# karfly/learnable-triangulation-pytorch

Hardware: AMD Instinct MI355X
Metric: multi-view samples/sec (4-view vol-softmax forward) (higher is better)
Workload: dtype bf16

## Files before the change

include/lt_hip.h:

```cpp
#ifndef LT_HIP_H
#define LT_HIP_H

#include <stddef.h>
#include <stdint.h>

#ifdef __cplusplus
extern "C" {
#endif

#define LT_ABI_VERSION 1

enum { LT_F32 = 0, LT_BF16 = 1,
       LT_FP8 = 2  };
enum { LT_OK = 0, LT_ERR_INVALID = -1, LT_ERR_UNSUPPORTED = -2, LT_ERR_LAUNCH = -3 };

enum { LT_AGG_SUM = 0, LT_AGG_MAX = 1, LT_AGG_SOFTMAX = 2, LT_AGG_CONF = 3,
       LT_AGG_CONF_NORM = 4  };

enum {
    LT_EPI_RELU_PRE = 1,
    LT_EPI_RELU_POST = 2,
    LT_EPI_STORE_F32 = 4,
    LT_EPI_SIGMOID = 8,
    LT_EPI_RES_F32 = 64,
    LT_BN_FROZEN = 32,
    LT_BN_Y_BF16 = 128,
    LT_ACT_BF16 = 256
};

const char* lt_last_error(void);
int lt_abi_version(void);
int lt_device_info(int* cu_count, int* lds_per_cu, char* arch, int arch_len);

#define LT_CONV_MAX_PHASES 8

typedef struct lt_conv_phase {
    const void* weight;
    const int32_t* taps;
    int32_t ntaps;
    int32_t out_off[3];
    const void* weight_frag;
    int32_t weight_frag_layout;
} lt_conv_phase;

typedef struct lt_conv_desc {
    int32_t dtype;
    int32_t N, D, H, W, Cin;
    int32_t Do, Ho, Wo;
    int32_t stride[3], pad[3];
    int32_t OD, OH, OW;
    int32_t out_stride[3];
    int32_t Cout, ldc;
    int32_t cout_pad, k_pad;
    int32_t nphase;
    int32_t flags;
    int32_t tile;
    int32_t stages;
    lt_conv_phase phase[LT_CONV_MAX_PHASES];
} lt_conv_desc;

int lt_conv_pack_weights(const void* weight, int32_t cout_pad, int32_t k_pad, void* packed, void* stream);
int lt_conv_pack_weights_t32(const void* weight, int32_t cout_pad, int32_t k_pad, int32_t cin, int32_t ntaps, void* packed,
                             void* stream);
int lt_conv_pack_weights32(const void* weight, int32_t cout_pad, int32_t k_pad, void* packed, void* stream);

enum { LT_TILE_AUTO = 0,
       LT_TILE_128x128 = 1, LT_TILE_128x64 = 2, LT_TILE_256x32 = 3, LT_TILE_256x16 = 4, LT_TILE_64x64 = 5,
       LT_TILE2_128x128 = 11, LT_TILE2_128x64 = 12, LT_TILE2_256x32 = 13, LT_TILE2_256x16 = 14, LT_TILE2_64x64 = 15,
       LT_TILE_HALO = 20,
       LT_TILE3_288 = 30,
       LT_TILE_DIRECT = 99  };

int lt_conv_fwd(const lt_conv_desc* desc, const void* x, const float* bias, const float* scale, const float* shift,
                const void* residual, void* y, void* stream);
typedef struct lt_conv_skip {
    const void* x;
    int32_t cin;
    const void* weight_frag;
} lt_conv_skip;
int lt_conv_skip_fwd(const lt_conv_desc* desc, const void* x, const float* bias, const float* scale, const float* shift,
                     const lt_conv_skip* skip, void* y, void* stream);
typedef struct lt_conv_cat2 {
    const void* x;
    int32_t cin, H, W, stride;
} lt_conv_cat2;
int lt_conv_cat2_fwd(const lt_conv_desc* desc, const void* x, const lt_conv_cat2* second, const float* bias, const float* scale, const float* shift,
                     const void* residual, void* y, void* stream);
int lt_conv_cout_pad(int32_t cout);
int32_t lt_conv_chunk_samples(int32_t N, int64_t per_sample);

typedef struct lt_wshape {
    int32_t nd;
    int64_t s[5];
} lt_wshape;
int lt_sel_conv_skip(int32_t dtype, const int32_t x[5], const lt_wshape* w, const int32_t skip_x[5], const lt_wshape* skip_w);
int lt_sel_conv_cat2(int32_t dtype, const int32_t t2[5], const lt_wshape* w_expand, const int32_t x[5], const lt_wshape* w_down, int32_t stride_down);
int lt_sel_splitk_slices(const lt_conv_desc* d, const lt_wshape* w, int32_t transposed);
int lt_sel_bottleneck(int32_t dtype, const int32_t x[5], const lt_wshape w[3], const int32_t strides[3]);
int lt_sel_bottleneck_ds(int32_t dtype, const int32_t x[5], const lt_wshape w[3], const int32_t strides[3], const lt_wshape* w_down, int32_t stride_down);
int lt_sel_expand_reduce(int32_t dtype, const int32_t t2[5], const int32_t res[5], const lt_wshape* w_expand, const lt_wshape* w_reduce);
int lt_sel_stem_pool(int32_t dtype, const int32_t x[5], const lt_wshape* w, int32_t stride, int32_t pad, const int32_t pool[3]);
int lt_sel_pwchain(int32_t dtype, const int32_t x[5], int32_t nlayers, const lt_wshape* w);
int lt_sel_frag_layout(const lt_conv_desc* d, const lt_wshape* w, int32_t transposed, int32_t has_residual);

int lt_maxpool_fwd(int32_t dtype, const void* x, void* y, int32_t N, int32_t D, int32_t H, int32_t W, int32_t C,
                   const int32_t k[3], const int32_t s[3], const int32_t p[3], void* stream);

int lt_global_avgpool(int32_t dtype, const void* x, void* y, int32_t N, int32_t HW, int32_t C, void* stream);

int lt_nchw_to_nhwc(int32_t dtype, const float* x, void* y, int32_t N, int32_t C, int32_t HW, int32_t c_pad, void* stream);
int lt_nhwc_to_nchw_f32(int32_t dtype, const void* x, float* y, int32_t N, int32_t C, int32_t HW, int32_t ld, void* stream);

int lt_splitk_reduce(int32_t dtype, const float* partial, int32_t S, int64_t N, int64_t rows_per_sample, int32_t C, const float* bias,
                     const float* scale, const float* shift, const void* residual, void* y, int32_t flags, void* stream);

int lt_coord_volumes(const float* pos, const float* center, const float* rot, float step, int32_t B, int32_t V,
                     int32_t cmu_transfer, float* coords, void* stream);
int lt_rotate_points(const float* x, const float* rot, float* y, int64_t n, void* stream);

int lt_unproject_fwd(int32_t dtype, const void* feats, const float* proj, const float* coords, const float* conf,
                     void* out, int32_t B, int32_t NV, int32_t C, int32_t h, int32_t w, int32_t v0, int32_t v1,
                     int32_t v2, int32_t agg, void* stream);
int lt_unproject_grid_fwd(int32_t dtype, const void* feats, const float* proj, const float* pos, const float* center, const float* rot,
                          float step, int32_t cmu_transfer, float* coords_out, const float* conf, void* out, int32_t B, int32_t NV,
                          int32_t C, int32_t h, int32_t w, int32_t V, int32_t agg, void* stream);
enum { LT_KIND_MPII = 0, LT_KIND_COCO = 1 };
int lt_cuboid_from_keypoints(const float* keypoints_3d, int32_t B, int32_t J, int32_t kind, double cuboid_side, float* pos, float* center,
                             void* stream);

size_t lt_softargmax3d_workspace(int32_t B, int32_t J, int64_t nvox);
int lt_softargmax3d_fwd(const float* logits, const float* coords, float mult, int32_t softmax, int32_t channels_last,
                        int32_t ld, float* kp, float* probs, int32_t B, int32_t J, int64_t nvox, void* workspace,
                        void* stream);

int lt_softargmax2d_fwd(const float* heatmaps, float mult, int32_t softmax, float* coords, float* probs, int32_t NJ,
                        int32_t h, int32_t w, void* stream);
int lt_softargmax2d_bwd(const float* probs, const float* coords, const float* grad_coords, float mult, int32_t softmax, float* grad_heatmaps,
                        int32_t NJ, int32_t h, int32_t w, void* stream);
int lt_triangulate_dlt_bwd(const float* proj, const float* points, const float* conf, const float* grad_out, float* grad_points, float* grad_conf,
                           int32_t B, int32_t NV, int32_t J, void* stream);

size_t lt_unproject_bwd_workspace(int32_t B, int32_t NV, int32_t C, int32_t v0, int32_t v1, int32_t v2);
int lt_unproject_bwd(int32_t dtype, const void* feats, const float* proj, const float* coords, const float* conf, const float* grad_out,
                     float* grad_feats, float* grad_conf, int32_t B, int32_t NV, int32_t C, int32_t h, int32_t w, int32_t v0, int32_t v1,
                     int32_t v2, int32_t agg, void* workspace, size_t workspace_bytes, void* stream);
int lt_softargmax3d_bwd(const float* probs, const float* coords, const float* kp, const float* grad_kp, const int32_t* gp_idx,
                        const float* gp_val, float multiplier, int32_t softmax, int32_t channels_last, float* grad_logits, int32_t B,
                        int32_t J, int64_t nvox, void* stream);
int lt_softargmax3d_bwd_dense(const float* probs, const float* coords, const float* kp, const float* grad_kp, const int32_t* gp_idx,
                              const float* gp_val, const float* gp_dense, float* workspace_bj, float multiplier, int32_t softmax,
                              int32_t channels_last, float* grad_logits, int32_t B, int32_t J, int64_t nvox, void* stream);
int lt_volumetric_ce_fwd(const float* coords, const float* probs, const float* keypoints_gt, const float* validity, float* terms,
                         int32_t* idx, float* grad_val, int32_t B, int32_t J, int64_t nvox, void* stream);
size_t lt_bn_stats_workspace(int64_t rows, int32_t C);
int lt_bn_stats_fwd(int32_t dtype, const void* x, int64_t rows, int32_t C, float* mean, float* var, float* running_mean,
                    float* running_var, float momentum, void* workspace, void* stream);

int lt_bn_act_fwd(const void* y , const float* mean, const float* var, const float* gamma, const float* beta, const void* residual, void* z,
                  void* z_bf16 , int64_t rows, int32_t C, float eps,
                  int32_t flags, void* stream);
size_t lt_bn_act_bwd_workspace(int64_t rows, int32_t C);
int lt_bn_act_bwd(const void* dz, const void* y , const void* residual, const float* mean, const float* var, const float* gamma, const float* beta,
                  void* dy, void* dy_bf16 , float* dgamma, float* dbeta, void* dres, int32_t accumulate_res,
                  int64_t rows, int32_t C, float eps, int32_t flags, void* workspace, void* stream);
int lt_act_bwd(const void* dz, const void* z, const void* residual, void* dy, void* dres, int32_t accumulate_res, int64_t total, int32_t flags,
               void* stream);
size_t lt_channel_sum_workspace(int64_t rows, int32_t C);
int lt_channel_sum(const float* x, int64_t rows, int32_t C, float* out, int32_t accumulate, void* workspace, void* stream);
int lt_channel_sum_dt(int32_t dtype, const void* x, int64_t rows, int32_t C, float* out, int32_t accumulate, void* workspace, void* stream);
int lt_maxpool_bwd(const float* x, const float* dy, float* dx, int32_t N, int32_t D, int32_t H, int32_t W, int32_t C, const int32_t k[3],
                   const int32_t s[3], const int32_t p[3], void* stream);
int lt_maxpool_bwd_dt(int32_t dtype, const void* x, const void* dy, void* dx, int32_t N, int32_t D, int32_t H, int32_t W, int32_t C, const int32_t k[3],
                      const int32_t s[3], const int32_t p[3], void* stream);
size_t lt_conv_wgrad_workspace(int64_t rows, int32_t cout_pad, int32_t k_pad);
int lt_conv_wgrad(const float* dy, const float* x, const int32_t* taps, float* dw, int32_t N, int32_t D, int32_t H, int32_t W, int32_t Cin, int32_t Do,
                  int32_t Ho, int32_t Wo, const int32_t stride[3], const int32_t pad[3], int32_t Cout, int32_t ldy, int32_t cout_pad, int32_t k_pad,
                  int32_t ntaps, int32_t accumulate, void* workspace, void* stream);
size_t lt_pack_n8_bf16_bytes(int32_t N, int64_t P, int32_t C);
// ... 69 lines not shown
    int32_t N, H, W;
    int32_t Cin, Cout;
    const void* weight;
    const float* bias;
    const float* scale;
    const float* shift;
    int32_t x_layout;
} lt_stem_desc;
size_t lt_stem_packed_bytes(void);
int lt_stem_pack_weights(const void* weight, int32_t k_pad, void* packed, void* stream);
int lt_stem_pool_fwd(const lt_stem_desc* desc, const void* x, void* y, void* stream);

typedef struct {
    int32_t dtype;
    int32_t N, H, W;
    int32_t C, P;
    const void* weight[3];
    const float* bias[3];
    const float* scale[3];
    const float* shift[3];
} lt_bneck_desc;
int lt_bottleneck_fwd(const lt_bneck_desc* desc, const void* x, void* y, void* stream);

typedef struct {
    int32_t dtype;
    int32_t N, H, W;
    int32_t Cin, P, C;
    const void* weight[4];
    const float* scale[4];
    const float* shift[4];
} lt_bneck_ds_desc;
int lt_bottleneck_ds_fwd(const lt_bneck_ds_desc* desc, const void* x, void* y, void* stream);

typedef struct {
    int32_t dtype;
    int32_t C, P;
    int64_t M;
    const void* weight[2];
    const float* scale[2];
    const float* shift[2];
    const float* consts;
} lt_xr_desc;
int lt_expand_reduce_fwd(const lt_xr_desc* desc, const void* t2, const void* residual, void* y, void* t1_next, void* stream);

int lt_graph_begin(void* stream);
int lt_graph_end(void* stream, void** graph_exec_out);
int lt_graph_launch(void* graph_exec, void* stream);
int lt_graph_destroy(void* graph_exec);
int lt_event_create(void** ev_out);
int lt_event_record(void* ev, void* stream);
int lt_event_elapsed_ms(void* ev_start, void* ev_stop, float* ms_out);
int lt_event_destroy(void* ev);

typedef struct lt_plan lt_plan;
typedef struct lt_named_tensor {
    const char* name;
    const float* data;
    int32_t ndim;
    int64_t shape[5];
} lt_named_tensor;
typedef struct lt_vol_plan_config {
    int32_t dtype;
    int32_t num_layers;
    int32_t style_caffe;
    int32_t num_joints;
    int32_t B, NV, H, W;
    int32_t volume_size;
    double cuboid_side;
    double volume_multiplier;
    int32_t volume_softmax;
    int32_t aggregation;
    int32_t transfer_cmu_to_human36m;
    int32_t use_graph;
} lt_vol_plan_config;
typedef struct lt_plan_info_t {
    int32_t launches;
    int32_t heatmap_h, heatmap_w;
    double flops;
    int64_t bytes_allocated;
    int32_t n_expand_reduce, n_bottleneck, n_bottleneck_ds, n_conv_cat2, n_conv2d_halo, n_pwchain, n_stem_pool, n_splitk, n_conv_skip;
    int32_t graph_captured;
    const float* logits;
    int32_t logits_planar;
} lt_plan_info_t;
int lt_plan_create_vol(const lt_vol_plan_config* cfg, const lt_named_tensor* weights, int32_t nweights, lt_plan** plan_out);
int lt_plan_forward_vol(lt_plan* plan, const float* images, const double* K_host, const double* R_host, const double* t_host, const double* base_points_host,
                        const double* rot_host, float* keypoints_3d, float* volumes, float* features, float* coord_volumes, float* vol_confidences, void* stream);
enum { LT_MODEL_ALG = 1, LT_MODEL_RANSAC = 2 };
typedef struct lt_alg_plan_config {
    int32_t model;
    int32_t dtype;
    int32_t num_layers;
    int32_t style_caffe;
    int32_t num_joints;
    int32_t B, NV, H, W;
    int32_t use_confidences;
    int32_t heatmap_softmax;
    double heatmap_multiplier;
    int32_t direct_optimization;
    double reprojection_error_epsilon;
    int32_t use_graph;
} lt_alg_plan_config;
int lt_plan_create_alg(const lt_alg_plan_config* cfg, const lt_named_tensor* weights, int32_t nweights, lt_plan** plan_out);
int lt_plan_forward_alg(lt_plan* plan, const float* images, const float* proj, float* keypoints_3d, void* keypoints_2d, float* heatmaps,
                        float* confidences, void* stream);
typedef struct lt_cascade_plan_config {
    lt_alg_plan_config alg;
    lt_vol_plan_config vol;
    int32_t kind;
} lt_cascade_plan_config;
int lt_plan_create_cascade(const lt_cascade_plan_config* cfg, const lt_named_tensor* alg_weights, int32_t n_alg, const lt_named_tensor* vol_weights,
                           int32_t n_vol, lt_plan** plan_out);
int lt_plan_forward_cascade(lt_plan* plan, const float* images, const double* K_host, const double* R_host, const double* t_host, const double* rot_host,
                            float* keypoints_3d, float* alg_keypoints_3d, float* base_points, float* volumes, float* features, float* coord_volumes,
                            float* vol_confidences, void* stream);
int lt_plan_info(const lt_plan* plan, lt_plan_info_t* info);
void lt_plan_destroy(lt_plan* plan);

#ifdef __cplusplus
}
#endif
#endif
```

learnable-triangulation-pytorch_amd/csrc/conv2d_halo.hip:

```cpp
#include <stdlib.h>

#include <type_traits>

#include "conv_common.h"

using namespace lt;

namespace {

__device__ uint4 g_zero_page_2d[4];

typedef __attribute__((address_space(3))) void* lptr_t;

__device__ __forceinline__ void dma16p(const void* src, unsigned lds_base) {
    unsigned keep;
    lds_base = __builtin_amdgcn_readfirstlane(lds_base);
    asm volatile(
        "s_mov_b32 %0, m0\n\t"
        "s_mov_b32 m0, %2\n\t"
        "s_nop 0\n\t"
        "global_load_lds_dwordx4 %1, off\n\t"
        "s_mov_b32 m0, %0"
        : "=&s"(keep)
        : "v"(src), "s"(lds_base)
        : "memory");
}

template <int I0, int I1, typename F>
__device__ __forceinline__ void static_for_p(F&& f) {
    if constexpr (I0 < I1) {
        f(std::integral_constant<int, I0>{});
        static_for_p<I0 + 1, I1>(f);
    }
}

struct Halo2dPhase {
    const bf16_t* wfrag;
    const int4* taps;
    int ooh, oow;
};

struct Halo2dArgs {
    const bf16_t* x;
    bf16_t* y;
    const float* bias;
    const float* scale;
    const float* shift;
    int N, H, W, OH, OW, osh, osw, ldc, flags, tiles_h, tiles_w, pad_h, pad_w;
    int tile0;
    Halo2dPhase ph[4];
};

template <int TH, int NT, int NPH>
__global__ __launch_bounds__(512, (TH == 8 ? 1 : 2)) void conv2d_halo_kernel(const Halo2dArgs a) {
    typedef bf16_t T;
    constexpr int CIN = 256, CP = 256, TW = 24, G = CIN / 16, NB = CP / 32, PW = TW + 2, HH = TH + 2, PXB = CIN * 2;
    constexpr int RG = TH / 4, CG = TW / 8, FR = RG * CG;
    constexpr int HV = HH * PW, NI = HV * PXB / 1024;
    static_assert(HV % 2 == 0 && PXB == 512 && NB == 8, "two pixels per DMA piece; eight waves = eight output blocks");
    auto swz = [](int hh_, int hw_) -> int { return (hw_ & 7) | ((hh_ & 1) << 3); };

    extern __shared__ __attribute__((aligned(1024))) unsigned char smem[];
    const unsigned lds0 = (unsigned)(size_t)(lptr_t)smem;
    unsigned long long zp_bits = (unsigned long long)(size_t)g_zero_page_2d;
    asm volatile("" : "+s"(zp_bits));
    const void* const zero_page = (const void*)(size_t)zp_bits;

    const int t = threadIdx.x, lane = t & 63;
    const int wave = __builtin_amdgcn_readfirstlane(t >> 6);
    int lin = blockIdx.x;
    {
        const int nb = gridDim.x, q = nb >> 3, r = nb & 7, xcd = lin & 7, j = lin >> 3;
        lin = (xcd < r ? xcd * (q + 1) : r * (q + 1) + (xcd - r) * q) + j;
    }
    lin += a.tile0;
    const int tpi = a.tiles_h * a.tiles_w;
    const int n = lin / tpi, rem = lin - n * tpi;
    const int h0 = (rem / a.tiles_w) * TH, w0 = (rem % a.tiles_w) * TW;
    const T* __restrict__ x = a.x + (size_t)n * a.H * a.W * CIN;

    for (int i = wave; i < NI; i += 8) {
        const int hv = 2 * i + (lane >> 5), ps = lane & 31;
        const int hh_ = hv / PW, hw_ = hv - hh_ * PW;
        const int ih = h0 - 1 + hh_, iw = w0 - 1 + hw_;
        const bool ok = ((unsigned)ih < (unsigned)a.H) & ((unsigned)iw < (unsigned)a.W);
        const void* src = ok ? (const void*)(x + ((size_t)ih * a.W + iw) * CIN + (ps ^ swz(hh_, hw_)) * 8) : zero_page;
        dma16p(src, lds0 + i * 1024);
    }

    const int cb = wave;
    const int vl = lane & 31, hk = lane >> 5;
#ifndef LT_H2D_WD
#define LT_H2D_WD 7
#endif
    constexpr int NU = NT * G, WD = LT_H2D_WD, NS = WD + 1;
    static_assert(NU % NS == 0, "the fragment ring must close at a phase boundary");
    auto wptr = [&](int p) -> const T* { return a.ph[p].wfrag + ((size_t)cb * 64 + lane) * 8; };
    auto load_w = [&](int p, int u) -> V16 {
        V16 v;
        v.u = *(const uint4*)(wptr(p) + (size_t)u * NB * 64 * 8);
        return v;
    };
    V16 wf[NS];
#pragma unroll
    for (int u = 0; u < WD; ++u) wf[u] = load_w(0, u);

    float esc[16], esf[16];
    auto load_consts = [&]() {
#pragma unroll
        for (int e = 0; e < 16; ++e) {
            const int c = 32 * cb + 16 * (e >> 3) + 8 * hk + (e & 7);
            const float bi = a.bias ? a.bias[c] : 0.f, sc = a.scale ? a.scale[c] : 1.f, sf = a.shift ? a.shift[c] : 0.f;
            esc[e] = sc; esf[e] = bi * sc + sf;
        }
    };
    if constexpr (NPH > 1) load_consts();
    const EpiFloors fl = epi_floors(a.flags);
    int tapo[NPH][NT];
    {
        int4 tv[NPH][NT];
#pragma unroll
        for (int p = 0; p < NPH; ++p)
#pragma unroll
            for (int tp = 0; tp < NT; ++tp) tv[p][tp] = a.ph[p].taps[tp];
        bool bad = false;
#pragma unroll
        for (int p = 0; p < NPH; ++p)
#pragma unroll
            for (int tp = 0; tp < NT; ++tp) {
                const int dh = tv[p][tp].y - a.pad_h, dw = tv[p][tp].z - a.pad_w;
                bad |= (tv[p][tp].x != 0) | (dh < -1) | (dh > 1) | (dw < -1) | (dw > 1);
                tapo[p][tp] = __builtin_amdgcn_readfirstlane((1 + dh) * 32 + (1 + dw));
            }
        if (bad) __builtin_trap();
    }

    asm volatile("s_waitcnt vmcnt(0)\n\ts_barrier" ::: "memory");

    static_for_p<0, NPH>([&](auto pc) {
        constexpr int p = decltype(pc)::value;
        unsigned lp[NT][RG];
#pragma unroll
        for (int i = 0; i < RG; ++i) {
            const int th = 4 * i + (vl >> 3), tw = vl & 7;
#pragma unroll
            for (int tp = 0; tp < NT; ++tp) {
                const int row = th + (tapo[p][tp] >> 5), col = tw + (tapo[p][tp] & 31);
                lp[tp][i] = lds0 + (row * PW + col) * PXB + ((hk ^ swz(row, col)) << 4);
            }
        }
        f32x16 acc[FR];
#pragma unroll
        for (int f = 0; f < FR; ++f)
#pragma unroll
            for (int e = 0; e < 16; ++e) acc[f][e] = 0.f;
#ifndef LT_H2D_XLOOK
#define LT_H2D_XLOOK 1
#endif
        constexpr int XL = LT_H2D_XLOOK, XS = XL + 1;
        V16 xa[XS][FR];
        auto load_x = [&](auto uc, V16 (&dst)[FR]) {
            constexpr int u = decltype(uc)::value;
            constexpr int tap = u / G, g = u % G;
            static_for_p<0, FR>([&](auto fc) {
                constexpr int f = decltype(fc)::value, i = f / CG, j = f % CG;
                dst[f].u = *(const uint4*)((lptr_t)(size_t)((lp[tap][i] ^ (g << 5)) + j * 8 * PXB));
            });
        };
        static_for_p<0, XL>([&](auto uc) { load_x(uc, xa[decltype(uc)::value % XS]); });
        static_for_p<0, NU>([&](auto uc) {
            constexpr int u = decltype(uc)::value;
            if constexpr (u + WD < NU) wf[(u + WD) % NS] = load_w(p, u + WD);
            else if constexpr (p + 1 < NPH) wf[(u + WD) % NS] = load_w(p + 1, u + WD - NU);
            if constexpr (u + XL < NU) load_x(std::integral_constant<int, u + XL>{}, xa[(u + XL) % XS]);
#pragma unroll
            for (int f = 0; f < FR; ++f)
                acc[f] = __builtin_amdgcn_mfma_f32_32x32x16_bf16(wf[u % NS].h, xa[u % XS][f].h, acc[f], 0, 0, 0);
            __builtin_amdgcn_sched_barrier(0);
        });

        if constexpr (NPH == 1) load_consts();
#pragma unroll
        for (int f = 0; f < FR; ++f) {
            const int th = 4 * (f / CG) + (vl >> 3), tw = 8 * (f % CG) + (vl & 7);
            bf16_t* yo = a.y + (((size_t)n * a.OH + (h0 + th) * a.osh + a.ph[p].ooh) * a.OW + (w0 + tw) * a.osw + a.ph[p].oow) * a.ldc + 32 * cb + 8 * hk;
#pragma unroll
            for (int q = 0; q < 2; ++q) {
                unsigned o[4];
#pragma unroll
                for (int d = 0; d < 4; ++d) {
                    const int e = 8 * q + 2 * d;
                    o[d] = pack_bf16x2(epi_apply(fmaf(acc[f][e], esc[e], esf[e]), fl, 0.f), epi_apply(fmaf(acc[f][e + 1], esc[e + 1], esf[e + 1]), fl, 0.f));
                }
                *(uint4*)(yo + 16 * q) = make_uint4(o[0], o[1], o[2], o[3]);
            }
        }
    });
}

template <int TH, int NT, int NPH>
int launch_halo2d(const Halo2dArgs& a0, hipStream_t s, long long first = 0, long long count = -1) {
    Halo2dArgs a = a0;
    a.tiles_h = a.H / TH;
    a.tiles_w = a.W / 24;
    const long long total = (long long)a.N * a.tiles_h * a.tiles_w;
    if (count < 0) count = total - first;
    if (count <= 0) return LT_OK;
    a.tile0 = (int)first;
    constexpr int lds = (TH + 2) * 26 * 512;
    static_assert(lds <= 160 * 1024, "halo fits LDS");
    auto kern = conv2d_halo_kernel<TH, NT, NPH>;
    LT_OPT_IN_LDS(kern, 160 * 1024);
    hipLaunchKernelGGL(kern, dim3((unsigned)count), dim3(512), lds, s, a);
    LT_CHECK_LAUNCH("lt_conv_fwd(2D halo)");
    return LT_OK;
}

}

namespace lt {

int conv2d_halo_try(int dtype, const ConvArgs& c, int cout_pad, int nphase, hipStream_t s) {
    if (dtype != LT_BF16 || c.res || c.skip_x || c.x2 || !halo2d_fits(c, cout_pad, nphase)) return 0;
    Halo2dArgs a;
    for (int p = 0; p < nphase; ++p) {
        const PhaseArg& ph = c.phase[p];
        if (!ph.wfrag_t) return 0;
        a.ph[p].wfrag = (const bf16_t*)ph.wfrag_t; a.ph[p].taps = ph.taps; a.ph[p].ooh = ph.ooh; a.ph[p].oow = ph.oow;
    }
    a.x = (const bf16_t*)c.x; a.y = (bf16_t*)c.y;
    a.bias = c.bias; a.scale = c.scale; a.shift = c.shift;
    a.N = c.N; a.H = c.H; a.W = c.W; a.OH = c.OH; a.OW = c.OW; a.osh = c.osh; a.osw = c.osw; a.ldc = c.ldc; a.flags = c.flags; a.tiles_h = a.tiles_w = 0;
    a.pad_h = c.ph; a.pad_w = c.pw; a.tile0 = 0;
    const char* th = getenv("LT_H2D_TH");
    const long long tiles8 = (long long)c.N * (c.H / 8) * (c.W / 24);
    const int n_cu = lt::device_cu_count8();
    const bool th4 = th ? th[0] == '4' : tiles8 <= n_cu / 2;
    int rc;
    if (nphase != 1) rc = launch_halo2d<8, 4, 4>(a, s);
    else if (th4) rc = launch_halo2d<4, 9, 1>(a, s);
    else {
        const long long rem = tiles8 % n_cu;
        const bool split = !th && tiles8 > n_cu && rem > 0 && 2 * rem <= n_cu && (tiles8 - rem) % (c.W / 24) == 0 && !env_on("LT_H2D_NO_TAIL4");
        if (split) {
            rc = launch_halo2d<8, 9, 1>(a, s, 0, tiles8 - rem);
            if (rc == LT_OK) rc = launch_halo2d<4, 9, 1>(a, s, 2 * (tiles8 - rem), 2 * rem);
        } else rc = launch_halo2d<8, 9, 1>(a, s);
    }
    return rc == LT_OK ? 1 : rc;
}

}
```

learnable-triangulation-pytorch_amd/csrc/conv_common.h:

```cpp
#pragma once
#include "lt_common.h"

namespace lt {

typedef float f32x16 __attribute__((ext_vector_type(16)));
typedef float f32x4 __attribute__((ext_vector_type(4)));
typedef __bf16 bf16x8 __attribute__((ext_vector_type(8)));

struct PhaseArg {
    const void* w;
    const void* wfrag;
    const void* wfrag_t;
    const void* wfrag32;
    const int4* taps;
    int ntaps;
    int ood, ooh, oow;
};

struct ConvArgs {
    const void* x;
    void* y;
    const void* res;
    const float* bias;
    const float* scale;
    const float* shift;
    int N, D, H, W, Cin, log2Cin;
    int Do, Ho, Wo;
    int sd, sh, sw, pd, ph, pw;
    int OD, OH, OW, osd, osh, osw;
    int Cout, ldc, k_pad, flags;
    int M;
    int tiles_n;
    int stages;
    PhaseArg phase[LT_CONV_MAX_PHASES];
    const void* skip_x;
    const void* skip_w;
    const void* x2;
    int Cin2, H2, W2, s2;
};

inline ConvArgs conv_args_of(const lt_conv_desc& d) {
    ConvArgs a = {};
    a.N = d.N; a.D = d.D; a.H = d.H; a.W = d.W; a.Cin = d.Cin;
    a.Do = d.Do; a.Ho = d.Ho; a.Wo = d.Wo;
    a.sd = d.stride[0]; a.sh = d.stride[1]; a.sw = d.stride[2];
    a.pd = d.pad[0]; a.ph = d.pad[1]; a.pw = d.pad[2];
    a.OD = d.OD; a.OH = d.OH; a.OW = d.OW;
    a.osd = d.out_stride[0]; a.osh = d.out_stride[1]; a.osw = d.out_stride[2];
    a.Cout = d.Cout; a.ldc = d.ldc; a.k_pad = d.k_pad; a.flags = d.flags; a.tiles_n = 1; a.stages = d.stages;
    for (int p = 0; p < d.nphase && p < LT_CONV_MAX_PHASES; ++p) {
        const lt_conv_phase& ph = d.phase[p];
        a.phase[p].w = ph.weight;
        a.phase[p].wfrag = ph.weight_frag_layout == 1 ? ph.weight_frag : nullptr;
        a.phase[p].wfrag_t = ph.weight_frag_layout == 2 ? ph.weight_frag : nullptr;
        a.phase[p].wfrag32 = ph.weight_frag_layout == 3 ? ph.weight_frag : nullptr;
        a.phase[p].taps = (const int4*)ph.taps; a.phase[p].ntaps = ph.ntaps;
        a.phase[p].ood = ph.out_off[0]; a.phase[p].ooh = ph.out_off[1]; a.phase[p].oow = ph.out_off[2];
    }
    return a;
}

inline bool halo_col_fits(long long N, int D, int H, int W) {
    if (D % 4 || H % 8 || W % 8) return false;
    const long long nblk = N * (D / 4) * (H / 8) * (W / 8), cols = N * (H / 8) * (W / 8);
    return nblk >= 1024 && nblk % 8 == 0 && D / 4 >= 2 && cols % 8 == 0 && cols >= 256;
}

inline bool halo2d_fits(const ConvArgs& c, int cout_pad, int nphase) {
    if ((nphase != 1 && nphase != 4) || c.D != 1 || c.Do != 1 || c.OD != 1) return false;
    if (c.sh != 1 || c.sw != 1 || c.H != c.Ho || c.W != c.Wo || c.W % 24 || c.H % 8) return false;
    if (c.Cin != 256 || cout_pad != 256 || c.Cout != 256 || c.ldc % 8 || (c.flags & (LT_EPI_STORE_F32 | LT_EPI_SIGMOID)) || c.pd != 0) return false;
    if (nphase == 1 && (c.osh != 1 || c.osw != 1 || c.OH != c.Ho || c.OW != c.Wo || c.ph != 1 || c.pw != 1)) return false;
    if (nphase == 4 && (c.osh != 2 || c.osw != 2 || c.OH != 2 * c.Ho || c.OW != 2 * c.Wo || c.ph != 0 || c.pw != 0)) return false;
    for (int p = 0; p < nphase; ++p)
        if (c.phase[p].ntaps != (nphase == 1 ? 9 : 4) || c.phase[p].ood) return false;
    return true;
}

union V16 {
    uint4 u;
    f32x4 f;
    bf16x8 h;
};

template <typename T, int MF> struct Mma;
template <> struct Mma<float, 32> {
    typedef f32x16 acc_t;
    static __device__ __forceinline__ void run(acc_t& c, const V16& a, const V16& b) {
#pragma unroll
        for (int e = 0; e < 4; ++e) c = __builtin_amdgcn_mfma_f32_32x32x2f32(a.f[e], b.f[e], c, 0, 0, 0);
    }
};
template <> struct Mma<float, 16> {
    typedef f32x4 acc_t;
    static __device__ __forceinline__ void run(acc_t& c, const V16& a, const V16& b) {
#pragma unroll
        for (int e = 0; e < 4; ++e) c = __builtin_amdgcn_mfma_f32_16x16x4f32(a.f[e], b.f[e], c, 0, 0, 0);
    }
};
template <> struct Mma<bf16_t, 32> {
    typedef f32x16 acc_t;
    static __device__ __forceinline__ void run(acc_t& c, const V16& a, const V16& b) {
        c = __builtin_amdgcn_mfma_f32_32x32x16_bf16(a.h, b.h, c, 0, 0, 0);
    }
};
template <> struct Mma<bf16_t, 16> {
    typedef f32x4 acc_t;
    static __device__ __forceinline__ void run(acc_t& c, const V16& a, const V16& b) {
        c = __builtin_amdgcn_mfma_f32_16x16x32_bf16(a.h, b.h, c, 0, 0, 0);
    }
};

union V16Q {
    uint4 u;
    long q[2];
};
template <> struct Mma<fp8_t, 32> {
    typedef f32x16 acc_t;
    static __device__ __forceinline__ void run(acc_t& c, const V16& a, const V16& b) {
        V16Q qa, qb;
        qa.u = a.u; qb.u = b.u;
        c = __builtin_amdgcn_mfma_f32_32x32x16_fp8_fp8(qa.q[0], qb.q[0], c, 0, 0, 0);
        c = __builtin_amdgcn_mfma_f32_32x32x16_fp8_fp8(qa.q[1], qb.q[1], c, 0, 0, 0);
    }
};
template <> struct Mma<fp8_t, 16> {
    typedef f32x4 acc_t;
    static __device__ __forceinline__ void run(acc_t& c, const V16& a, const V16& b) {
        V16Q qa, qb;
        qa.u = a.u; qb.u = b.u;
        c = __builtin_amdgcn_mfma_f32_16x16x32_fp8_fp8(qa.q[0], qb.q[0], c, 0, 0, 0);
        c = __builtin_amdgcn_mfma_f32_16x16x32_fp8_fp8(qa.q[1], qb.q[1], c, 0, 0, 0);
    }
};

__device__ __forceinline__ void decode_row(const ConvArgs& a, int m, int& n, int& od, int& oh, int& ow) {
    int hw = a.Ho * a.Wo;
    int dhw = a.Do * hw;
    n = m / dhw;
    int r = m - n * dhw;
    od = r / hw;
    r -= od * hw;
    oh = r / a.Wo;
    ow = r - oh * a.Wo;
}

constexpr int ROW_BYTES = 128;
constexpr int LT_EPI_NO_RES_PREFETCH = 1 << 16;
constexpr int LT_EPI_NO_XCD_REMAP = 1 << 17;

int conv2_dispatch(int dtype, const ConvArgs& a, int cout_pad, int nphase, int max_taps, int tile, hipStream_t s);
int conv3_try(int dtype, const ConvArgs& a, int cout_pad, int nphase, int max_taps, bool forced, hipStream_t s);
int conv7_try(const ConvArgs& a, int cout_pad, int max_taps, bool pw, hipStream_t s);
int conv_pw_try(int dtype, const ConvArgs& a, int cout_pad, int nphase, hipStream_t s);
int conv2d_halo_try(int dtype, const ConvArgs& a, int cout_pad, int nphase, hipStream_t s);
int conv3d_halo_try(int dtype, const ConvArgs& a, int cout_pad, int nphase, bool forced, hipStream_t s);

}
```

learnable-triangulation-pytorch_amd/csrc/conv_igemm.hip:

```cpp
#include <stdlib.h>

#include "conv_common.h"

using namespace lt;

namespace {


template <typename T, int BM, int BN, int WM, int WN, int MF>
__global__ __launch_bounds__(256) void conv_igemm_kernel(const ConvArgs a) {
    constexpr int VEC = elt<T>::vec;
    constexpr int BK = 8 * VEC;
    constexpr int A_IT = BM / 32;
    constexpr int B_VECS = BN * 8;
    constexpr int B_IT = (B_VECS + 255) / 256;
    constexpr int SM = WM / MF, SN = WN / MF;
    constexpr int WAVES_N = BN / WN;
    constexpr int G = (MF == 32) ? 4 : 2;
    constexpr int NACC = (MF == 32) ? 16 : 4;
    static_assert((BM / WM) * WAVES_N == 4, "4 waves");
    typedef typename Mma<T, MF>::acc_t acc_t;

    extern __shared__ __attribute__((aligned(16))) unsigned char smem[];
    unsigned char* sA = smem;
// ... 321 lines not shown
                                      (((d->flags & LT_EPI_STORE_F32) && (!residual || (d->flags & LT_EPI_RES_F32))) ||
                                       (!(d->flags & LT_EPI_STORE_F32) && d->Cout % 8 == 0 && d->ldc % 8 == 0))),
               LT_ERR_UNSUPPORTED, "lt_conv_fwd: an fp8 convolution stores fp32 (LT_EPI_STORE_F32, fp32 residual: LT_EPI_RES_F32) or, with Cout %% 8 == 0, bf16 (bf16 residual)");
    LT_REQUIRE(d->dtype != LT_FP8 || d->tile == LT_TILE_AUTO || d->tile == LT_TILE_HALO || (d->tile >= LT_TILE2_128x128 && d->tile <= LT_TILE2_64x64), LT_ERR_UNSUPPORTED,
               "lt_conv_fwd: fp8 convolutions run on the generic implicit-GEMM tiles and the halo kernel only");
    const int l2 = ilog2_exact(d->Cin);
    LT_REQUIRE(l2 >= 0 && d->Cin >= vec, LT_ERR_UNSUPPORTED,
               "lt_conv_fwd: Cin=%d must be a power of two >= %d (pad the channel dimension)", d->Cin, vec);
    LT_REQUIRE(d->nphase >= 1 && d->nphase <= LT_CONV_MAX_PHASES, LT_ERR_INVALID, "lt_conv_fwd: nphase=%d", d->nphase);
    LT_REQUIRE(d->k_pad > 0 && d->k_pad % (8 * vec) == 0, LT_ERR_INVALID, "lt_conv_fwd: k_pad=%d not a multiple of %d", d->k_pad, 8 * vec);
    LT_REQUIRE(d->Cout >= 1 && d->ldc >= d->Cout && d->cout_pad >= d->Cout, LT_ERR_INVALID, "lt_conv_fwd: Cout/ldc/cout_pad");
    LT_REQUIRE(!(d->flags & LT_EPI_RES_F32) || ((d->flags & LT_EPI_STORE_F32) && d->dtype != LT_F32), LT_ERR_INVALID,
               "lt_conv_fwd: LT_EPI_RES_F32 goes with LT_EPI_STORE_F32 on a bf16 / fp8 convolution");
    const long long M = (long long)d->N * d->Do * d->Ho * d->Wo;
    const long long in_elems = (long long)d->N * d->D * d->H * d->W * d->Cin;
    const long long out_pix = (long long)d->N * d->OD * d->OH * d->OW;
    LT_REQUIRE(M > 0 && M < (1ll << 31) && in_elems < (1ll << 31) && out_pix < (1ll << 31), LT_ERR_UNSUPPORTED,
               "lt_conv_fwd: tensor too large for 32-bit indexing (M=%lld, in=%lld)", M, in_elems);
    ConvArgs a = conv_args_of(*d);
    a.x = x; a.y = y; a.res = residual; a.bias = bias; a.scale = scale; a.shift = shift; a.log2Cin = l2; a.M = (int)M;
    a.skip_x = skip ? skip->x : nullptr; a.skip_w = skip ? skip->weight_frag : nullptr;
    a.x2 = cat2 ? cat2->x : nullptr; a.Cin2 = cat2 ? cat2->cin : 0; a.H2 = cat2 ? cat2->H : 0; a.W2 = cat2 ? cat2->W : 0; a.s2 = cat2 ? cat2->stride : 0;
    int max_taps = 0;
    for (int p = 0; p < d->nphase; ++p) {
        const lt_conv_phase& ph = d->phase[p];
        LT_REQUIRE(ph.weight && ph.taps && ph.ntaps >= 1, LT_ERR_INVALID, "lt_conv_fwd: phase %d incomplete", p);
        LT_REQUIRE((long long)ph.ntaps * d->Cin <= d->k_pad, LT_ERR_INVALID, "lt_conv_fwd: phase %d: ntaps*Cin > k_pad", p);
        if (ph.ntaps > max_taps) max_taps = ph.ntaps;
    }
    LT_REQUIRE(max_taps <= 2048, LT_ERR_UNSUPPORTED, "lt_conv_fwd: too many taps (%d)", max_taps);
    hipStream_t s = (hipStream_t)stream;
    if (skip) {
        LT_REQUIRE(skip->x && skip->weight_frag && skip->cin == 16 && d->dtype == LT_BF16 && !residual && d->Cin == 32 && d->Cout == 32 && d->cout_pad == 32,
                   LT_ERR_UNSUPPORTED, "lt_conv_skip_fwd: bf16 3x3x3 32 -> 32 with a 16-channel skip tensor only (cin %d, Cin %d, Cout %d)", skip->cin, d->Cin, d->Cout);
        const int rc = conv3d_halo_try(LT_BF16, a, d->cout_pad, d->nphase, true, s);
        LT_REQUIRE(rc == 1, rc < 0 ? rc : LT_ERR_UNSUPPORTED, "lt_conv_skip_fwd: this shape is not covered by the column-walk halo kernel (N %d, %d x %d x %d)",
                   d->N, d->D, d->H, d->W);
        return LT_OK;
    }
    if (cat2) {
        const bool pointwise = d->nphase == 1 && d->phase[0].ntaps == 1 && d->D == 1 && d->Do == 1 && d->OD == 1 && d->H == d->Ho && d->W == d->Wo &&
                               d->OH == d->Ho && d->OW == d->Wo && d->stride[1] == 1 && d->stride[2] == 1 && d->pad[1] == 0 && d->pad[2] == 0 &&
                               d->out_stride[1] == 1 && d->out_stride[2] == 1 && !d->phase[0].out_off[1] && !d->phase[0].out_off[2];
        LT_REQUIRE(cat2->x && d->dtype == LT_BF16 && pointwise && d->Cin % 32 == 0 && cat2->cin % 32 == 0 && d->k_pad == d->Cin + cat2->cin && d->k_pad % 64 == 0 &&
                       d->cout_pad % 256 == 0 && d->phase[0].weight_frag_layout == 3 && d->phase[0].weight_frag && (cat2->stride == 1 || cat2->stride == 2) &&
                       cat2->H == d->Ho * cat2->stride && cat2->W == d->Wo * cat2->stride && !(d->flags & (LT_EPI_STORE_F32 | LT_EPI_SIGMOID)) &&
                       (long long)d->N * cat2->H * cat2->W * cat2->cin < (1ll << 31),
                   LT_ERR_UNSUPPORTED, "lt_conv_cat2_fwd: bf16 1x1 convolution, Cin %d + %d (multiples of 32, k_pad %d their sum), cout_pad %d (%% 256), fragment layout 3, "
                   "second map %d x %d = stride %d x the output's", d->Cin, cat2->cin, d->k_pad, d->cout_pad, cat2->H, cat2->W, cat2->stride);
        const int rc = conv7_try(a, d->cout_pad, max_taps, true, s);
        LT_REQUIRE(rc == 1, rc < 0 ? rc : LT_ERR_UNSUPPORTED, "lt_conv_cat2_fwd: not covered by the 288 x 256 pointwise kernel");
        return LT_OK;
    }
    if (d->dtype == LT_F32) return dispatch<float>(a, d->cout_pad, d->nphase, max_taps, d->tile, s);
    if (d->dtype == LT_FP8) {
        if ((d->tile == LT_TILE_AUTO || d->tile == LT_TILE_HALO) && !(d->flags & LT_EPI_STORE_F32)) {
            const int rc = conv3d_halo_try(LT_FP8, a, d->cout_pad, d->nphase, d->tile == LT_TILE_HALO, s);
            if (rc == 1) return LT_OK;
            if (rc < 0) return rc;
        }
        LT_REQUIRE(d->tile != LT_TILE_HALO, LT_ERR_UNSUPPORTED, "lt_conv_fwd: LT_TILE_HALO requested but this fp8 problem has no halo kernel");
        return conv2_dispatch(LT_FP8, a, d->cout_pad, d->nphase, max_taps, d->tile, s);
    }
    return dispatch<bf16_t>(a, d->cout_pad, d->nphase, max_taps, d->tile, s);
}

extern "C" int lt_conv_fwd(const lt_conv_desc* d, const void* x, const float* bias, const float* scale, const float* shift,
                           const void* residual, void* y, void* stream) {
    return conv_fwd_impl(d, x, bias, scale, shift, residual, nullptr, nullptr, y, stream);
}

extern "C" int lt_conv_cat2_fwd(const lt_conv_desc* d, const void* x, const lt_conv_cat2* second, const float* bias, const float* scale, const float* shift,
                                const void* residual, void* y, void* stream) {
    LT_REQUIRE(second, LT_ERR_INVALID, "lt_conv_cat2_fwd: null second-source descriptor");
    return conv_fwd_impl(d, x, bias, scale, shift, residual, nullptr, second, y, stream);
}

extern "C" int lt_conv_skip_fwd(const lt_conv_desc* d, const void* x, const float* bias, const float* scale, const float* shift,
                                const lt_conv_skip* skip, void* y, void* stream) {
    LT_REQUIRE(skip, LT_ERR_INVALID, "lt_conv_skip_fwd: null skip descriptor");
    return conv_fwd_impl(d, x, bias, scale, shift, nullptr, skip, nullptr, y, stream);
}

extern "C" int lt_conv_cout_pad(int32_t cout) {
    if (cout <= 16) return 16;
    if (cout <= 32) return 32;
    if (cout <= 64) return 64;
    return (cout + 127) / 128 * 128;
}
```

learnable-triangulation-pytorch_amd/csrc/plan.hip:

```cpp
#include <math.h>
#include <stdlib.h>
#include <string.h>

#include <array>
#include <deque>
#include <functional>
#include <map>
#include <string>
#include <unordered_map>
#include <vector>

#include "lt_common.h"

using namespace lt;

namespace {

#define PL_TRY(call)                   \
    do {                               \
        const int rc_ = (call);        \
        if (rc_ != LT_OK) return rc_;  \
    } while (0)
#define PL_HIP(call)                                                        \
    do {                                                                    \
// ... 106 lines not shown
    LT_REQUIRE(stride == 2, LT_ERR_UNSUPPORTED, "plan: only stride-2 transposed convolutions");
    const int ks[3] = {kd, kh, kw}, dims[3] = {D, Hh, W};
    int outs[3];
    for (int i = 0; i < 3; ++i) {
        if (!nd3 && i == 0) { outs[i] = 1; continue; }
        const int o = (dims[i] - 1) * 2 - 2 * pd[i] + ks[i] + output_padding;
        LT_REQUIRE(o == 2 * dims[i], LT_ERR_UNSUPPORTED, "plan: a transposed convolution must exactly double the size (k = 4, p = 1 / k = 2, p = 0)");
        outs[i] = o;
    }
    const int cp = cout_pad_of(cout);
    struct DimPhase { int phi; std::vector<std::pair<int, int>> taps; };
    auto dim_phases = [&](int i) {
        std::vector<DimPhase> res;
        if (!nd3 && i == 0) { res.push_back({0, {{0, 0}}}); return res; }
        for (int phi = 0; phi < 2; ++phi) {
            DimPhase dp; dp.phi = phi;
            for (int kk = 0; kk < ks[i]; ++kk)
                if (floormod(phi + pd[i] - kk, 2) == 0) dp.taps.push_back({kk, floordiv(phi + pd[i] - kk, 2)});
            res.push_back(dp);
        }
        return res;
    };
    const int64_t ktot = (int64_t)kd * kh * kw;
    struct Raw { std::vector<std::pair<std::vector<float>, int>> dummy; };
    std::vector<PhaseSpec> phases;
    std::vector<std::vector<int>> phase_k;
    int ntaps_max = 0;
    for (const DimPhase& A : dim_phases(0))
        for (const DimPhase& Bp : dim_phases(1))
            for (const DimPhase& Cp : dim_phases(2)) {
                PhaseSpec ph; std::vector<int> kidx;
                for (auto& ta : A.taps)
                    for (auto& tb : Bp.taps)
                        for (auto& tc : Cp.taps) {
                            const int da = ta.second, db = tb.second, dc = tc.second;
                            ph.taps.push_back(da); ph.taps.push_back(db); ph.taps.push_back(dc); ph.taps.push_back(((da * Hh + db) * W + dc) * cin);
                            kidx.push_back((ta.first * kh + tb.first) * kw + tc.first);
                        }
                if (kidx.empty()) { ph.taps = {0, 0, 0, 0}; kidx.push_back(-1); }
                ph.ntaps = (int)kidx.size();
                ph.off[0] = A.phi; ph.off[1] = Bp.phi; ph.off[2] = Cp.phi;
                if (ph.ntaps > ntaps_max) ntaps_max = ph.ntaps;
                phases.push_back(ph); phase_k.push_back(kidx);
            }
    const int K = ntaps_max * cin, k_pad = (K + kstep - 1) / kstep * kstep;
    for (size_t p = 0; p < phases.size(); ++p) {
        PhaseSpec& ph = phases[p];
        ph.w.assign((size_t)cp * k_pad, 0.f);
        for (int t = 0; t < ph.ntaps; ++t) {
            const int kt = phase_k[p][t];
            if (kt < 0) continue;
            for (int ci = 0; ci < cin; ++ci)
                for (int co = 0; co < cout; ++co) ph.w[(size_t)co * k_pad + (size_t)t * cin + ci] = w.d[((int64_t)ci * cout + co) * ktot + kt];
        }
    }
    LT_REQUIRE((int)phases.size() <= LT_CONV_MAX_PHASES, LT_ERR_UNSUPPORTED, "plan: %d phases", (int)phases.size());
    sp.Cin = cin; sp.Do = D; sp.Ho = Hh; sp.Wo = W; sp.OD = outs[0]; sp.OH = outs[1]; sp.OW = outs[2];
    for (int i = 0; i < 3; ++i) { sp.st[i] = 1; sp.pd[i] = 0; }
    sp.ostr[0] = nd3 ? 2 : 1; sp.ostr[1] = 2; sp.ostr[2] = 2;
    sp.Cout = cout; sp.cout_pad = cp; sp.k_pad = k_pad;
    fold_bn(cout, bias, bn, cp, sp.bias, sp.scale, sp.shift);
    sp.ph = std::move(phases);
    return LT_OK;
}

}

struct lt_plan {
    lt_vol_plan_config cfg;
    int model = 0;
    lt_alg_plan_config acfg = {};
    const char* who = "lt_plan_create_vol";
    int dtype = LT_F32, es = 4;
    std::unordered_map<std::string, const lt_named_tensor*> sd;
    std::vector<void*> allocs;
    std::map<std::pair<size_t, int>, std::vector<char*>> pool;
    size_t bytes_alloc = 0;
    double flops = 0;
    typedef std::function<int(hipStream_t)> Op;
    std::vector<Op> ops;
    int npre = 0, ntail = 0;
    std::deque<lt_conv_desc> conv_descs;
    std::deque<lt_conv_skip> skip_descs;
    std::deque<lt_conv_cat2> cat2_descs;
    std::deque<lt_pwchain_desc> pw_descs;
    std::deque<lt_stem_desc> stem_descs;
    std::deque<lt_bneck_desc> bneck_descs;
    std::deque<lt_bneck_ds_desc> bneck_ds_descs;
    std::deque<lt_xr_desc> xr_descs;
    hipGraphExec_t graph = nullptr;
    bool captured = false;
    hipStream_t own_stream = nullptr; hipEvent_t own_ev[2] = {nullptr, nullptr};
    const float* cur_images = nullptr;
    float* out_kp = nullptr; float* out_probs = nullptr; float* out_feats = nullptr;
    const float* cur_proj = nullptr; void* out_kp2d = nullptr; float* out_hm = nullptr; float* out_conf = nullptr;
    float* geo_dev = nullptr; float* geo_host[GEO_RING] = {nullptr, nullptr, nullptr, nullptr}; hipEvent_t geo_ev[GEO_RING] = {nullptr, nullptr, nullptr, nullptr};
    int geo_slot = 0; size_t n_geo = 0, o_pos = 0, o_cen = 0, o_rot = 0;
    Act feats, vol, logits, volc;
    float* coords = nullptr; float* kp = nullptr; float* probs = nullptr; void* sa_ws = nullptr;
    Act algc;
    float* hm_nchw = nullptr; float* kp_hm = nullptr; int64_t* kp_i64 = nullptr;
    int hm_h = 0, hm_w = 0;
    lt_plan* sub_alg = nullptr; lt_plan* sub_vol = nullptr; int kind = 0;
    float* cproj_dev = nullptr; float* cproj_host[GEO_RING] = {nullptr, nullptr, nullptr, nullptr}; float* ckp_alg = nullptr;
    int n_xr = 0, n_bneck = 0, n_bneck_ds = 0, n_cat2 = 0, n_halo2d = 0, n_pwchain = 0, n_stem = 0, n_splitk = 0, n_conv_skip = 0;

    ~lt_plan() {
        if (graph) (void)hipGraphExecDestroy(graph);
        if (own_stream) (void)hipStreamDestroy(own_stream);
        for (int i = 0; i < 2; ++i) if (own_ev[i]) (void)hipEventDestroy(own_ev[i]);
        for (void* p : allocs) (void)hipFree(p);
        for (int i = 0; i < GEO_RING; ++i) { if (geo_host[i]) (void)hipHostFree(geo_host[i]); if (geo_ev[i]) (void)hipEventDestroy(geo_ev[i]); }
        for (int i = 0; i < GEO_RING; ++i) if (cproj_host[i]) (void)hipHostFree(cproj_host[i]);
        delete sub_alg;
        delete sub_vol;
    }

    int dev_alloc(size_t bytes, void** out) {
        void* p = nullptr;
        PL_HIP(hipMalloc(&p, bytes ? bytes : 16));
        allocs.push_back(p);
        bytes_alloc += bytes;
        *out = p;
        return LT_OK;
    }
    int alloc(int n, int d, int h, int w, int c, int esz, Act& a) {
        a = Act(); a.n = n; a.d = d; a.h = h; a.w = w; a.c = c; a.es = esz;
        auto it = pool.find({a.bytes(), esz});
        if (it != pool.end() && !it->second.empty()) { a.p = it->second.back(); it->second.pop_back(); return LT_OK; }
        void* p; PL_TRY(dev_alloc(a.bytes(), &p)); a.p = (char*)p;
        return LT_OK;
    }
    void release(const Act& a) { if (a.p && a.pooled) pool[{a.bytes(), a.es}].push_back(a.p); }
    int upload(const void* host, size_t bytes, void** out) {
        PL_TRY(dev_alloc(bytes, out));
        PL_HIP(hipMemcpy(*out, host, bytes, hipMemcpyHostToDevice));
        return LT_OK;
    }
    int upload_f32(const std::vector<float>& v, const float** out) { void* p; PL_TRY(upload(v.data(), v.size() * 4, &p)); *out = (const float*)p; return LT_OK; }
    int upload_w(const std::vector<float>& v, const void** out) {
        if (es == 4) { void* p; PL_TRY(upload(v.data(), v.size() * 4, &p)); *out = p; return LT_OK; }
        std::vector<unsigned short> h(v.size());
        for (size_t i = 0; i < v.size(); ++i) h[i] = bf16_rne(v[i]);
        void* p; PL_TRY(upload(h.data(), h.size() * 2, &p)); *out = p;
        return LT_OK;
    }
    int upload_i32(const std::vector<int32_t>& v, const int32_t** out) { void* p; PL_TRY(upload(v.data(), v.size() * 4, &p)); *out = (const int32_t*)p; return LT_OK; }

    int get(const std::string& name, WT& w, int nd_expect = 0) {
        auto it = sd.find(name);
        LT_REQUIRE(it != sd.end(), LT_ERR_INVALID, "%s: state dict has no '%s'", who, name.c_str());
        const lt_named_tensor* t = it->second;
        LT_REQUIRE(t->data && t->ndim >= 1 && t->ndim <= 5 && (!nd_expect || t->ndim == nd_expect), LT_ERR_INVALID, "%s: '%s' has %d dimensions", who, name.c_str(), t->ndim);
        w.d = t->data; w.nd = t->ndim;
        for (int i = 0; i < t->ndim; ++i) w.s[i] = t->shape[i];
        return LT_OK;
    }
    bool has(const std::string& name) const { return sd.find(name) != sd.end(); }
    int get_vec(const std::string& name, int n, const float** out) {
        WT w; PL_TRY(get(name, w));
        LT_REQUIRE(w.numel() == n, LT_ERR_INVALID, "%s: '%s' has %lld elements, expected %d", who, name.c_str(), (long long)w.numel(), n);
        *out = w.d;
        return LT_OK;
    }
    int get_bn(const std::string& prefix, int c, BN& bn) {
        PL_TRY(get_vec(prefix + ".weight", c, &bn.g)); PL_TRY(get_vec(prefix + ".bias", c, &bn.b));
        PL_TRY(get_vec(prefix + ".running_mean", c, &bn.m)); PL_TRY(get_vec(prefix + ".running_var", c, &bn.v));
        return LT_OK;
    }

    struct ConvOpt {
        const float* bias = nullptr; const BN* bn = nullptr;
        int stride = 1, pad = 0; bool transposed = false, relu = false, relu_pre = false, out_f32 = false, sigmoid = false;
        const Act* residual = nullptr;
        const Act* skip_x = nullptr; const WT* skip_w = nullptr; const float* skip_bias = nullptr; const BN* skip_bn = nullptr;
    };

    void fill_desc(lt_conv_desc& d, const ConvSpec& sp) {
        memset(&d, 0, sizeof(d));
        d.dtype = dtype;
        d.N = sp.N; d.D = sp.D; d.H = sp.H; d.W = sp.W; d.Cin = sp.Cin; d.Do = sp.Do; d.Ho = sp.Ho; d.Wo = sp.Wo;
        for (int i = 0; i < 3; ++i) { d.stride[i] = sp.st[i]; d.pad[i] = sp.pd[i]; d.out_stride[i] = sp.ostr[i]; }
        d.OD = sp.OD; d.OH = sp.OH; d.OW = sp.OW;
        d.Cout = sp.Cout; d.ldc = sp.Cout; d.cout_pad = sp.cout_pad; d.k_pad = sp.k_pad;
        d.nphase = (int)sp.ph.size(); d.flags = sp.flags; d.tile = 0; d.stages = 0;
        for (size_t i = 0; i < sp.ph.size(); ++i) {
            d.phase[i].ntaps = sp.ph[i].ntaps;
            for (int k = 0; k < 3; ++k) d.phase[i].out_off[k] = sp.ph[i].off[k];
        }
    }

    int pack_frag(const void* wdev, size_t elems, int which, int cout_pad, int k_pad, int cin, int ntaps, const void** out) {
        void* p; PL_TRY(dev_alloc(elems * 2, &p));
        int rc;
        if (which == 2) rc = lt_conv_pack_weights_t32(wdev, cout_pad, k_pad, cin, ntaps, p, nullptr);
        else if (which == 3) rc = lt_conv_pack_weights32(wdev, cout_pad, k_pad, p, nullptr);
        else rc = lt_conv_pack_weights(wdev, cout_pad, k_pad, p, nullptr);
        PL_TRY(rc);
        PL_HIP(hipStreamSynchronize(nullptr));
        *out = p;
        return LT_OK;
    }

    int conv(const Act& x, const WT& w, const ConvOpt& o, Act& y) {
        const int flags = (o.relu ? LT_EPI_RELU_POST : 0) | (o.relu_pre ? LT_EPI_RELU_PRE : 0) | (o.out_f32 ? LT_EPI_STORE_F32 : 0) | (o.sigmoid ? LT_EPI_SIGMOID : 0);
        const int in[5] = {x.n, x.d, x.h, x.w, x.c};
        ConvSpec sp;
        PL_TRY(make_conv_spec(w, o.bias, o.bn, in, o.stride, o.pad, es, o.transposed, flags, 0, sp));
        const lt_wshape ws = wshape(w);
        lt_conv_skip* sk = nullptr;
        if (o.skip_x) {
            const lt_wshape sws = wshape(*o.skip_w);
            LT_REQUIRE(!o.residual && !o.relu_pre && !o.out_f32 && lt_sel_conv_skip(dtype, in, &ws, dims(*o.skip_x).data(), &sws), LT_ERR_INVALID, "plan: conv_skip on an unsupported shape");
            const int sin[5] = {o.skip_x->n, o.skip_x->d, o.skip_x->h, o.skip_x->w, o.skip_x->c};
            ConvSpec ss;
            PL_TRY(make_conv_spec(*o.skip_w, o.skip_bias, o.skip_bn, sin, 1, 0, es, false, 0, 0, ss));
            LT_REQUIRE(ss.cout_pad == 32 && sp.cout_pad == 32, LT_ERR_INVALID, "plan: conv_skip widths");
            std::vector<float> wf((size_t)32 * ss.k_pad);
            for (int co = 0; co < 32; ++co) for (int k = 0; k < ss.k_pad; ++k) wf[(size_t)co * ss.k_pad + k] = ss.ph[0].w[(size_t)co * ss.k_pad + k] * ss.scale[co];
            for (int co = 0; co < 32; ++co) { const float bs = ss.bias[co] * ss.scale[co]; const float t = sp.shift[co] + bs; sp.shift[co] = t + ss.shift[co]; }
            const void* wsk; PL_TRY(upload_w(wf, &wsk));
            const void* wfr; PL_TRY(pack_frag(wsk, 32 * 16, 2, 32, ss.k_pad, 16, 1, &wfr));
            skip_descs.emplace_back();
            sk = &skip_descs.back();
            sk->x = o.skip_x->p; sk->cin = 16; sk->weight_frag = wfr;
            ++n_conv_skip;
        }
        lt_conv_desc d0;
        fill_desc(d0, sp);
        const int S = lt_sel_splitk_slices(&d0, &ws, o.transposed);
        if (S > 1) return conv_splitk(x, w, sp, S, o.residual, y);
        PL_TRY(alloc(sp.N, sp.OD, sp.OH, sp.OW, sp.Cout, o.out_f32 ? 4 : es, y));
        if (o.residual) LT_REQUIRE(o.residual->n == y.n && o.residual->d == y.d && o.residual->h == y.h && o.residual->w == y.w && o.residual->c == y.c && o.residual->es == es,
                                   LT_ERR_INVALID, "plan: residual shape");
        conv_descs.push_back(d0);
        lt_conv_desc& d = conv_descs.back();
        const int layout = lt_sel_frag_layout(&d, &ws, o.transposed, o.residual != nullptr);
        if (layout == 2 && w.nd == 4) ++n_halo2d;
        for (size_t i = 0; i < sp.ph.size(); ++i) {
            const PhaseSpec& ph = sp.ph[i];
            const void* wdev; PL_TRY(upload_w(ph.w, &wdev));
            const int32_t* tdev; PL_TRY(upload_i32(ph.taps, &tdev));
            d.phase[i].weight = wdev; d.phase[i].taps = tdev;
            if (layout) {
                const void* wfr; PL_TRY(pack_frag(wdev, (size_t)sp.cout_pad * sp.k_pad, layout, sp.cout_pad, sp.k_pad, sp.Cin, ph.ntaps, &wfr));
                d.phase[i].weight_frag = wfr; d.phase[i].weight_frag_layout = layout;
            }
        }
        const float *bi, *sc, *sh;
        PL_TRY(upload_f32(sp.bias, &bi)); PL_TRY(upload_f32(sp.scale, &sc)); PL_TRY(upload_f32(sp.shift, &sh));
        long long taps = 0;
        for (auto& q : sp.ph) taps += q.ntaps;
        flops += 2.0 * sp.N * sp.Do * sp.Ho * sp.Wo * sp.Cout * taps * (o.transposed ? w.s[0] : w.s[1]);
        const lt_conv_desc* dp = &d;
        const void* xp = x.p; void* yp = y.p; const void* rp = o.residual ? o.residual->p : nullptr;
        if (sk) {
            flops += 2.0 * sp.N * sp.Do * sp.Ho * sp.Wo * sp.Cout * 16;
            ops.push_back([=](hipStream_t s) { return lt_conv_skip_fwd(dp, xp, bi, sc, sh, sk, yp, s); });
        } else
            ops.push_back([=](hipStream_t s) { return lt_conv_fwd(dp, xp, bi, sc, sh, rp, yp, s); });
        return LT_OK;
    }

    int conv_splitk(const Act& x, const WT& w, const ConvSpec& sp, int S, const Act* residual, Act& y) {
        const PhaseSpec& ph0 = sp.ph[0];
        const int ntaps = ph0.ntaps, Cin = sp.Cin, kstep = 128 / es;
        std::vector<int> bounds(S + 1);
        int maxg = 0;
        for (int i = 0; i <= S; ++i) bounds[i] = ntaps * i / S;
        for (int i = 0; i < S; ++i) if (bounds[i + 1] - bounds[i] > maxg) maxg = bounds[i + 1] - bounds[i];
        const int kp = (maxg * Cin + kstep - 1) / kstep * kstep;
        Act part; PL_TRY(alloc(sp.N, S * sp.Do, sp.Ho, sp.Wo, sp.Cout, 4, part));
        PL_TRY(alloc(sp.N, sp.Do, sp.Ho, sp.Wo, sp.Cout, es, y));
        const long long rows = (long long)sp.N * sp.Do * sp.Ho * sp.Wo;
        conv_descs.emplace_back();
        lt_conv_desc& d = conv_descs.back();
        fill_desc(d, sp);
        d.OD = S * sp.Do; d.k_pad = kp; d.nphase = S; d.flags = LT_EPI_STORE_F32;
        d.tile = rows >= 8192 ? LT_TILE2_128x128 : LT_TILE2_64x64;
        for (int i = 0; i < S; ++i) {
            const int t0 = bounds[i], t1 = bounds[i + 1];
            std::vector<float> wk((size_t)sp.cout_pad * kp, 0.f);
            for (int co = 0; co < sp.cout_pad; ++co)
                for (int k = t0 * Cin; k < t1 * Cin; ++k) wk[(size_t)co * kp + (k - t0 * Cin)] = ph0.w[(size_t)co * sp.k_pad + k];
            std::vector<int32_t> tp(ph0.taps.begin() + 4 * t0, ph0.taps.begin() + 4 * t1);
            const void* wdev; PL_TRY(upload_w(wk, &wdev));
            const int32_t* tdev; PL_TRY(upload_i32(tp, &tdev));
            d.phase[i].weight = wdev; d.phase[i].taps = tdev; d.phase[i].ntaps = t1 - t0;
            d.phase[i].out_off[0] = i * sp.Do; d.phase[i].out_off[1] = 0; d.phase[i].out_off[2] = 0;
        }
        std::vector<float> zero(sp.cout_pad, 0.f), one(sp.cout_pad, 1.f);
        const float *ibi, *isc, *ish, *bi, *sc, *sh;
        PL_TRY(upload_f32(zero, &ibi)); PL_TRY(upload_f32(one, &isc)); PL_TRY(upload_f32(zero, &ish));
        PL_TRY(upload_f32(sp.bias, &bi)); PL_TRY(upload_f32(sp.scale, &sc)); PL_TRY(upload_f32(sp.shift, &sh));
        flops += 2.0 * rows * sp.Cout * ntaps * w.s[1];
        const lt_conv_desc* dp = &d;
        const void* xp = x.p; float* pp = (float*)part.p; void* yp = y.p; const void* rp = residual ? residual->p : nullptr;
        ops.push_back([=](hipStream_t s) { return lt_conv_fwd(dp, xp, ibi, isc, ish, nullptr, pp, s); });
        const int dt = dtype, N = sp.N, C = sp.Cout, fl = sp.flags;
        const long long R = (long long)sp.Do * sp.Ho * sp.Wo;
        ops.push_back([=](hipStream_t s) { return lt_splitk_reduce(dt, pp, S, N, R, C, bi, sc, sh, rp, yp, fl, s); });
        release(part);
        ++n_splitk;
        return LT_OK;
    }

    int conv_cat2(const Act& t2, const WT& we, const BN& bne, const Act& x, const WT& wd, const BN& bnd, int sds, Act& y) {
        const int N = t2.n, Ho = t2.h, Wo = t2.w, P = t2.c, Cc = (int)we.s[0], Cin2 = (int)wd.s[1];
        const int t2s[5] = {t2.n, t2.d, t2.h, t2.w, t2.c}, xs[5] = {x.n, x.d, x.h, x.w, x.c};
        ConvSpec s3, sd_;
        PL_TRY(make_conv_spec(we, nullptr, &bne, t2s, 1, 0, es, false, LT_EPI_RELU_POST, 0, s3));
        PL_TRY(make_conv_spec(wd, nullptr, &bnd, xs, sds, 0, es, false, 0, 0, sd_));
        LT_REQUIRE(s3.cout_pad == Cc && sd_.cout_pad == Cc, LT_ERR_INVALID, "plan: conv_cat2 widths");
        const int kp = P + Cin2;
        std::vector<float> wcat((size_t)Cc * kp), shift(Cc), zero(Cc, 0.f);
        for (int co = 0; co < Cc; ++co) {
            for (int k = 0; k < P; ++k) wcat[(size_t)co * kp + k] = s3.ph[0].w[(size_t)co * s3.k_pad + k] * s3.scale[co];
            for (int k = 0; k < Cin2; ++k) wcat[(size_t)co * kp + P + k] = sd_.ph[0].w[(size_t)co * sd_.k_pad + k] * sd_.scale[co];
            const float a = s3.bias[co] * s3.scale[co], a2 = a + s3.shift[co], b = sd_.bias[co] * sd_.scale[co], b2 = b + sd_.shift[co];
            shift[co] = a2 + b2;
        }
        PL_TRY(alloc(N, 1, Ho, Wo, Cc, es, y));
        conv_descs.emplace_back();
        lt_conv_desc& d = conv_descs.back();
        memset(&d, 0, sizeof(d));
        d.dtype = dtype; d.N = N; d.D = 1; d.H = Ho; d.W = Wo; d.Cin = P; d.Do = 1; d.Ho = Ho; d.Wo = Wo;
        for (int i = 0; i < 3; ++i) { d.stride[i] = 1; d.pad[i] = 0; d.out_stride[i] = 1; }
        d.OD = 1; d.OH = Ho; d.OW = Wo; d.Cout = Cc; d.ldc = Cc; d.cout_pad = Cc; d.k_pad = kp; d.nphase = 1; d.flags = LT_EPI_RELU_POST;
        const void* wdev; PL_TRY(upload_w(wcat, &wdev));
        const int32_t* tdev; PL_TRY(upload_i32(s3.ph[0].taps, &tdev));
        const void* wfr; PL_TRY(pack_frag(wdev, (size_t)Cc * kp, 3, Cc, kp, 0, 0, &wfr));
        d.phase[0].weight = wdev; d.phase[0].taps = tdev; d.phase[0].ntaps = 1; d.phase[0].weight_frag = wfr; d.phase[0].weight_frag_layout = 3;
        cat2_descs.emplace_back();
        lt_conv_cat2& c2 = cat2_descs.back();
        c2.x = x.p; c2.cin = Cin2; c2.H = x.h; c2.W = x.w; c2.stride = sds;
        const float *bi, *sh;
        PL_TRY(upload_f32(zero, &bi)); PL_TRY(upload_f32(shift, &sh));
        flops += 2.0 * N * Ho * Wo * Cc * kp;
        const lt_conv_desc* dp = &d; const lt_conv_cat2* cp = &c2;
        const void* xp = t2.p; void* yp = y.p;
        ops.push_back([=](hipStream_t s) { return lt_conv_cat2_fwd(dp, xp, cp, bi, nullptr, sh, nullptr, yp, s); });
        ++n_cat2;
        return LT_OK;
// ... 150 lines not shown
        else { b.strides[0] = stride; b.strides[1] = 1; b.strides[2] = 1; }
        for (int i = 0; i < b.nconv; ++i) {
            PL_TRY(get(pre + ".conv" + std::to_string(i + 1) + ".weight", b.w[i], 4));
            PL_TRY(get_bn(pre + ".bn" + std::to_string(i + 1), (int)b.w[i].s[0], b.bn[i]));
        }
        if (ds) { PL_TRY(get(pre + ".downsample.0.weight", b.wd, 4)); PL_TRY(get_bn(pre + ".downsample.1", (int)b.wd.s[0], b.bnd)); }
        return LT_OK;
    }
    int record_block(const Block& b, const Act& x, const Act* t1_in, const Block* nxt, Act& y, Act& t1n) {
        t1n = Act();
        const lt_wshape w3[3] = {wshape(b.w[0]), wshape(b.w[1]), wshape(b.w[2])}, wd = wshape(b.wd);
        if (b.bottleneck && !b.has_ds && !t1_in && !nxt && lt_sel_bottleneck(dtype, dims(x).data(), w3, b.strides)) return bottleneck(x, b.w, b.bn, y);
        if (b.bottleneck && b.has_ds && !t1_in && !nxt && lt_sel_bottleneck_ds(dtype, dims(x).data(), w3, b.strides, &wd, b.sds))
            return bottleneck_ds(x, b.w, b.bn, b.wd, b.bnd, y);
        if (t1_in || nxt) {
            Act t1, t2;
            ConvOpt o;
            if (t1_in) t1 = *t1_in;
            else { o = ConvOpt(); o.bn = &b.bn[0]; o.relu = true; PL_TRY(conv(x, b.w[0], o, t1)); }
            o = ConvOpt(); o.bn = &b.bn[1]; o.relu = true; o.pad = 1; PL_TRY(conv(t1, b.w[1], o, t2));
            release(t1);
            const lt_wshape wr = nxt ? wshape(nxt->w[0]) : lt_wshape{};
            if (nxt && lt_sel_expand_reduce(dtype, dims(t2).data(), dims(x).data(), &w3[2], &wr)) {
                PL_TRY(expand_reduce(t2, x, b.w[2], b.bn[2], nxt->w[0], nxt->bn[0], y, t1n));
                release(t2);
                return LT_OK;
            }
            o = ConvOpt(); o.bn = &b.bn[2]; o.relu = true; o.residual = &x; PL_TRY(conv(t2, b.w[2], o, y));
            release(t2);
            return LT_OK;
        }
        if (b.bottleneck && b.has_ds) {
            const int Ho = (x.h - 1) / b.sds + 1, Wo = (x.w - 1) / b.sds + 1;
            const int t2s[5] = {x.n, 1, Ho, Wo, (int)b.w[2].s[1]};
            if (lt_sel_conv_cat2(dtype, t2s, &w3[2], dims(x).data(), &wd, b.sds)) {
                Act t1, t2; ConvOpt o;
                o.bn = &b.bn[0]; o.relu = true; o.stride = b.strides[0]; PL_TRY(conv(x, b.w[0], o, t1));
                o = ConvOpt(); o.bn = &b.bn[1]; o.relu = true; o.stride = b.strides[1]; o.pad = 1; PL_TRY(conv(t1, b.w[1], o, t2));
                release(t1);
                PL_TRY(conv_cat2(t2, b.w[2], b.bn[2], x, b.wd, b.bnd, b.sds, y));
                release(t2);
                return LT_OK;
            }
        }
        Act res = x; bool own_res = false;
        if (b.has_ds) { ConvOpt o; o.bn = &b.bnd; o.stride = b.sds; PL_TRY(conv(x, b.wd, o, res)); own_res = true; }
        Act cur = x;
        for (int i = 0; i < b.nconv; ++i) {
            const bool last = i + 1 == b.nconv;
            ConvOpt o; o.bn = &b.bn[i]; o.relu = true; o.stride = b.strides[i]; o.pad = (int)b.w[i].s[2] / 2; o.residual = last ? &res : nullptr;
            Act z; PL_TRY(conv(cur, b.w[i], o, z));
            if (cur.p != x.p) release(cur);
            cur = z;
        }
        if (own_res) release(res);
        y = cur;
        return LT_OK;
    }

    int record_gap_head(const std::string& pre, const Act& x, Act& out) {
        WT w0, w4; const float *b0, *b4; BN bn1, bn5;
        PL_TRY(get(pre + ".features.0.weight", w0, 4)); PL_TRY(get_vec(pre + ".features.0.bias", (int)w0.s[0], &b0)); PL_TRY(get_bn(pre + ".features.1", (int)w0.s[0], bn1));
        PL_TRY(get(pre + ".features.4.weight", w4, 4)); PL_TRY(get_vec(pre + ".features.4.bias", (int)w4.s[0], &b4)); PL_TRY(get_bn(pre + ".features.5", (int)w4.s[0], bn5));
        Act y, p, g;
        ConvOpt o; o.bias = b0; o.bn = &bn1; o.pad = 1; o.relu = true; PL_TRY(conv(x, w0, o, y));
        PL_TRY(maxpool(y, 2, 2, 0, 2, p)); release(y);
        o = ConvOpt(); o.bias = b4; o.bn = &bn5; o.pad = 1; o.relu = true; PL_TRY(conv(p, w4, o, y)); release(p);
        PL_TRY(maxpool(y, 2, 2, 0, 2, p)); release(y);
        PL_TRY(global_avgpool(p, g)); release(p);
        Act cur = g;
        for (int i = 0; i < 3; ++i) {
            WT lw; const float* lb;
            PL_TRY(get(pre + ".head." + std::to_string(2 * i) + ".weight", lw, 2));
            PL_TRY(get_vec(pre + ".head." + std::to_string(2 * i) + ".bias", (int)lw.s[0], &lb));
            lw.nd = 4; lw.s[2] = 1; lw.s[3] = 1;
            ConvOpt lo; lo.bias = lb; lo.relu = i < 2; lo.sigmoid = i == 2; lo.out_f32 = i == 2;
            Act z; PL_TRY(conv(cur, lw, lo, z)); release(cur);
            cur = z;
        }
        out = cur;
        return LT_OK;
    }

    int record_backbone(int N, int Hh, int W, int num_layers, bool caffe, const char* conf_head, bool want_heatmaps, Act& feats256, Act& conf, Act& heatmaps) {
        int nb[4]; bool bott;
        switch (num_layers) {
            case 18: bott = false; nb[0] = 2; nb[1] = 2; nb[2] = 2; nb[3] = 2; break;
            case 34: bott = false; nb[0] = 3; nb[1] = 4; nb[2] = 6; nb[3] = 3; break;
            case 50: bott = true; nb[0] = 3; nb[1] = 4; nb[2] = 6; nb[3] = 3; break;
            case 101: bott = true; nb[0] = 3; nb[1] = 4; nb[2] = 23; nb[3] = 3; break;
            case 152: bott = true; nb[0] = 3; nb[1] = 8; nb[2] = 36; nb[3] = 3; break;
            default: set_error("%s: num_layers %d (18 / 34 / 50 / 101 / 152)", who, num_layers); return LT_ERR_INVALID;
        }
        if (caffe) bott = true;
        const int exp = bott ? 4 : 1;
        WT w1; BN bn1;
        PL_TRY(get("backbone.conv1.weight", w1, 4)); PL_TRY(get_bn("backbone.bn1", 64, bn1));
        Act y;
        const int32_t stem_in[5] = {N, 1, Hh, W, 8}, pool[3] = {3, 2, 1};
        const lt_wshape ws1 = wshape(w1);
        if (w1.s[1] == 3 && lt_sel_stem_pool(dtype, stem_in, &ws1, 2, 3, pool)) PL_TRY(stem_pool(N, Hh, W, w1, bn1, y));
        else {
            const int cpad = 16 / es;
            Act xin; PL_TRY(alloc(N, 1, Hh, W, cpad, es, xin)); xin.pooled = false;
            const int dt = dtype; lt_plan* self = this; void* xp = xin.p;
            ops.push_back([=](hipStream_t s) { return lt_nchw_to_nhwc(dt, self->cur_images, xp, N, 3, Hh * W, cpad, s); });
            npre = 1;
            ConvOpt o; o.bn = &bn1; o.stride = 2; o.pad = 3; o.relu = true;
            Act c1; PL_TRY(conv(xin, w1, o, c1));
            PL_TRY(maxpool(c1, 3, 2, 1, 2, y)); release(c1);
        }
        int inplanes = 64;
        const int planes_of[4] = {64, 128, 256, 512};
        for (int li = 0; li < 4; ++li) {
            const int planes = planes_of[li], stride = li == 0 ? 1 : 2;
            std::vector<Block> blocks(nb[li]);
            for (int bi = 0; bi < nb[li]; ++bi) {
                const int st = bi == 0 ? stride : 1;
                const bool ds = bi == 0 && (st != 1 || inplanes != planes * exp);
                PL_TRY(load_block("backbone.layer" + std::to_string(li + 1) + "." + std::to_string(bi), bott, caffe, st, ds, blocks[bi]));
                inplanes = planes * exp;
            }
            Act t1; bool have_t1 = false;
            for (int bi = 0; bi < nb[li]; ++bi) {
                const Block& blk = blocks[bi];
                const Block* nxt = bi + 1 < nb[li] ? &blocks[bi + 1] : nullptr;
                const bool chain = nxt && blk.identity_bottleneck() && nxt->identity_bottleneck() && dtype == LT_BF16 && blk.w[2].s[0] == 1024 && blk.w[2].s[1] == 256 &&
                                   nxt->w[0].s[0] == 256 && nxt->w[0].s[1] == 1024;
                Act z, t1n;
                if (chain) PL_TRY(record_block(blk, y, have_t1 ? &t1 : nullptr, nxt, z, t1n));
                else if (have_t1) PL_TRY(record_block(blk, y, &t1, nullptr, z, t1n));
                else PL_TRY(record_block(blk, y, nullptr, nullptr, z, t1n));
                release(y);
                y = z; t1 = t1n; have_t1 = !t1n.null();
            }
        }
        conf = Act();
        if (conf_head) PL_TRY(record_gap_head(conf_head, y, conf));
        for (int i = 0; i < 3; ++i) {
            WT dw; BN dbn;
            PL_TRY(get("backbone.deconv_layers." + std::to_string(3 * i) + ".weight", dw, 4));
            PL_TRY(get_bn("backbone.deconv_layers." + std::to_string(3 * i + 1), (int)dw.s[1], dbn));
            const float* db = nullptr;
            if (has("backbone.deconv_layers." + std::to_string(3 * i) + ".bias")) PL_TRY(get_vec("backbone.deconv_layers." + std::to_string(3 * i) + ".bias", (int)dw.s[1], &db));
            LT_REQUIRE(dw.s[2] == 4 && dw.s[3] == 4, LT_ERR_UNSUPPORTED, "%s: only the 4x4 stride-2 deconvolution of the reference configs", who);
            ConvOpt o; o.bias = db; o.bn = &dbn; o.stride = 2; o.pad = 1; o.transposed = true; o.relu = true;
            Act z; PL_TRY(conv(y, dw, o, z)); release(y);
            y = z;
        }
        feats256 = y;
        heatmaps = Act();
        if (want_heatmaps) {
            WT fw; const float* fb;
            PL_TRY(get("backbone.final_layer.weight", fw, 4)); PL_TRY(get_vec("backbone.final_layer.bias", (int)fw.s[0], &fb));
            ConvOpt o; o.bias = fb; o.pad = fw.s[2] == 3 ? 1 : 0; o.out_f32 = true;
            PL_TRY(conv(y, fw, o, heatmaps));
        }
        return LT_OK;
    }

    struct C3 { WT w; const float* b = nullptr; BN bn; bool has_bn = false; };
    int load_c3(const std::string& conv, const std::string& bnname, bool transposed, C3& c) {
        PL_TRY(get(conv + ".weight", c.w, 5));
        const int cout = (int)(transposed ? c.w.s[1] : c.w.s[0]);
        PL_TRY(get_vec(conv + ".bias", cout, &c.b));
        if (!bnname.empty()) { PL_TRY(get_bn(bnname, cout, c.bn)); c.has_bn = true; }
        return LT_OK;
    }
    int res3d(const std::string& pre, const Act& x, Act& out) {
        C3 c0, c3, sk;
        PL_TRY(load_c3(pre + ".res_branch.0", pre + ".res_branch.1", false, c0));
        PL_TRY(load_c3(pre + ".res_branch.3", pre + ".res_branch.4", false, c3));
        const bool has_skip = has(pre + ".skip_con.0.weight");
        if (has_skip) PL_TRY(load_c3(pre + ".skip_con.0", pre + ".skip_con.1", false, sk));
        const int mid[5] = {x.n, x.d, x.h, x.w, (int)c0.w.s[0]};
        Act y, z;
        const lt_wshape w3 = wshape(c3.w), wsk = has_skip ? wshape(sk.w) : lt_wshape{};
        if (has_skip && lt_sel_conv_skip(dtype, mid, &w3, dims(x).data(), &wsk)) {
            ConvOpt o; o.bias = c0.b; o.bn = &c0.bn; o.pad = 1; o.relu = true; PL_TRY(conv(x, c0.w, o, y));
            o = ConvOpt(); o.bias = c3.b; o.bn = &c3.bn; o.pad = 1; o.relu = true; o.skip_x = &x; o.skip_w = &sk.w; o.skip_bias = sk.b; o.skip_bn = &sk.bn;
            PL_TRY(conv(y, c3.w, o, z)); release(y);
            out = z;
            return LT_OK;
        }
        Act skip = x; bool own = false;
        if (has_skip) { ConvOpt o; o.bias = sk.b; o.bn = &sk.bn; PL_TRY(conv(x, sk.w, o, skip)); own = true; }
        ConvOpt o; o.bias = c0.b; o.bn = &c0.bn; o.pad = 1; o.relu = true; PL_TRY(conv(x, c0.w, o, y));
        o = ConvOpt(); o.bias = c3.b; o.bn = &c3.bn; o.pad = 1; o.relu = true; o.residual = &skip; PL_TRY(conv(y, c3.w, o, z));
        release(y);
        if (own) release(skip);
        out = z;
        return LT_OK;
    }
    int record_v2v(const Act& vol_in, Act& logits_out) {
        const std::string V = "volume_net.";
        Act x = vol_in, y;
        {
            C3 c; PL_TRY(load_c3(V + "front_layers.0.block.0", V + "front_layers.0.block.1", false, c));
            ConvOpt o; o.bias = c.b; o.bn = &c.bn; o.pad = (int)(c.w.s[2] - 1) / 2; o.relu = true;
            PL_TRY(conv(x, c.w, o, y)); release(x); x = y;
            for (int i = 1; i <= 3; ++i) { PL_TRY(res3d(V + "front_layers." + std::to_string(i), x, y)); release(x); x = y; }
        }
        {
            const std::string E = V + "encoder_decoder.";
            Act skips[5];
            for (int lvl = 1; lvl <= 5; ++lvl) {
                PL_TRY(res3d(E + "skip_res" + std::to_string(lvl), x, skips[lvl - 1]));
                Act p; PL_TRY(maxpool(x, 2, 2, 0, 3, p)); release(x);
                PL_TRY(res3d(E + "encoder_res" + std::to_string(lvl), p, x)); release(p);
            }
            PL_TRY(res3d(E + "mid_res", x, y)); release(x); x = y;
            for (int lvl = 5; lvl >= 1; --lvl) {
                PL_TRY(res3d(E + "decoder_res" + std::to_string(lvl), x, y)); release(x);
                C3 u; PL_TRY(load_c3(E + "decoder_upsample" + std::to_string(lvl) + ".block.0", E + "decoder_upsample" + std::to_string(lvl) + ".block.1", true, u));
                ConvOpt o; o.bias = u.b; o.bn = &u.bn; o.stride = 2; o.pad = 0; o.transposed = true; o.relu_pre = true; o.residual = &skips[lvl - 1];
                PL_TRY(conv(y, u.w, o, x));
                release(y); release(skips[lvl - 1]);
            }
        }
        PL_TRY(res3d(V + "back_layers.0", x, y)); release(x); x = y;
        C3 t1, t2, ol;
        PL_TRY(load_c3(V + "back_layers.1.block.0", V + "back_layers.1.block.1", false, t1));
        PL_TRY(load_c3(V + "back_layers.2.block.0", V + "back_layers.2.block.1", false, t2));
        PL_TRY(load_c3(V + "output_layer", "", false, ol));
        std::vector<PwLayer> chain = {{t1.w, t1.b, &t1.bn, true}, {t2.w, t2.b, &t2.bn, true}, {ol.w, ol.b, nullptr, false}};
        const lt_wshape wchain[3] = {wshape(t1.w), wshape(t2.w), wshape(ol.w)};
        if (lt_sel_pwchain(dtype, dims(x).data(), 3, wchain)) {
            PL_TRY(pwchain(x, chain, logits_out)); release(x);
            return LT_OK;
        }
        for (C3* c : {&t1, &t2}) { ConvOpt o; o.bias = c->b; o.bn = &c->bn; o.relu = true; PL_TRY(conv(x, c->w, o, y)); release(x); x = y; }
        ConvOpt o; o.bias = ol.b; o.out_f32 = true;
        PL_TRY(conv(x, ol.w, o, logits_out)); release(x);
        return LT_OK;
    }

    int build() {
        const int B = cfg.B, NV = cfg.NV, V = cfg.volume_size, J = cfg.num_joints;
        Act f256, no_hm;
        const bool conf_head = cfg.aggregation == LT_AGG_CONF || cfg.aggregation == LT_AGG_CONF_NORM;
        PL_TRY(record_backbone(B * NV, cfg.H, cfg.W, cfg.num_layers, cfg.style_caffe != 0, conf_head ? "backbone.vol_confidences" : nullptr, false, f256, volc, no_hm));
        WT pw; const float* pb;
        PL_TRY(get("process_features.0.weight", pw, 4)); PL_TRY(get_vec("process_features.0.bias", (int)pw.s[0], &pb));
        LT_REQUIRE(pw.s[0] == 32, LT_ERR_UNSUPPORTED, "lt_plan_create_vol: process_features has %d output channels (32)", (int)pw.s[0]);
        ConvOpt o; o.bias = pb;
        PL_TRY(conv(f256, pw, o, feats)); release(f256);
        feats.pooled = false;
        hm_h = feats.h; hm_w = feats.w;
        n_geo = (size_t)B * NV * 12 + (size_t)B * 15; o_pos = (size_t)B * NV * 12; o_cen = o_pos + 3 * B; o_rot = o_pos + 6 * B;
        void* g; PL_TRY(dev_alloc(n_geo * 4, &g)); geo_dev = (float*)g;
        for (int i = 0; i < GEO_RING; ++i) { PL_HIP(hipHostMalloc((void**)&geo_host[i], n_geo * 4, hipHostMallocDefault)); }
        void* c; PL_TRY(dev_alloc((size_t)B * V * V * V * 3 * 4, &c)); coords = (float*)c;
        PL_TRY(alloc(B, V, V, V, 32, es, vol));
        const float step = (float)(cfg.cuboid_side / (double)(V - 1));
        {
            const int dt = dtype, agg = cfg.aggregation, cmu = cfg.transfer_cmu_to_human36m ? 1 : 0, h = hm_h, w = hm_w;
            const float* gp = geo_dev; const size_t op = o_pos, oc = o_cen, orr = o_rot;
            const void* fp = feats.p; float* cp = coords; void* vp = vol.p; const float* confp = volc.null() ? nullptr : (const float*)volc.p;
            ops.push_back([=](hipStream_t s) { return lt_unproject_grid_fwd(dt, fp, gp, gp + op, gp + oc, gp + orr, step, cmu, cp, confp, vp, B, NV, 32, h, w, V, agg, s); });
        }
        PL_TRY(record_v2v(vol, logits));
        void* k; PL_TRY(dev_alloc((size_t)B * J * 3 * 4, &k)); kp = (float*)k;
        PL_TRY(dev_alloc((size_t)B * J * V * V * V * 4, &k)); probs = (float*)k;
        const long long nvox = (long long)V * V * V;
        const size_t wsb = lt_softargmax3d_workspace(B, J, nvox);
        PL_TRY(dev_alloc(wsb ? wsb : 16, &sa_ws));
        {
            const int dt = dtype, h = hm_h, w = hm_w; const void* fp = feats.p; lt_plan* self = this;
            ops.push_back([=](hipStream_t s) { return self->out_feats ? lt_nhwc_to_nchw_f32(dt, fp, self->out_feats, B * NV, 32, h * w, 32, s) : LT_OK; });
        }
        {
            const float mult = (float)cfg.volume_multiplier; const int sm = cfg.volume_softmax ? 1 : 0, cl = logits.planar ? 0 : 1;
            const float* lp = (const float*)logits.p; const float* cp = coords; void* ws = sa_ws; lt_plan* self = this;
            float* kpd = kp; float* prd = probs;
            ops.push_back([=](hipStream_t s) {
                return lt_softargmax3d_fwd(lp, cp, mult, sm, cl, J, self->out_kp ? self->out_kp : kpd, self->out_probs ? self->out_probs : prd, B, J, nvox, ws, s);
            });
        }
        ntail = 2;
        return LT_OK;
    }

    int build_alg() {
        const lt_alg_plan_config& c = acfg;
        const int B = c.B, NV = c.NV, N = B * NV, J = c.num_joints, Hh = c.H, W = c.W;
        const bool ransac = c.model == LT_MODEL_RANSAC;
        Act f256, hm;
        PL_TRY(record_backbone(N, Hh, W, c.num_layers, c.style_caffe != 0, !ransac && c.use_confidences ? "backbone.alg_confidences" : nullptr, true, f256, algc, hm));
        release(f256);
        LT_REQUIRE(hm.c == J, LT_ERR_INVALID, "%s: backbone.final_layer has %d output channels, num_joints is %d", who, hm.c, J);
        hm_h = hm.h; hm_w = hm.w;
        const int h = hm_h, w = hm_w;
        void* q;
        PL_TRY(dev_alloc((size_t)N * J * h * w * 4, &q)); hm_nchw = (float*)q;
        const float* hp = (const float*)hm.p; float* hn = hm_nchw; lt_plan* self = this;
        if (ransac) {
            PL_TRY(dev_alloc((size_t)N * J * 2 * 8, &q)); kp_i64 = (int64_t*)q;
            const int ld = hm.c; int64_t* kpp = kp_i64;
            ops.push_back([=](hipStream_t s) { return lt_heatmap_argmax_nchw_f32(hp, ld, hn, nullptr, kpp, N, J, h, w, Hh, W, s); });
            const double eps = c.reprojection_error_epsilon; const int direct = c.direct_optimization ? 1 : 0;
            ops.push_back([=](hipStream_t s) { return lt_triangulate_ransac(self->cur_proj, kpp, nullptr, 0, eps, direct, self->out_kp, nullptr, B, NV, J, s); });
            ntail = 1;
            return LT_OK;
        }
        ops.push_back([=](hipStream_t s) { return lt_nhwc_to_nchw_f32(LT_F32, hp, hn, N, J, h * w, J, s); });
        PL_TRY(dev_alloc((size_t)N * J * 2 * 4, &q)); kp_hm = (float*)q;
        PL_TRY(dev_alloc((size_t)N * J * h * w * 4, &q)); probs = (float*)q;
        {
            const float mult = (float)c.heatmap_multiplier; const int sm = c.heatmap_softmax ? 1 : 0; float* kh = kp_hm; float* pr = probs;
            ops.push_back([=](hipStream_t s) { return lt_softargmax2d_fwd(hn, mult, sm, kh, self->out_hm ? self->out_hm : pr, N * J, h, w, s); });
        }
        {
            const float sx = (float)((double)W / (double)w), sy = (float)((double)Hh / (double)h);
            const float* kh = kp_hm; const float* cp = algc.null() ? nullptr : (const float*)algc.p; const int ldc = algc.null() ? J : algc.c;
            ops.push_back([=](hipStream_t s) {
                return lt_alg_tail_fwd(kh, cp, ldc, self->cur_proj, sx, sy, (float*)self->out_kp2d, self->out_conf, self->out_kp, B, NV, J, s);
            });
        }
        ntail = 2;
        return LT_OK;
    }

    int enter(hipStream_t& st, bool& detour) {
        detour = st == nullptr && cfg.use_graph;
        if (!detour) return LT_OK;
        if (!own_stream) {
            PL_HIP(hipStreamCreateWithFlags(&own_stream, hipStreamNonBlocking));
            for (int i = 0; i < 2; ++i) PL_HIP(hipEventCreateWithFlags(&own_ev[i], hipEventDisableTiming));
        }
// ... 208 lines not shown
    }
    PL_TRY(p->leave(st, detour));
    return LT_OK;
}

extern "C" int lt_plan_create_cascade(const lt_cascade_plan_config* cfg, const lt_named_tensor* alg_weights, int32_t n_alg, const lt_named_tensor* vol_weights,
                                      int32_t n_vol, lt_plan** plan_out) {
    const char* who = "lt_plan_create_cascade";
    LT_REQUIRE(cfg && alg_weights && vol_weights && plan_out && n_alg > 0 && n_vol > 0, LT_ERR_INVALID, "%s: null argument", who);
    const lt_alg_plan_config& a = cfg->alg; const lt_vol_plan_config& v = cfg->vol;
    PL_TRY(check_alg_config(a, who));
    LT_REQUIRE(a.model == LT_MODEL_ALG, LT_ERR_INVALID, "%s: alg.model %d (the pelvis comes from LT_MODEL_ALG; LT_MODEL_RANSAC is not a stage of the cascade)", who, a.model);
    PL_TRY(check_vol_config(&v, who));
    LT_REQUIRE(v.B == a.B && v.NV == a.NV && v.H == a.H && v.W == a.W, LT_ERR_INVALID,
               "%s: vol.B %d, vol.NV %d, vol.H %d, vol.W %d differ from alg.B %d, alg.NV %d, alg.H %d, alg.W %d (both stages read the same images)", who, v.B, v.NV, v.H,
               v.W, a.B, a.NV, a.H, a.W);
    LT_REQUIRE(cfg->kind == LT_KIND_MPII || cfg->kind == LT_KIND_COCO, LT_ERR_INVALID, "%s: kind %d (LT_KIND_MPII | LT_KIND_COCO)", who, cfg->kind);
    const int need = cfg->kind == LT_KIND_COCO ? 13 : 7;
    LT_REQUIRE(a.num_joints >= need, LT_ERR_INVALID, "%s: alg.num_joints %d, kind '%s' reads joint %d", who, a.num_joints, cfg->kind == LT_KIND_COCO ? "coco" : "mpii", need - 1);
    PL_TRY(check_alg_heads(a, alg_weights, n_alg, who));
    *plan_out = nullptr;
    lt_plan* p = new lt_plan();
    p->who = who; p->model = MODEL_CASCADE; p->kind = cfg->kind;
    p->cfg = v; p->acfg = a;
    p->cfg.use_graph = (a.use_graph || v.use_graph) ? 1 : 0;
    p->dtype = v.dtype; p->es = v.dtype == LT_F32 ? 4 : 2;
    int rc = make_alg_plan(a, alg_weights, n_alg, who, &p->sub_alg);
    if (rc == LT_OK) rc = make_vol_plan(&v, vol_weights, n_vol, who, &p->sub_vol);
    auto finish = [&]() -> int {
        const size_t nproj = (size_t)a.B * a.NV * 12 * 4;
        void* q;
        PL_TRY(p->dev_alloc(nproj, &q)); p->cproj_dev = (float*)q;
        PL_TRY(p->dev_alloc((size_t)a.B * a.num_joints * 3 * 4, &q)); p->ckp_alg = (float*)q;
        for (int i = 0; i < GEO_RING; ++i) PL_HIP(hipHostMalloc((void**)&p->cproj_host[i], nproj, hipHostMallocDefault));
        return LT_OK;
    };
    if (rc == LT_OK) rc = finish();
    if (rc != LT_OK) { delete p; return rc; }
    *plan_out = p;
    return LT_OK;
}

extern "C" int lt_plan_forward_cascade(lt_plan* p, const float* images, const double* K_host, const double* R_host, const double* t_host, const double* rot_host,
                                       float* keypoints_3d, float* alg_keypoints_3d, float* base_points, float* volumes, float* features, float* coord_volumes,
                                       float* vol_confidences, void* stream) {
    LT_REQUIRE(p, LT_ERR_INVALID, "lt_plan_forward_cascade: null argument");
    LT_REQUIRE(p->model == MODEL_CASCADE, LT_ERR_INVALID, "lt_plan_forward_cascade: the plan is %s; run it with %s", plan_kind_name(p),
               p->model == 0 ? "lt_plan_forward_vol" : "lt_plan_forward_alg");
    LT_REQUIRE(images && K_host && R_host && t_host && keypoints_3d, LT_ERR_INVALID, "lt_plan_forward_cascade: null argument (images, K, R, t and keypoints_3d are required)");
    lt_plan* A = p->sub_alg; lt_plan* Vp = p->sub_vol;
    LT_REQUIRE(!vol_confidences || !Vp->volc.null(), LT_ERR_INVALID,
               "lt_plan_forward_cascade: vol_confidences asked of a plan without the confidence head (aggregation %d)", Vp->cfg.aggregation);
    hipStream_t st = (hipStream_t)stream;
    bool detour;
    PL_TRY(p->enter(st, detour));
    const int B = Vp->cfg.B, NV = Vp->cfg.NV, V = Vp->cfg.volume_size;
    PL_TRY(Vp->stage_geometry(K_host, R_host, t_host, nullptr, rot_host, st, p->cproj_host));
    PL_HIP(hipMemcpyAsync(p->cproj_dev, p->cproj_host[Vp->geo_slot], (size_t)B * NV * 12 * 4, hipMemcpyHostToDevice, st));
    PL_HIP(hipEventRecord(Vp->geo_ev[Vp->geo_slot], st));
    float* kp_alg = alg_keypoints_3d ? alg_keypoints_3d : p->ckp_alg;
    A->cur_images = images; A->cur_proj = p->cproj_dev; A->out_kp = kp_alg; A->out_kp2d = nullptr; A->out_hm = nullptr; A->out_conf = nullptr;
    PL_TRY(A->run(st));
    PL_TRY(lt_cuboid_from_keypoints(kp_alg, B, p->acfg.num_joints, p->kind, Vp->cfg.cuboid_side, Vp->geo_dev + Vp->o_pos, Vp->geo_dev + Vp->o_cen, st));
    if (base_points) PL_HIP(hipMemcpyAsync(base_points, Vp->geo_dev + Vp->o_cen, (size_t)B * 3 * 4, hipMemcpyDeviceToDevice, st));
    Vp->cur_images = images; Vp->out_kp = keypoints_3d; Vp->out_probs = volumes; Vp->out_feats = features;
    PL_TRY(Vp->run(st));
    if (coord_volumes) PL_HIP(hipMemcpyAsync(coord_volumes, Vp->coords, (size_t)B * V * V * V * 3 * 4, hipMemcpyDeviceToDevice, st));
    if (vol_confidences) PL_HIP(hipMemcpyAsync(vol_confidences, Vp->volc.p, (size_t)B * NV * 32 * 4, hipMemcpyDeviceToDevice, st));
    PL_TRY(p->leave(st, detour));
    return LT_OK;
}

extern "C" int lt_plan_info(const lt_plan* p, lt_plan_info_t* info) {
    LT_REQUIRE(p && info, LT_ERR_INVALID, "lt_plan_info: null argument");
    memset(info, 0, sizeof(*info));
    if (p->model == MODEL_CASCADE) {
        lt_plan_info_t a;
        PL_TRY(lt_plan_info(p->sub_vol, info));
        PL_TRY(lt_plan_info(p->sub_alg, &a));
        info->launches += a.launches + 1;
        info->flops += a.flops; info->bytes_allocated += a.bytes_allocated + (int64_t)p->bytes_alloc;
        info->n_expand_reduce += a.n_expand_reduce; info->n_bottleneck += a.n_bottleneck; info->n_bottleneck_ds += a.n_bottleneck_ds; info->n_conv_cat2 += a.n_conv_cat2;
        info->n_conv2d_halo += a.n_conv2d_halo; info->n_pwchain += a.n_pwchain; info->n_stem_pool += a.n_stem_pool; info->n_splitk += a.n_splitk;
        info->n_conv_skip += a.n_conv_skip;
        info->graph_captured = (!p->sub_alg->cfg.use_graph || a.graph_captured) && (!p->sub_vol->cfg.use_graph || info->graph_captured) &&
                               (p->sub_alg->cfg.use_graph || p->sub_vol->cfg.use_graph) ? 1 : 0;
        return LT_OK;
    }
    info->launches = (int32_t)p->ops.size();
    info->heatmap_h = p->hm_h; info->heatmap_w = p->hm_w;
    info->flops = p->flops; info->bytes_allocated = (int64_t)p->bytes_alloc;
    info->n_expand_reduce = p->n_xr; info->n_bottleneck = p->n_bneck; info->n_bottleneck_ds = p->n_bneck_ds; info->n_conv_cat2 = p->n_cat2;
    info->n_conv2d_halo = p->n_halo2d; info->n_pwchain = p->n_pwchain; info->n_stem_pool = p->n_stem; info->n_splitk = p->n_splitk; info->n_conv_skip = p->n_conv_skip;
    info->graph_captured = p->captured ? 1 : 0;
    info->logits = (const float*)p->logits.p; info->logits_planar = p->logits.planar ? 1 : 0;
    return LT_OK;
}

extern "C" void lt_plan_destroy(lt_plan* p) { delete p; }
```

learnable-triangulation-pytorch_amd/csrc/select.hip:

```cpp
#include "conv_common.h"

using namespace lt;

namespace {

bool wshape_is(const lt_wshape* w, int nd, int64_t s0, int64_t s1, int64_t s2, int64_t s3, int64_t s4 = 0) {
    const int64_t s[5] = {s0, s1, s2, s3, s4};
    if (w->nd != nd) return false;
    for (int i = 0; i < nd; ++i)
        if (w->s[i] != s[i]) return false;
    return true;
}

bool pointwise(const lt_wshape* w) {
    for (int i = 2; i < w->nd; ++i)
        if (w->s[i] != 1) return false;
    return true;
}

}

extern "C" int lt_sel_conv_skip(int32_t dtype, const int32_t x[5], const lt_wshape* w, const int32_t skip_x[5], const lt_wshape* skip_w) {
    if (dtype != LT_BF16 || env_on("LT_NO_CONV_SKIP") || env_on("LT_HALO_NO_COL") || env_on("LT_HALO_NO_PERSIST") || env_on("LT_CONV_NO_HALO")) return 0;
    if (!wshape_is(w, 5, 32, 32, 3, 3, 3) || !wshape_is(skip_w, 5, 32, 16, 1, 1, 1)) return 0;
    const int N = x[0], D = x[1], H = x[2], W = x[3];
    if (x[4] != 32 || skip_x[0] != N || skip_x[1] != D || skip_x[2] != H || skip_x[3] != W || skip_x[4] != 16) return 0;
    const int nc = lt_conv_chunk_samples(N, (long long)D * H * W * 32);
    if (nc < 1) return 0;
    return halo_col_fits(nc, D, H, W) && halo_col_fits(N - (N - 1) / nc * nc, D, H, W);
}

extern "C" int lt_sel_conv_cat2(int32_t dtype, const int32_t t2[5], const lt_wshape* we, const int32_t x[5], const lt_wshape* wd, int32_t s) {
    if (dtype != LT_BF16 || env_on("LT_NO_CONV_CAT2") || env_on("LT_CONV_NO_V7") || env_on("LT_CONV_NO_V3")) return 0;
    const int N = t2[0], Ho = t2[2], Wo = t2[3], P = t2[4];
    if (t2[1] != 1 || we->nd != 4 || wd->nd != 4 || !pointwise(we) || !pointwise(wd)) return 0;
    const long long Cc = we->s[0], Cin2 = wd->s[1];
    if (we->s[1] != P || wd->s[0] != Cc || (s != 1 && s != 2) || x[0] != N || x[1] != 1 || x[2] != Ho * s || x[3] != Wo * s || x[4] != Cin2) return 0;
    if (P % 32 || Cin2 % 32 || (P + Cin2) % 64 || Cc % 256 || (P & (P - 1))) return 0;
    const long long tiles = (((long long)N * Ho * Wo + 287) / 288) * (Cc / 256);
    if (tiles < 200 && !env_on("LT_CAT2_ANY_SIZE")) return 0;
    return (long long)N * Ho * Wo * Cc < (1ll << 31) && (long long)N * x[2] * x[3] * Cin2 < (1ll << 31);
}

extern "C" int lt_sel_splitk_slices(const lt_conv_desc* d, const lt_wshape* w, int32_t transposed) {
    if (d->dtype != LT_BF16 || transposed || (d->flags & (LT_EPI_STORE_F32 | LT_EPI_SIGMOID)) || env_on("LT_CONV_NO_SPLITK")) return 1;
    if (w->nd != 5 || w->s[2] != 3 || w->s[3] != 3 || w->s[4] != 3) return 1;
    for (int i = 0; i < 3; ++i)
        if (d->stride[i] != 1 || d->pad[i] != 1) return 1;
    if (d->Cin < 128 || d->Cin % 64 || d->Cout % 4 || d->Cout != d->cout_pad || d->D * d->H * d->W > 512) return 1;
    const long long rows = (long long)d->N * d->Do * d->Ho * d->Wo;
    const int bm = rows >= 8192 ? 128 : 64;
    const long long tiles = ((rows + bm - 1) / bm) * (d->cout_pad / bm);
    const long long S = 256 / tiles;
    return S > 8 ? 8 : S < 1 ? 1 : (int)S;
}

extern "C" int lt_sel_bottleneck(int32_t dtype, const int32_t x[5], const lt_wshape w[3], const int32_t strides[3]) {
    if (dtype != LT_BF16 || env_on("LT_NO_BNECK")) return 0;
    if (x[1] != 1 || strides[0] != 1 || strides[1] != 1 || strides[2] != 1) return 0;
    const int C = x[4];
    const int64_t P = w[0].s[0];
    if (!((C == 256 && P == 64) || (C == 512 && P == 128))) return 0;
    if (!wshape_is(&w[0], 4, P, C, 1, 1) || !wshape_is(&w[1], 4, P, P, 3, 3) || !wshape_is(&w[2], 4, C, P, 1, 1)) return 0;
    return x[2] % 8 == 0 && x[3] % 16 == 0 && (long long)x[0] * x[2] * x[3] * C < (1ll << 31);
}

extern "C" int lt_sel_bottleneck_ds(int32_t dtype, const int32_t x[5], const lt_wshape w[3], const int32_t strides[3], const lt_wshape* wd, int32_t sd) {
    if (dtype != LT_BF16 || env_on("LT_NO_BNECK") || env_on("LT_NO_BNECK_DS")) return 0;
    if (x[1] != 1 || strides[0] != 1 || strides[1] != 1 || strides[2] != 1 || sd != 1) return 0;
    if (x[4] != 64 || !wshape_is(&w[0], 4, 64, 64, 1, 1) || !wshape_is(&w[1], 4, 64, 64, 3, 3) || !wshape_is(&w[2], 4, 256, 64, 1, 1) ||
        !wshape_is(wd, 4, 256, 64, 1, 1))
        return 0;
    return x[2] % 8 == 0 && x[3] % 16 == 0 && (long long)x[0] * x[2] * x[3] * 256 < (1ll << 31);
}

extern "C" int lt_sel_expand_reduce(int32_t dtype, const int32_t t2[5], const int32_t res[5], const lt_wshape* we, const lt_wshape* wr) {
    if (dtype != LT_BF16 || env_on("LT_NO_XR")) return 0;
    if (t2[1] != 1 || res[1] != 1 || t2[0] != res[0] || t2[2] != res[2] || t2[3] != res[3] || res[4] != 1024 || t2[4] != 256) return 0;
    if ((long long)t2[0] * t2[2] * t2[3] < 36 * 96 && !env_on("LT_XR_ANY_SIZE")) return 0;
    return wshape_is(we, 4, 1024, 256, 1, 1) && wshape_is(wr, 4, 256, 1024, 1, 1);
}

extern "C" int lt_sel_stem_pool(int32_t dtype, const int32_t x[5], const lt_wshape* w, int32_t stride, int32_t pad, const int32_t pool[3]) {
    return dtype == LT_BF16 && x[1] == 1 && x[4] == 8 && w->nd == 4 && w->s[2] == 7 && w->s[3] == 7 && w->s[0] == 64 && w->s[1] <= 8 && stride == 2 &&
           pad == 3 && pool[0] == 3 && pool[1] == 2 && pool[2] == 1;
}

extern "C" int lt_sel_pwchain(int32_t dtype, const int32_t x[5], int32_t nlayers, const lt_wshape* w) {
    if (dtype != LT_BF16 || nlayers < 1 || nlayers > LT_PWCHAIN_MAX || x[4] != 32) return 0;
    if ((long long)x[0] * x[1] * x[2] * x[3] % 64) return 0;
    int64_t cin = 32;
    for (int i = 0; i < nlayers; ++i) {
        if (!pointwise(&w[i]) || w[i].s[1] != cin || w[i].s[0] > 32 || (i + 1 < nlayers && w[i].s[0] != 32)) return 0;
        cin = w[i].s[0];
    }
    return 1;
}

extern "C" int lt_sel_frag_layout(const lt_conv_desc* d, const lt_wshape* w, int32_t transposed, int32_t has_residual) {
    if (d->dtype != LT_BF16) return 0;
    const bool w3x3 = !transposed && wshape_is(w, 4, 256, 256, 3, 3) && d->W == 24;
    const bool w4x4t = transposed && wshape_is(w, 4, 256, 256, 4, 4) && !env_on("LT_DECONV_NO_H2D");
    if ((w3x3 || w4x4t) && d->tile == LT_TILE_AUTO && !has_residual && !env_on("LT_CONV_NO_H2D") && !env_on("LT_CONV_V1") &&
        ((long long)d->N * (d->H / 8) * (d->W / 24) >= 60 || env_on("LT_H2D_ANY_SIZE")) && halo2d_fits(conv_args_of(*d), d->cout_pad, d->nphase))
        return 2;
    if (d->cout_pad % 256 == 0 && d->k_pad % 64 == 0) {
        const bool short_pw = pointwise(w) && d->k_pad <= 256 && !transposed;
        return !env_on("LT_CONV_NO_V7") && !short_pw ? 3 : 1;
    }
    const bool wreg = wshape_is(w, 5, 64, 64, 3, 3, 3) || wshape_is(w, 5, 64, 32, 3, 3, 3) || wshape_is(w, 5, 128, 128, 3, 3, 3) || wshape_is(w, 5, 32, 16, 3, 3, 3);
    if (transposed || !wreg || d->Cin != w->s[1]) return 0;
    for (int i = 0; i < 3; ++i)
// ... 4 lines not shown
```

learnable-triangulation-pytorch_amd/lt_engine.py:

```python
import ctypes as C
from collections import OrderedDict
from dataclasses import dataclass, field
from typing import List, Optional, Tuple

import numpy as np
import torch
import torch.nn as nn

import lt_hip as H

BN_EPS = 1e-5


def cout_pad_of(cout):
    if cout <= 16:
        return 16
    if cout <= 32:
        return 32
    if cout <= 64:
        return 64
    return (cout + 127) // 128 * 128


def conv_chunk_samples(N, per_sample):
# ... 98 lines not shown
        k_pad = (K + kstep - 1) // kstep * kstep
        wk = w.permute(0, 2, 3, 4, 1).reshape(cout, K)
        taps = [(a, b, c, ((a * Hh + b) * W + c) * cin_buf) for a in range(kd) for b in range(kh) for c in range(kw)]
        bi, sc, sh = fold_bn(cout, bias, bn, cp)
        spec = ConvSpec(N, D, Hh, W, cin_buf, Do, Ho, Wo, st, pd, Do, Ho, Wo, (1, 1, 1), cout, cp, k_pad, flags, bi, sc, sh)
        spec.phases.append(ConvPhaseSpec(_pad_k(wk, cp, k_pad), torch.tensor(taps, dtype=torch.int32).reshape(-1, 4), (0, 0, 0)))
        return spec
    cin, cout, kd, kh, kw = w.shape
    assert cin == cin_buf, "transposed conv input may not be channel padded"
    nd3 = weight.dim() == 5
    assert all(s == 2 for s in (st if nd3 else st[1:])), "only stride-2 transposed convolutions"
    ks = (kd, kh, kw)
    dims = (D, Hh, W)
    outs = []
    for i in range(3):
        if not nd3 and i == 0:
            outs.append(1)
        else:
            o = (dims[i] - 1) * 2 - 2 * pd[i] + ks[i] + output_padding
            assert o == 2 * dims[i], "transposed conv must exactly double the size (k=4,p=1 / k=2,p=0; with output_padding=1: k=3,p=1 / k=1,p=0 -- the input gradients of the stride-2 convolutions)"
            outs.append(o)
    cp = cout_pad_of(cout)

    def dim_phases(i):
        if not nd3 and i == 0:
            return [(0, [(0, 0)])]
        res = []
        for phi in (0, 1):
            res.append((phi, [(kk, (phi + pd[i] - kk) // 2) for kk in range(ks[i]) if (phi + pd[i] - kk) % 2 == 0]))
        return res

    phase_list = []
    ntaps_max = 0
    for pa, ta in dim_phases(0):
        for pb, tb in dim_phases(1):
            for pc, tc in dim_phases(2):
                taps, cols = [], []
                for (ka, da) in ta:
                    for (kb, db) in tb:
                        for (kc, dc) in tc:
                            taps.append((da, db, dc, ((da * Hh + db) * W + dc) * cin))
                            cols.append(w[:, :, ka, kb, kc].t())
                if not taps:
                    taps, cols = [(0, 0, 0, 0)], [torch.zeros(cout, cin)]
                wk = torch.cat(cols, dim=1)
                phase_list.append((wk, taps, (pa, pb, pc)))
                ntaps_max = max(ntaps_max, len(taps))
    K = ntaps_max * cin
    k_pad = (K + kstep - 1) // kstep * kstep
    bi, sc, sh = fold_bn(cout, bias, bn, cp)
    ostr = (2 if nd3 else 1, 2, 2)
    spec = ConvSpec(N, D, Hh, W, cin, D, Hh, W, (1, 1, 1), (0, 0, 0), outs[0], outs[1], outs[2], ostr, cout, cp, k_pad, flags, bi, sc, sh)
    for wk, taps, off in phase_list:
        spec.phases.append(ConvPhaseSpec(_pad_k(wk, cp, k_pad), torch.tensor(taps, dtype=torch.int32).reshape(-1, 4), off))
    assert len(spec.phases) <= H.MAX_PHASES
    return spec


def stage_images(x, act, stream):
    N, Cc, Hh, W = x.shape
    H.check(H.lib().lt_nchw_to_nhwc(H.dtype_code(act.t.dtype), x.data_ptr(), act.t.data_ptr(), N, Cc, Hh * W, act.t.shape[-1], stream), "lt_nchw_to_nhwc")


class Act:
    __slots__ = ("t", "pooled")

    def __init__(self, t):
        self.t = t
        self.pooled = True

    @property
    def shape(self):
        return tuple(self.t.shape)


class Recorder:

    dtype = torch.float32
    live_weights = False

    def _declines(self, *a, **k):
        return False

    can_conv_skip = can_conv_cat2 = can_chain_pointwise = can_bottleneck = can_bottleneck_ds = can_expand_reduce = can_stem_pool = _declines


class PlanBuilder(Recorder):

    def __init__(self, device, dtype, tile_override=0, dry_run=False, stages=0):
        self.device = torch.device(device)
        self.dry_run = dry_run
        if self.device.type != "cuda" and not dry_run:
            raise RuntimeError("liblt_hip plans run on the GPU only (device=%s); there is no CPU fallback" % device)
        self.lib = None if dry_run else H.lib()
        self.dtype = dtype
        self.code = H.dtype_code(dtype)
        self.out_dtype = torch.bfloat16 if dtype == torch.float8_e4m3fn else dtype
        self.ops = []
        self.keep = []
        self.pool = {}
        self.tile_override = tile_override
        self.stages = stages
        self.live_weights = False
        self.live_frag = False
        self.flops = 0
        self.bytes_alloc = 0
        self.ntail = 0
        self.npre = 0

    def alloc(self, shape, dtype=None):
        dtype = dtype or self.dtype
        n = int(np.prod(shape)) * esize(dtype)
        lst = self.pool.get((n, dtype))
        if lst:
            t = lst.pop().view(*shape)
        else:
            t = torch.empty(shape, dtype=dtype, device=self.device)
            self.bytes_alloc += n
        self.keep.append(t)
        return Act(t)

    def release(self, act):
        if act is None or not act.pooled:
            return
        t = act.t
        n = t.numel() * t.element_size()
        self.pool.setdefault((n, t.dtype), []).append(t.reshape(-1))

    def const(self, t, dtype=None):
        t = t.to(device=self.device, dtype=dtype or t.dtype).contiguous()
        self.keep.append(t)
        return t

    def _add(self, fn, kind="op", label="", flops=0, nbytes=0, info=None):
        meta = {"kind": kind, "label": label, "flops": flops, "bytes": nbytes}
        if self.dry_run:
            meta["info"] = info or {}
        self.last_info = info or {}
        self.ops.append((fn, meta))

    def _fusable(self):
        return not (self.live_weights or self.tile_override)

    def can_conv_skip(self, x_shape, weight, skip_shape, skip_weight):
        if not self._fusable():
            return False
        return bool(H.lib().lt_sel_conv_skip(self.code, H.dims(x_shape), H.wshape(weight), H.dims(skip_shape), H.wshape(skip_weight)))

    def _desc(self, spec):
        d = H.ConvDesc()
        d.dtype = self.code
        d.N, d.D, d.H, d.W, d.Cin = spec.N, spec.D, spec.H, spec.W, spec.Cin
        d.Do, d.Ho, d.Wo = spec.Do, spec.Ho, spec.Wo
        d.stride = H.i3(spec.stride); d.pad = H.i3(spec.pad)
        d.OD, d.OH, d.OW = spec.OD, spec.OH, spec.OW
        d.out_stride = H.i3(spec.out_stride)
        d.Cout, d.ldc, d.cout_pad, d.k_pad = spec.Cout, spec.Cout, spec.cout_pad, spec.k_pad
        d.nphase, d.flags, d.tile, d.stages = len(spec.phases), spec.flags, self.tile_override, self.stages
        for i, ph in enumerate(spec.phases):
            d.phase[i].ntaps = ph.taps.shape[0]; d.phase[i].out_off = H.i3(ph.out_off)
        return d

    def frag_layout(self, spec, weight, transposed, residual):
        if self.live_weights and not self.live_frag:
            return 0
        return H.lib().lt_sel_frag_layout(self._desc(spec), H.wshape(weight), int(transposed), int(residual))

    @staticmethod
    def _frag_packer(layout, spec, ntaps):
        if layout == 2:
            return lambda sp, dp, a=(spec.cout_pad, spec.k_pad, spec.Cin, ntaps): H.check(
                H.lib().lt_conv_pack_weights_t32(sp, *a, dp, H.cur_stream()), "lt_conv_pack_weights_t32")
        name = "lt_conv_pack_weights32" if layout == 3 else "lt_conv_pack_weights"
        return lambda sp, dp, a=(spec.cout_pad, spec.k_pad): H.check(getattr(H.lib(), name)(sp, *a, dp, H.cur_stream()), name)

    def _frag_copy(self, wdev, layout, spec, ntaps):
        wfr = torch.empty_like(wdev)
        pack = self._frag_packer(layout, spec, ntaps)
        if not self.dry_run:
            pack(wdev.data_ptr(), wfr.data_ptr())
        self.keep.append(wfr)
        return wfr, pack

    def _pack_layer(self, weight, bn, in_shape, pad, flags):
        spec = make_conv_spec(weight, None, bn, in_shape, 1, pad, self.dtype, False, flags)
        ph = spec.phases[0]
        ntaps = int(ph.taps.shape[0])
        assert spec.cout_pad == spec.Cout and spec.k_pad == ntaps * spec.Cin, (spec.cout_pad, spec.k_pad)
        wdev = self.const(ph.weight, self.dtype)
        sc, sh = self.const(spec.scale), self.const(spec.shift)
        wfr, _ = self._frag_copy(wdev, 2, spec, ntaps)
        self.flops += 2 * spec.N * spec.Ho * spec.Wo * spec.Cout * ntaps * spec.Cin
        return spec, wfr.data_ptr(), sc.data_ptr(), sh.data_ptr()

    def conv(self, x, weight, bias=None, bn=None, stride=1, pad=0, transposed=False, relu=False, relu_pre=False,
             residual=None, out_f32=False, out=None, sigmoid=False, output_padding=0, residual_f32=False, skip=None):
        flags = ((H.EPI_RELU_POST if relu else 0) | (H.EPI_RELU_PRE if relu_pre else 0) | (H.EPI_STORE_F32 if out_f32 else 0)
                 | (H.EPI_SIGMOID if sigmoid else 0) | (H.EPI_RES_F32 if residual_f32 else 0))
        assert not residual_f32 or (out_f32 and residual is not None and self.dtype in (torch.bfloat16, torch.float8_e4m3fn))
        spec = make_conv_spec(weight, bias, bn, x.shape, stride, pad, self.dtype, transposed, flags, output_padding)
        skip_info = None
        if skip is not None:
            sx, sw, sb, sbn = skip
            assert residual is None and not relu_pre and not out_f32 and out is None and self.can_conv_skip(x.shape, weight, sx.shape, sw)
            ss = make_conv_spec(sw, sb, sbn, sx.shape, 1, 0, self.dtype, False, 0)
            assert ss.cout_pad == spec.cout_pad == 32
            wfold = (ss.phases[0].weight * ss.scale[:, None]).to(self.dtype)
            spec.shift = spec.shift + ss.bias * ss.scale + ss.shift
            wfr, _ = self._frag_copy(self.const(wfold, self.dtype), 2, ss, 1)
            sk = H.ConvSkip()
            sk.x, sk.cin, sk.weight_frag = sx.t.data_ptr(), 16, wfr.data_ptr()
            self.keep += [sx.t, sk]
            skip_info = {"x": sx, "w": wfold[:, :16].float(), "desc": sk}
        S = self.splitk_slices(spec, weight, transposed, out_f32, sigmoid, out)
        if S > 1:
            return self._conv_splitk(x, weight, spec, S, residual)
        y = out or self.alloc((spec.N, spec.OD, spec.OH, spec.OW, spec.Cout), torch.float32 if out_f32 else self.out_dtype)
        self.keep.append(x.t)
        if residual is not None:
            self.keep.append(residual.t)
        if residual is not None:
            assert residual.shape == y.shape and residual.t.dtype == (torch.float32 if residual_f32 else self.out_dtype), (residual.shape, y.shape)
        d = self._desc(spec)
        layout = self.frag_layout(spec, weight, transposed, residual is not None)
        wdevs, wfrags = [], []
        for i, ph in enumerate(spec.phases):
            wdev = self.const(ph.weight, self.dtype)
            wdevs.append(wdev)
            tdev = self.const(ph.taps)
            d.phase[i].weight = wdev.data_ptr(); d.phase[i].taps = tdev.data_ptr()
            if layout and not self.dry_run:
                wfr, pack = self._frag_copy(wdev, layout, spec, int(ph.taps.shape[0]))
                wfrags.append((i, wfr, pack))
                d.phase[i].weight_frag, d.phase[i].weight_frag_layout = wfr.data_ptr(), layout
        bi, sc, sh = self.const(spec.bias), self.const(spec.scale), self.const(spec.shift)
        self.keep.append(d)
        macs = spec.N * spec.Do * spec.Ho * spec.Wo * spec.Cout * sum(int(p.taps.shape[0]) for p in spec.phases) * (
            weight.shape[1] if not transposed else weight.shape[0])
        self.flops += 2 * macs
        ksz = "x".join(str(k) for k in weight.shape[2:])
        label = "%s%s %d->%d @%s" % ("deconv" if transposed else "conv", ksz, spec.Cin, spec.Cout,
                                     "x".join(str(v) for v in (spec.N, spec.Do, spec.Ho, spec.Wo)))
        esz = esize(self.dtype)
        nbytes = (x.t.numel() + y.t.numel() + (residual.t.numel() if residual is not None else 0)) * esz + \
            sum(p.weight.numel() for p in spec.phases) * esz
        info = {"spec": spec, "x": x, "y": y, "res": residual, "wdev": wdevs, "bias_dev": bi, "scale_dev": sc, "shift_dev": sh, "desc": d, "wfrag": wfrags}
        if skip_info is not None:
            macs += spec.N * spec.Do * spec.Ho * spec.Wo * spec.Cout * 16
            self.flops += 2 * spec.N * spec.Do * spec.Ho * spec.Wo * spec.Cout * 16
            nbytes += skip_info["x"].t.numel() * esz
            info["skip"] = skip_info
            self._add(lambda s, d=d, xp=x.t.data_ptr(), bip=bi.data_ptr(), scp=sc.data_ptr(), shp=sh.data_ptr(), sk=skip_info["desc"], yp=y.t.data_ptr():
                      H.check(self.lib.lt_conv_skip_fwd(C.byref(d), xp, bip, scp, shp, C.byref(sk), yp, s), "lt_conv_skip_fwd"),
                      "conv", label + " + skip conv1x1x1 16->32", 2 * macs, nbytes, info)
            return y
        self._add(lambda s, d=d, xp=x.t.data_ptr(), bip=bi.data_ptr(), scp=sc.data_ptr(), shp=sh.data_ptr(),
                  rp=H.ptr(residual.t) if residual is not None else None, yp=y.t.data_ptr():
                  H.check(self.lib.lt_conv_fwd(C.byref(d), xp, bip, scp, shp, rp, yp, s), "lt_conv_fwd"),
                  "conv", label, 2 * macs, nbytes, info)
        return y

    def can_conv_cat2(self, t2_shape, w_expand, x_shape, w_down, stride_down):
        if not self._fusable():
            return False
        return bool(H.lib().lt_sel_conv_cat2(self.code, H.dims(t2_shape), H.wshape(w_expand), H.dims(x_shape), H.wshape(w_down), stride_down))

    def conv_cat2(self, t2, w_expand, bn_expand, x, w_down, bn_down, stride_down):
        assert self.can_conv_cat2(t2.shape, w_expand, x.shape, w_down, stride_down)
        N, _, Ho, Wo, P = t2.shape
        Cc, Cin2 = w_expand.shape[0], w_down.shape[1]
        s3 = make_conv_spec(w_expand, None, bn_expand, t2.shape, 1, 0, self.dtype, False, H.EPI_RELU_POST)
        sd = make_conv_spec(w_down, None, bn_down, x.shape, stride_down, 0, self.dtype, False, 0)
        assert s3.cout_pad == sd.cout_pad == Cc and (s3.Do, s3.Ho, s3.Wo) == (sd.Do, sd.Ho, sd.Wo) == (1, Ho, Wo)
        wcat = torch.cat([s3.phases[0].weight[:, :P] * s3.scale[:, None], sd.phases[0].weight[:, :Cin2] * sd.scale[:, None]], dim=1).to(self.dtype)
        shift = (s3.bias * s3.scale + s3.shift) + (sd.bias * sd.scale + sd.shift)
        kp = P + Cin2
        spec = ConvSpec(N, 1, Ho, Wo, kp, 1, Ho, Wo, (1, 1, 1), (0, 0, 0), 1, Ho, Wo, (1, 1, 1), Cc, Cc, kp, H.EPI_RELU_POST,
                        torch.zeros(Cc), torch.ones(Cc), shift)
        spec.phases.append(ConvPhaseSpec(wcat.float(), s3.phases[0].taps, (0, 0, 0)))
        y = self.alloc((N, 1, Ho, Wo, Cc))
        self.keep += [t2.t, x.t]
        d = self._desc(spec)
        d.Cin, d.tile, d.stages = P, 0, 0
        wdev = self.const(wcat, self.dtype)
        tdev = self.const(s3.phases[0].taps)
        wfr, _ = self._frag_copy(wdev, 3, spec, 1)
        d.phase[0].weight, d.phase[0].taps = wdev.data_ptr(), tdev.data_ptr()
        d.phase[0].weight_frag, d.phase[0].weight_frag_layout = wfr.data_ptr(), 3
        c2 = H.ConvCat2()
        c2.x, c2.cin, c2.H, c2.W, c2.stride = x.t.data_ptr(), Cin2, x.shape[2], x.shape[3], stride_down
        bi, sh = self.const(spec.bias), self.const(spec.shift)
        self.keep += [d, c2]
        macs = N * Ho * Wo * Cc * kp
        self.flops += 2 * macs
        esz = t2.t.element_size()
        nbytes = (t2.t.numel() + N * Ho * Wo * Cin2 + y.t.numel() + wcat.numel()) * esz
        label = "conv1x1 %d+%d->%d @%s (expand + stride-%d downsample)" % (P, Cin2, Cc, "x".join(str(v) for v in (N, 1, Ho, Wo)), stride_down)
        self._add(lambda s, d=d, xp=t2.t.data_ptr(), c2=c2, bip=bi.data_ptr(), shp=sh.data_ptr(), yp=y.t.data_ptr():
                  H.check(self.lib.lt_conv_cat2_fwd(C.byref(d), xp, C.byref(c2), bip, None, shp, None, yp, s), "lt_conv_cat2_fwd"),
                  "conv", label, 2 * macs, nbytes, {"cat2": True, "spec": spec, "x": t2, "x2": x, "stride2": stride_down, "y": y})
        return y

    def splitk_slices(self, spec, weight, transposed, out_f32, sigmoid, out):
        if not self._fusable() or out is not None:
            return 1
        d = self._desc(spec)
        d.flags |= (H.EPI_STORE_F32 if out_f32 else 0) | (H.EPI_SIGMOID if sigmoid else 0)
        return H.lib().lt_sel_splitk_slices(d, H.wshape(weight), int(transposed))

    def _conv_splitk(self, x, weight, spec, S, residual):
        ph0 = spec.phases[0]
        ntaps, Cin = ph0.taps.shape[0], spec.Cin
        bounds = [ntaps * i // S for i in range(S + 1)]
        kstep = k_step_of(self.dtype)
        kp = (max(bounds[i + 1] - bounds[i] for i in range(S)) * Cin + kstep - 1) // kstep * kstep
        ident = (torch.zeros(spec.cout_pad), torch.ones(spec.cout_pad), torch.zeros(spec.cout_pad))
        pspec = ConvSpec(spec.N, spec.D, spec.H, spec.W, Cin, spec.Do, spec.Ho, spec.Wo, spec.stride, spec.pad, S * spec.Do, spec.Ho, spec.Wo, (1, 1, 1),
                         spec.Cout, spec.cout_pad, kp, H.EPI_STORE_F32, *ident)
        for i in range(S):
            t0, t1 = bounds[i], bounds[i + 1]
            pspec.phases.append(ConvPhaseSpec(_pad_k(ph0.weight[:, t0 * Cin:t1 * Cin], spec.cout_pad, kp), ph0.taps[t0:t1].contiguous(), (i * spec.Do, 0, 0)))
        part = self.alloc((spec.N, S * spec.Do, spec.Ho, spec.Wo, spec.Cout), torch.float32)
        y = self.alloc((spec.N, spec.Do, spec.Ho, spec.Wo, spec.Cout))
        self.keep.append(x.t)
        if residual is not None:
            assert residual.shape == y.shape and residual.t.dtype == self.dtype, (residual.shape, y.shape)
            self.keep.append(residual.t)
        rows = spec.N * spec.Do * spec.Ho * spec.Wo
        d = self._desc(pspec)
        d.tile = H.TILE2_128x128 if rows >= 8192 else H.TILE2_64x64
        wdevs = []
        for i, ph in enumerate(pspec.phases):
            wdev, tdev = self.const(ph.weight, self.dtype), self.const(ph.taps)
            wdevs.append(wdev)
            d.phase[i].weight = wdev.data_ptr(); d.phase[i].taps = tdev.data_ptr()
        ibi, isc, ish = (self.const(t) for t in ident)
        bi, sc, sh = self.const(spec.bias), self.const(spec.scale), self.const(spec.shift)
# ... 307 lines not shown
```

learnable-triangulation-pytorch_amd/lt_hip.py:

```python
import ctypes as C
import os

import torch

HERE = os.path.dirname(os.path.abspath(__file__))
LIB_PATH = os.environ.get("LT_HIP_LIB") or os.path.join(HERE, "lib", "liblt_hip.so")

LT_F32, LT_BF16, LT_FP8 = 0, 1, 2
AGG = {"sum": 0, "max": 1, "softmax": 2, "conf": 3, "conf_norm": 4}
LT_MODEL_ALG, LT_MODEL_RANSAC = 1, 2
LT_KIND_MPII, LT_KIND_COCO = 0, 1
KIND = {"mpii": LT_KIND_MPII, "coco": LT_KIND_COCO}
EPI_RELU_PRE, EPI_RELU_POST, EPI_STORE_F32, EPI_SIGMOID = 1, 2, 4, 8
EPI_RES_F32 = 64
BN_FROZEN = 32
BN_Y_BF16 = 128
ACT_BF16 = 256
TILE_AUTO, TILE_128x128, TILE_128x64, TILE_256x32, TILE_256x16, TILE_64x64, TILE_DIRECT = 0, 1, 2, 3, 4, 5, 99
TILE2_128x128, TILE2_128x64, TILE2_256x32, TILE2_256x16, TILE2_64x64 = 11, 12, 13, 14, 15
TILE_HALO = 20
TILE3_288 = 30
MAX_PHASES = 8

vp, i32, i64, f32 = C.c_void_p, C.c_int32, C.c_int64, C.c_float


class ConvPhase(C.Structure):
    _fields_ = [("weight", vp), ("taps", vp), ("ntaps", i32), ("out_off", i32 * 3), ("weight_frag", vp), ("weight_frag_layout", i32)]


class ConvDesc(C.Structure):
    _fields_ = [("dtype", i32), ("N", i32), ("D", i32), ("H", i32), ("W", i32), ("Cin", i32),
                ("Do", i32), ("Ho", i32), ("Wo", i32), ("stride", i32 * 3), ("pad", i32 * 3),
                ("OD", i32), ("OH", i32), ("OW", i32), ("out_stride", i32 * 3),
                ("Cout", i32), ("ldc", i32), ("cout_pad", i32), ("k_pad", i32),
                ("nphase", i32), ("flags", i32), ("tile", i32), ("stages", i32),
                ("phase", ConvPhase * MAX_PHASES)]


class ConvSkip(C.Structure):
    _fields_ = [("x", vp), ("cin", i32), ("weight_frag", vp)]


class ConvCat2(C.Structure):
    _fields_ = [("x", vp), ("cin", i32), ("H", i32), ("W", i32), ("stride", i32)]


class WShape(C.Structure):
    _fields_ = [("nd", i32), ("s", i64 * 5)]


def wshape(t):
    return WShape(t.dim(), (i64 * 5)(*t.shape))


def dims(shape):
    return (i32 * 5)(*shape)


PWCHAIN_MAX = 3


class PwChainDesc(C.Structure):
    _fields_ = [("dtype", i32), ("nlayers", i32), ("rows", i64), ("cin", i32), ("ldy", i32),
                ("cout", i32 * PWCHAIN_MAX), ("k_pad", i32 * PWCHAIN_MAX), ("flags", i32 * PWCHAIN_MAX),
                ("weight", vp * PWCHAIN_MAX), ("bias", vp * PWCHAIN_MAX), ("scale", vp * PWCHAIN_MAX), ("shift", vp * PWCHAIN_MAX),
                ("plane", i64)]


class StemDesc(C.Structure):
    _fields_ = [("dtype", i32), ("N", i32), ("H", i32), ("W", i32), ("Cin", i32), ("Cout", i32),
                ("weight", vp), ("bias", vp), ("scale", vp), ("shift", vp), ("x_layout", i32)]


class BneckDesc(C.Structure):
    _fields_ = [("dtype", i32), ("N", i32), ("H", i32), ("W", i32), ("C", i32), ("P", i32),
                ("weight", vp * 3), ("bias", vp * 3), ("scale", vp * 3), ("shift", vp * 3)]


class BneckDsDesc(C.Structure):
    _fields_ = [("dtype", i32), ("N", i32), ("H", i32), ("W", i32), ("Cin", i32), ("P", i32), ("C", i32),
                ("weight", vp * 4), ("scale", vp * 4), ("shift", vp * 4)]


class XrDesc(C.Structure):
    _fields_ = [("dtype", i32), ("C", i32), ("P", i32), ("M", C.c_int64), ("weight", vp * 2), ("scale", vp * 2), ("shift", vp * 2), ("consts", vp)]


class NamedTensor(C.Structure):
    _fields_ = [("name", C.c_char_p), ("data", vp), ("ndim", i32), ("shape", C.c_int64 * 5)]


class VolPlanConfig(C.Structure):
    _fields_ = [("dtype", i32), ("num_layers", i32), ("style_caffe", i32), ("num_joints", i32), ("B", i32), ("NV", i32), ("H", i32), ("W", i32),
                ("volume_size", i32), ("cuboid_side", C.c_double), ("volume_multiplier", C.c_double), ("volume_softmax", i32), ("aggregation", i32),
                ("transfer_cmu_to_human36m", i32), ("use_graph", i32)]


class AlgPlanConfig(C.Structure):
    _fields_ = [("model", i32), ("dtype", i32), ("num_layers", i32), ("style_caffe", i32), ("num_joints", i32), ("B", i32), ("NV", i32), ("H", i32),
                ("W", i32), ("use_confidences", i32), ("heatmap_softmax", i32), ("heatmap_multiplier", C.c_double), ("direct_optimization", i32),
                ("reprojection_error_epsilon", C.c_double), ("use_graph", i32)]


class CascadePlanConfig(C.Structure):
    _fields_ = [("alg", AlgPlanConfig), ("vol", VolPlanConfig), ("kind", i32)]


class PlanInfo(C.Structure):
    _fields_ = [("launches", i32), ("heatmap_h", i32), ("heatmap_w", i32), ("flops", C.c_double), ("bytes_allocated", C.c_int64),
                ("n_expand_reduce", i32), ("n_bottleneck", i32), ("n_bottleneck_ds", i32), ("n_conv_cat2", i32), ("n_conv2d_halo", i32), ("n_pwchain", i32),
                ("n_stem_pool", i32), ("n_splitk", i32), ("n_conv_skip", i32), ("graph_captured", i32), ("logits", vp), ("logits_planar", i32)]


SIGNATURES = {
    "lt_plan_create_vol": (C.c_int, [C.POINTER(VolPlanConfig), C.POINTER(NamedTensor), i32, C.POINTER(vp)]),
    "lt_plan_forward_vol": (C.c_int, [vp, vp, vp, vp, vp, vp, vp, vp, vp, vp, vp, vp, vp]),
    "lt_plan_create_alg": (C.c_int, [C.POINTER(AlgPlanConfig), C.POINTER(NamedTensor), i32, C.POINTER(vp)]),
    "lt_plan_forward_alg": (C.c_int, [vp, vp, vp, vp, vp, vp, vp, vp]),
    "lt_plan_create_cascade": (C.c_int, [C.POINTER(CascadePlanConfig), C.POINTER(NamedTensor), i32, C.POINTER(NamedTensor), i32, C.POINTER(vp)]),
    "lt_plan_forward_cascade": (C.c_int, [vp, vp, vp, vp, vp, vp, vp, vp, vp, vp, vp, vp, vp, vp]),
    "lt_plan_info": (C.c_int, [vp, C.POINTER(PlanInfo)]),
    "lt_plan_destroy": (None, [vp]),
    "lt_last_error": (C.c_char_p, []),
    "lt_abi_version": (C.c_int, []),
    "lt_device_info": (C.c_int, [C.POINTER(C.c_int), C.POINTER(C.c_int), C.c_char_p, C.c_int]),
    "lt_conv_fwd": (C.c_int, [C.POINTER(ConvDesc), vp, vp, vp, vp, vp, vp, vp]),
    "lt_conv_skip_fwd": (C.c_int, [C.POINTER(ConvDesc), vp, vp, vp, vp, C.POINTER(ConvSkip), vp, vp]),
    "lt_conv_cat2_fwd": (C.c_int, [C.POINTER(ConvDesc), vp, C.POINTER(ConvCat2), vp, vp, vp, vp, vp, vp]),
    "lt_conv_cout_pad": (C.c_int, [i32]),
    "lt_conv_chunk_samples": (i32, [i32, i64]),
    "lt_sel_conv_skip": (C.c_int, [i32, i32 * 5, C.POINTER(WShape), i32 * 5, C.POINTER(WShape)]),
    "lt_sel_conv_cat2": (C.c_int, [i32, i32 * 5, C.POINTER(WShape), i32 * 5, C.POINTER(WShape), i32]),
    "lt_sel_splitk_slices": (C.c_int, [C.POINTER(ConvDesc), C.POINTER(WShape), i32]),
    "lt_sel_bottleneck": (C.c_int, [i32, i32 * 5, WShape * 3, i32 * 3]),
    "lt_sel_bottleneck_ds": (C.c_int, [i32, i32 * 5, WShape * 3, i32 * 3, C.POINTER(WShape), i32]),
    "lt_sel_expand_reduce": (C.c_int, [i32, i32 * 5, i32 * 5, C.POINTER(WShape), C.POINTER(WShape)]),
    "lt_sel_stem_pool": (C.c_int, [i32, i32 * 5, C.POINTER(WShape), i32, i32, i32 * 3]),
    "lt_sel_pwchain": (C.c_int, [i32, i32 * 5, i32, C.POINTER(WShape)]),
    "lt_sel_frag_layout": (C.c_int, [C.POINTER(ConvDesc), C.POINTER(WShape), i32, i32]),
    "lt_conv_pack_weights": (C.c_int, [vp, i32, i32, vp, vp]),
    "lt_conv_pack_weights_t32": (C.c_int, [vp, i32, i32, i32, i32, vp, vp]),
    "lt_conv_pack_weights32": (C.c_int, [vp, i32, i32, vp, vp]),
    "lt_pwchain_fwd": (C.c_int, [C.POINTER(PwChainDesc), vp, vp, vp]),
    "lt_stem_pool_fwd": (C.c_int, [C.POINTER(StemDesc), vp, vp, vp]),
    "lt_bottleneck_fwd": (C.c_int, [C.POINTER(BneckDesc), vp, vp, vp]),
    "lt_bottleneck_ds_fwd": (C.c_int, [C.POINTER(BneckDsDesc), vp, vp, vp]),
    "lt_expand_reduce_fwd": (C.c_int, [C.POINTER(XrDesc), vp, vp, vp, vp, vp]),
    "lt_stem_packed_bytes": (C.c_size_t, []),
    "lt_stem_pack_weights": (C.c_int, [vp, i32, vp, vp]),
    "lt_maxpool_fwd": (C.c_int, [i32, vp, vp, i32, i32, i32, i32, i32, i32 * 3, i32 * 3, i32 * 3, vp]),
    "lt_global_avgpool": (C.c_int, [i32, vp, vp, i32, i32, i32, vp]),
    "lt_nchw_to_nhwc": (C.c_int, [i32, vp, vp, i32, i32, i32, i32, vp]),
    "lt_nhwc_to_nchw_f32": (C.c_int, [i32, vp, vp, i32, i32, i32, i32, vp]),
    "lt_coord_volumes": (C.c_int, [vp, vp, vp, f32, i32, i32, i32, vp, vp]),
    "lt_rotate_points": (C.c_int, [vp, vp, vp, i64, vp]),
    "lt_unproject_fwd": (C.c_int, [i32, vp, vp, vp, vp, vp, i32, i32, i32, i32, i32, i32, i32, i32, i32, vp]),
    "lt_unproject_grid_fwd": (C.c_int, [i32, vp, vp, vp, vp, vp, f32, i32, vp, vp, vp, i32, i32, i32, i32, i32, i32, i32, vp]),
    "lt_cuboid_from_keypoints": (C.c_int, [vp, i32, i32, i32, C.c_double, vp, vp, vp]),
    "lt_softargmax3d_workspace": (C.c_size_t, [i32, i32, i64]),
    "lt_softargmax3d_fwd": (C.c_int, [vp, vp, f32, i32, i32, i32, vp, vp, i32, i32, i64, vp, vp]),
    "lt_softargmax2d_fwd": (C.c_int, [vp, f32, i32, vp, vp, i32, i32, i32, vp]),
    "lt_triangulate_dlt": (C.c_int, [vp, vp, vp, vp, i32, i32, i32, vp]),
    "lt_alg_tail_fwd": (C.c_int, [vp, vp, i32, vp, f32, f32, vp, vp, vp, i32, i32, i32, vp]),
    "lt_heatmap_argmax_nchw_f32": (C.c_int, [vp, i32, vp, vp, vp, i32, i32, i32, i32, i32, i32, vp]),
    "lt_triangulate_ransac": (C.c_int, [vp, vp, vp, i32, C.c_double, i32, vp, vp, i32, i32, i32, vp]),
    "lt_crop_resize_u8": (C.c_int, [vp, i64, vp, vp, i32, i32, i32, vp, vp, vp]),
    "lt_undistort_crop_resize_u8": (C.c_int, [vp, i64, vp, vp, vp, i64, i32, i32, i32, vp, vp, vp]),
    "lt_bn_act_fwd": (C.c_int, [vp, vp, vp, vp, vp, vp, vp, vp, i64, i32, f32, i32, vp]),
    "lt_bn_act_bwd_workspace": (C.c_size_t, [i64, i32]),
    "lt_bn_act_bwd": (C.c_int, [vp, vp, vp, vp, vp, vp, vp, vp, vp, vp, vp, vp, i32, i64, i32, f32, i32, vp, vp]),
    "lt_act_bwd": (C.c_int, [vp, vp, vp, vp, vp, i32, i64, i32, vp]),
    "lt_channel_sum_workspace": (C.c_size_t, [i64, i32]),
    "lt_channel_sum": (C.c_int, [vp, i64, i32, vp, i32, vp, vp]),
    "lt_channel_sum_dt": (C.c_int, [i32, vp, i64, i32, vp, i32, vp, vp]),
    "lt_maxpool_bwd_dt": (C.c_int, [i32, vp, vp, vp, i32, i32, i32, i32, i32, i32 * 3, i32 * 3, i32 * 3, vp]),
    "lt_convert_pad": (C.c_int, [i32, vp, i32, vp, i64, i32, i32, vp]),
    "lt_maxpool_bwd": (C.c_int, [vp, vp, vp, i32, i32, i32, i32, i32, i32 * 3, i32 * 3, i32 * 3, vp]),
    "lt_adam_step_multi": (C.c_int, [vp, i32, i32, f32, f32, f32, f32, i32, vp]),
    "lt_add_f32": (C.c_int, [vp, vp, i64, vp]),
    "lt_pad_channels_f32": (C.c_int, [vp, vp, i64, i32, i32, vp]),
    "lt_zero": (C.c_int, [vp, i64, vp]),
    "lt_softargmax2d_bwd": (C.c_int, [vp, vp, vp, C.c_float, i32, vp, i32, i32, i32, vp]),
    "lt_triangulate_dlt_bwd": (C.c_int, [vp, vp, vp, vp, vp, vp, i32, i32, i32, vp]),
    "lt_splitk_reduce": (C.c_int, [i32, vp, i32, i64, i64, i32, vp, vp, vp, vp, vp, i32, vp]),
    "lt_add_i64_multi": (C.c_int, [vp, i32, i64, vp]),
    "lt_cast_f32_bf16": (C.c_int, [vp, vp, i64, vp]),
    "lt_gather_f32_multi": (C.c_int, [vp, i32, i32, vp]),
    "lt_amax_f32": (C.c_int, [vp, i64, vp, vp]),
    "lt_amax_dt": (C.c_int, [i32, vp, i64, vp, vp]),
    "lt_quant_fp8_dt": (C.c_int, [i32, vp, vp, i64, vp, vp, vp]),
    "lt_quant_fp8": (C.c_int, [vp, vp, i64, vp, vp, vp]),
    "lt_gather_f32_fp8": (C.c_int, [vp, vp, vp, i64, vp, vp, vp]),
    "lt_scale_product": (C.c_int, [vp, i32, vp, vp, vp]),
    "lt_gather_f32": (C.c_int, [vp, vp, vp, i64, vp]),
    "lt_gather_f32_bf16": (C.c_int, [vp, vp, vp, i64, vp]),
    "lt_conv_wgrad_workspace": (C.c_size_t, [i64, i32, i32]),
    "lt_pack_n8_bf16_bytes": (C.c_size_t, [i32, i64, i32]),
    "lt_pack_n8_bf16": (C.c_int, [vp, vp, i32, i64, i32, i32, vp]),
    "lt_pack_n8_from_bf16": (C.c_int, [vp, vp, i32, i64, i32, i32, vp]),
    "lt_conv_wgrad_bf16_workspace": (C.c_size_t, [i64, i32, i32]),
    "lt_conv_wgrad_bf16": (C.c_int, [vp, vp, vp, vp, i32, i32, i32, i32, i32, i32, i32, i32, i32 * 3, i32 * 3, i32, i32, i32, i32, i32, i32, vp, vp]),
    "lt_conv_wgrad_bf16_nhwc_ok": (C.c_int, [i32, i32, i32, i32, i32, i32, i32, i32, i32, i32 * 3, i32 * 3, i32, i32, i32, i32, i32]),
    "lt_conv_wgrad_bf16_nhwc": (C.c_int, [vp, vp, vp, vp, i32, i32, i32, i32, i32, i32, i32, i32, i32, i32 * 3, i32 * 3, i32, i32, i32, i32, i32, i32, vp, vp]),
    "lt_conv_wgrad": (C.c_int, [vp, vp, vp, vp, i32, i32, i32, i32, i32, i32, i32, i32, i32 * 3, i32 * 3, i32, i32, i32, i32, i32, i32, vp, vp]),
    "lt_adam_step": (C.c_int, [vp, vp, vp, vp, i64, f32, f32, f32, f32, f32, i32, vp]),
    "lt_unproject_bwd_workspace": (C.c_size_t, [i32, i32, i32, i32, i32, i32]),
    "lt_unproject_bwd": (C.c_int, [i32, vp, vp, vp, vp, vp, vp, vp, i32, i32, i32, i32, i32, i32, i32, i32, i32, vp, C.c_size_t, vp]),
    "lt_global_avgpool_bwd": (C.c_int, [vp, vp, i32, i32, i32, i32, vp]),
    "lt_global_avgpool_bwd_dt": (C.c_int, [i32, vp, vp, i32, i32, i32, i32, vp]),
    "lt_softargmax3d_bwd": (C.c_int, [vp, vp, vp, vp, vp, vp, f32, i32, i32, vp, i32, i32, i64, vp]),
    "lt_softargmax3d_bwd_dense": (C.c_int, [vp, vp, vp, vp, vp, vp, vp, vp, f32, i32, i32, vp, i32, i32, i64, vp]),
    "lt_volumetric_ce_fwd": (C.c_int, [vp, vp, vp, vp, vp, vp, vp, i32, i32, i64, vp]),
    "lt_bn_stats_workspace": (C.c_size_t, [i64, i32]),
    "lt_bn_stats_fwd": (C.c_int, [i32, vp, i64, i32, vp, vp, vp, vp, f32, vp, vp]),
# ... 118 lines not shown
```

learnable-triangulation-pytorch_amd/mvn/models/pose_resnet.py:

```python
import torch
import torch.nn as nn

import lt_engine as E
import lt_hip as H

BN_MOMENTUM = 0.1

resnet_spec = {18: ("basic", [2, 2, 2, 2]), 34: ("basic", [3, 4, 6, 3]), 50: ("bottleneck", [3, 4, 6, 3]),
               101: ("bottleneck", [3, 4, 23, 3]), 152: ("bottleneck", [3, 8, 36, 3])}


def _bn(c):
    return nn.BatchNorm2d(c, momentum=BN_MOMENTUM)


def bn_tuple(bn):
    return E.BnParams(bn)


class ResidualBlock(nn.Module):

    def __init__(self, kind, inplanes, planes, stride=1, downsample=None, caffe=False):
        super().__init__()
        self.kind, self.stride = kind, stride
# ... 46 lines not shown
                b.release(t1)
                y = b.conv_cat2(t2, self.conv3.weight, bn_tuple(self.bn3), x, ds.weight, bn_tuple(self.downsample[1]), sds)
                b.release(t2)
                return y
        res = x
        if self.downsample is not None:
            res = b.conv(x, self.downsample[0].weight, None, bn_tuple(self.downsample[1]), stride=self.downsample[0].stride[0], pad=0)
        y = x
        for i in range(1, n + 1):
            conv, bn = getattr(self, "conv%d" % i), getattr(self, "bn%d" % i)
            last = i == n
            z = b.conv(y, conv.weight, None, bn_tuple(bn), stride=conv.stride[0], pad=conv.padding[0], relu=True,
                       residual=res if last else None)
            if y is not x:
                b.release(y)
            y = z
        if res is not x:
            b.release(res)
        return y


class GlobalAveragePoolingHead(nn.Module):

    def __init__(self, in_channels, n_classes):
        super().__init__()
        self.features = nn.Sequential(
            nn.Conv2d(in_channels, 512, 3, stride=1, padding=1), _bn(512), nn.MaxPool2d(2), nn.ReLU(inplace=True),
            nn.Conv2d(512, 256, 3, stride=1, padding=1), _bn(256), nn.MaxPool2d(2), nn.ReLU(inplace=True))
        self.head = nn.Sequential(nn.Linear(256, 512), nn.ReLU(inplace=True), nn.Linear(512, 256), nn.ReLU(inplace=True),
                                  nn.Linear(256, n_classes), nn.Sigmoid())

    def record(self, b, x):
        f = self.features
        y = b.conv(x, f[0].weight, f[0].bias, bn_tuple(f[1]), stride=1, pad=1, relu=True)
        p = b.maxpool(y, 2, 2, 0, nd=2); b.release(y)
        y = b.conv(p, f[4].weight, f[4].bias, bn_tuple(f[5]), stride=1, pad=1, relu=True); b.release(p)
        p = b.maxpool(y, 2, 2, 0, nd=2); b.release(y)
        g = b.global_avgpool(p); b.release(p)
        h = self.head
        y = b.conv(g, h[0].weight[:, :, None, None], h[0].bias, None, relu=True); b.release(g)
        z = b.conv(y, h[2].weight[:, :, None, None], h[2].bias, None, relu=True); b.release(y)
        o = b.conv(z, h[4].weight[:, :, None, None], h[4].bias, None, sigmoid=True, out_f32=True); b.release(z)
        return o


class PoseResNet(E.PlanCache):
    def __init__(self, block_kind, layers, num_joints, num_input_channels=3, deconv_with_bias=False, num_deconv_layers=3,
                 num_deconv_filters=(256, 256, 256), num_deconv_kernels=(4, 4, 4), final_conv_kernel=1,
                 alg_confidences=False, vol_confidences=False, caffe=False):
        super().__init__()
        assert all(k == 4 for k in num_deconv_kernels), "only the 4x4 stride-2 deconvolution of the reference configs"
        self.num_joints, self.num_input_channels = num_joints, num_input_channels
        self.block_kind, self.caffe = block_kind, caffe
        exp = 4 if block_kind == "bottleneck" else 1
        self.conv1 = nn.Conv2d(num_input_channels, 64, kernel_size=7, stride=2, padding=3, bias=False)
        self.bn1 = _bn(64)
        inplanes = 64
        for li, (planes, nb) in enumerate(zip((64, 128, 256, 512), layers), 1):
            stride = 1 if li == 1 else 2
            blocks = []
            for bi in range(nb):
                st = stride if bi == 0 else 1
                ds = None
                if bi == 0 and (st != 1 or inplanes != planes * exp):
                    ds = nn.Sequential(nn.Conv2d(inplanes, planes * exp, kernel_size=1, stride=st, bias=False), _bn(planes * exp))
                blocks.append(ResidualBlock(block_kind, inplanes, planes, st, ds, caffe))
                inplanes = planes * exp
            setattr(self, "layer%d" % li, nn.Sequential(*blocks))
        if alg_confidences:
            self.alg_confidences = GlobalAveragePoolingHead(inplanes, num_joints)
        if vol_confidences:
            self.vol_confidences = GlobalAveragePoolingHead(inplanes, 32)
        dl = []
        for i in range(num_deconv_layers):
            dl += [nn.ConvTranspose2d(inplanes, num_deconv_filters[i], kernel_size=4, stride=2, padding=1, output_padding=0,
                                      bias=deconv_with_bias), _bn(num_deconv_filters[i]), nn.ReLU(inplace=True)]
            inplanes = num_deconv_filters[i]
        self.deconv_layers = nn.Sequential(*dl)
        self.final_layer = nn.Conv2d(inplanes, num_joints, kernel_size=final_conv_kernel, stride=1,
                                     padding=1 if final_conv_kernel == 3 else 0)
        self.compute_dtype = torch.float32
        self._init_plan_cache()

    def record(self, b, x, want_heatmaps=True, image_cell=None):
        if b.can_stem_pool(x, self.conv1.weight, 2, 3, (3, 2, 1)):
            y = b.stem_pool(x, self.conv1.weight, bn_tuple(self.bn1), image_cell=image_cell)
        else:
            y = b.conv(x, self.conv1.weight, None, bn_tuple(self.bn1), stride=2, pad=3, relu=True)
            p = b.maxpool(y, 3, 2, 1, nd=2); b.release(y)
            y = p
        for li in range(1, 5):
            blocks = list(getattr(self, "layer%d" % li))
            t1 = None
            for bi, blk in enumerate(blocks):
                nxt = blocks[bi + 1] if bi + 1 < len(blocks) else None
                chain = (nxt is not None and blk.is_identity_bottleneck() and nxt.is_identity_bottleneck() and
                         tuple(blk.conv3.weight.shape[:2]) == (1024, 256) and tuple(nxt.conv1.weight.shape[:2]) == (256, 1024) and b.dtype == torch.bfloat16 and
                         not b.live_weights)
                if chain:
                    z, t1n = blk.record(b, y, t1=t1, next_block=nxt)
                elif t1 is not None:
                    z, t1n = blk.record(b, y, t1=t1), None
                else:
                    z, t1n = blk.record(b, y), None
                b.release(y)
                y, t1 = z, t1n
        alg = self.alg_confidences.record(b, y) if hasattr(self, "alg_confidences") else None
        vol = self.vol_confidences.record(b, y) if hasattr(self, "vol_confidences") else None
        for i in range(0, len(self.deconv_layers), 3):
            dc, bn = self.deconv_layers[i], self.deconv_layers[i + 1]
            z = b.conv(y, dc.weight, dc.bias, bn_tuple(bn), stride=2, pad=1, transposed=True, relu=True)
            b.release(y)
            y = z
        feats = y
        hm = None
        if want_heatmaps:
            fl = self.final_layer
            hm = b.conv(feats, fl.weight, fl.bias, None, stride=1, pad=fl.padding[0], out_f32=True)
        return hm, feats, alg, vol

    def heatmap_shape(self, h, w):
        def down(v, k, s, p):
            return (v + 2 * p - k) // s + 1
        for k, s, p in ((7, 2, 3), (3, 2, 1), (3, 2, 1), (3, 2, 1), (3, 2, 1)):
            h, w = down(h, k, s, p), down(w, k, s, p)
        return h * 8, w * 8

    def forward(self, x):
        H.require_gpu(x, "images")
        if self.training:
            raise NotImplementedError("training runs through VolumetricTriangulationNet, whose step is recorded as a whole (lt_train.py); "
                                      "the stand-alone forward of this module is inference only: call .eval()")
        key = (tuple(x.shape), self.compute_dtype, x.device)
        N, _, Hh, W = x.shape

        def build():
            b = E.PlanBuilder(x.device, self.compute_dtype)
            inp = b.alloc((N, 1, Hh, W, E.min_cin_of(self.compute_dtype)))
            outs = self.record(b, inp, True)
            return {"plan": b.finish(), "inp": inp, "outs": outs}

        with torch.cuda.device(x.device):
            P = self._plan_for(key, build)
            plan, inp, (hm, feats, alg, vol) = P["plan"], P["inp"], P["outs"]
            st = torch.cuda.current_stream(x.device).cuda_stream
            E.stage_images(x.float().contiguous(), inp, st)
            plan.run_eager(st)
            to_nchw = lambda a: a.t[:, 0].permute(0, 3, 1, 2).to(torch.float32, copy=True)
            conf = lambda a: None if a is None else a.t.reshape(N, -1).clone()
            return to_nchw(hm), to_nchw(feats), conf(alg), conf(vol)


def get_pose_net(config, device="cuda:0"):
    kind, layers = resnet_spec[config.num_layers]
    if config.style == "caffe":
        kind = "bottleneck"
    model = PoseResNet(kind, layers, config.num_joints, num_input_channels=3, deconv_with_bias=False, num_deconv_layers=3,
                       num_deconv_filters=(256, 256, 256), num_deconv_kernels=(4, 4, 4), final_conv_kernel=1,
                       alg_confidences=config.alg_confidences, vol_confidences=config.vol_confidences,
                       caffe=(config.style == "caffe"))
    if config.init_weights:
        print("Loading pretrained weights from: {}".format(config.checkpoint))
        own = model.state_dict()
        loaded = torch.load(config.checkpoint, map_location="cpu")
        loaded = loaded.get("state_dict", loaded)
        picked = {}
        for k, v in loaded.items():
            name = k.replace("module.", "")
            if name in own and v.shape == own[name].shape:
                picked[name] = v
            elif name in ("final_layer.weight", "final_layer.bias"):
                print("Reiniting final layer:", k)
                o = torch.zeros_like(own[name])
                if name.endswith("weight"):
                    nn.init.xavier_uniform_(o)
                n = min(o.shape[0], v.shape[0])
                o[:n] = v[:n]
                picked[name] = o
        missing = {k.replace("module.", "") for k in loaded} - set(picked)
        if missing:
            print("Parameters [{}] were not inited".format(missing))
        model.load_state_dict(picked, strict=False)
        print("Successfully loaded pretrained weights for backbone")
    return model
```

learnable-triangulation-pytorch_amd/mvn/models/triangulation.py:

```python
import ctypes as C

from collections import OrderedDict

import os

import numpy as np
import torch
import torch.nn as nn

import lt_engine as E
import lt_hip as H
from mvn.models import pose_resnet
from mvn.models.v2v import V2VModel
from mvn.utils import multiview, op, volumetric


GEO_RING = 4
MAX_LAUNCH_ELEMS = 2 ** 31


def _bn_in_train_mode(m):
    return any(isinstance(c, nn.modules.batchnorm._BatchNorm) and c.training for c in m.modules())


# ... 238 lines not shown

    @staticmethod
    def forward(ctx, plan, x, *params):
        ctx.set_materialize_grads(False)
        with torch.cuda.device(x.device):
            hm, conf = plan.forward(x)
        ctx.plan, ctx.step_id, ctx.params = plan, plan.step_id, params
        if conf.numel() == 0:
            ctx.mark_non_differentiable(conf)
        return hm, conf

    @staticmethod
    def backward(ctx, g_hm, g_conf):
        plan = ctx.plan
        if ctx.step_id != plan.step_id:
            raise RuntimeError("only the LATEST training forward of a shape can be backpropagated (its activations live in the plan's buffers, "
                               "which a newer forward has overwritten)")
        with torch.cuda.device(plan.device):
            pg = plan.backward(g_hm, g_conf)
        return (None, None) + tuple(pg.get(p) if p.requires_grad else None for p in ctx.params)


class _PlannedNet(E.PlanCache):

    def __init__(self):
        super().__init__()
        self.compute_dtype = torch.float32
        self.use_graph = True
        self.copy_outputs = True
        self.tile_override = 0
        self._stream = None
        self._init_plan_cache()

    def set_compute_dtype(self, dtype):
        H.dtype_code(dtype)
        self.compute_dtype = dtype
        return self

    def _open_plan(self, N, Hh, W, device, dry_run=False):
        b = E.PlanBuilder(device, self.compute_dtype, self.tile_override, dry_run=dry_run)
        x_in = b.alloc((N, 1, Hh, W, E.min_cin_of(self.compute_dtype)))
        x_in.pooled = False
        return b, x_in

    def _side_stream(self, device):
        if self._stream is None or self._stream.device != device:
            self._stream = torch.cuda.Stream(device=device)
        return self._stream


class VolumetricTriangulationNet(_PlannedNet):
    def __init__(self, config, device="cuda:0"):
        super().__init__()
        m = config.model
        self.num_joints = m.backbone.num_joints
        self.volume_aggregation_method = m.volume_aggregation_method
        self.volume_softmax = m.volume_softmax
        self.volume_multiplier = m.volume_multiplier
        self.volume_size = m.volume_size
        self.cuboid_side = m.cuboid_side
        self.kind = m.kind
        self.use_gt_pelvis = m.use_gt_pelvis
        self.heatmap_softmax = m.heatmap_softmax
        self.heatmap_multiplier = m.heatmap_multiplier
        self.transfer_cmu_to_human36m = m.transfer_cmu_to_human36m if hasattr(m, "transfer_cmu_to_human36m") else False
        if self.volume_aggregation_method not in H.AGG:
            raise ValueError("Unknown volume_aggregation_method: {}".format(self.volume_aggregation_method))
        m.backbone.alg_confidences = False
        m.backbone.vol_confidences = self.volume_aggregation_method.startswith("conf")
        self.backbone = pose_resnet.get_pose_net(m.backbone, device=device)
        for p in self.backbone.final_layer.parameters():
            p.requires_grad = False
        self.process_features = nn.Sequential(nn.Conv2d(256, 32, 1))
        self.volume_net = V2VModel(32, self.num_joints)
        if hasattr(m, "compute_dtype"):
            self.compute_dtype = {"fp32": torch.float32, "float32": torch.float32, "bf16": torch.bfloat16,
                                  "bfloat16": torch.bfloat16}[str(m.compute_dtype)]

    def _build_plan(self, B, NV, Hh, W, device, dry_run=False):
        V, J = self.volume_size, self.num_joints
        b, x_in = self._open_plan(B * NV, Hh, W, device, dry_run)
        lib = b.lib
        image_cell = {"ptr": None, "ref": None}
        _, feats256, _, volc = self.backbone.record(b, x_in, want_heatmaps=False, image_cell=image_cell)
        if not b.npre:
            image_cell = None
        pf = self.process_features[0]
        feats = b.conv(feats256, pf.weight, pf.bias, None)
        b.release(feats256)
        feats.pooled = False
        h, w = feats.shape[2], feats.shape[3]
        n_geo = B * NV * 12 + B * 15
        geo = torch.zeros(n_geo, dtype=torch.float32, device=device)
        geo_ring = [torch.zeros(n_geo, dtype=torch.float32) for _ in range(1 if dry_run else GEO_RING)]
        if not dry_run:
            geo_ring = [g.pin_memory() for g in geo_ring]
        geo_host = geo_ring[0]
        o_pos, o_cen, o_rot = B * NV * 12, B * NV * 12 + 3 * B, B * NV * 12 + 6 * B
        coords = torch.empty(B, V, V, V, 3, dtype=torch.float32, device=device)
        step = float(np.float32(self.cuboid_side / (V - 1)))
        gp = geo.data_ptr()
        cmu = int(bool(self.transfer_cmu_to_human36m))
        conf = None
        if volc is not None:
            conf = volc.t.reshape(B, NV, 32)
        vol = b.alloc((B, V, V, V, 32))
        esz = E.esize(self.compute_dtype)
        agg = H.AGG[self.volume_aggregation_method]
        b.custom(lambda st: H.check(lib.lt_unproject_grid_fwd(b.code, feats.t.data_ptr(), gp, gp + 4 * o_pos, gp + 4 * o_cen, gp + 4 * o_rot, step, cmu,
                                                              coords.data_ptr(), H.ptr(conf), vol.t.data_ptr(), B, NV, 32, h, w, V, agg, st),
                                    "lt_unproject_grid_fwd"),
                 "unproject", nbytes=(B * NV * h * w * 32 + B * V ** 3 * 32) * esz + B * V ** 3 * 12,
                 info={"feats": feats, "geo": geo, "coords": coords, "conf": conf, "vol": vol, "agg": self.volume_aggregation_method, "NV": NV,
                       "offs": (o_pos, o_cen, o_rot), "step": step, "cmu": cmu})
        logits = self.volume_net.record(b, vol)
        kp = torch.empty(B, J, 3, dtype=torch.float32, device=device)
        probs = torch.empty(B, J, V, V, V, dtype=torch.float32, device=device)
        ws = torch.empty(1 if dry_run else max(1, lib.lt_softargmax3d_workspace(B, J, V ** 3)), dtype=torch.uint8, device=device)
        mult, sm = float(self.volume_multiplier), int(bool(self.volume_softmax))
        cl = int(logits.t.is_contiguous())
        assert cl or logits.t.permute(0, 4, 1, 2, 3).is_contiguous()
        b.custom(lambda st, outs=None: None if not outs or len(outs) < 3 or outs[2] is None else H.check(lib.lt_nhwc_to_nchw_f32(
                     b.code, feats.t.data_ptr(), outs[2].data_ptr(), B * NV, 32, h * w, 32, st), "lt_nhwc_to_nchw_f32"),
                 "features_out", nbytes=B * NV * h * w * 32 * (esz + 4), info={"feats": feats}, tail=True)
        b.custom(lambda st, outs=None: H.check(lib.lt_softargmax3d_fwd(
                     logits.t.data_ptr(), coords.data_ptr(), mult, sm, cl, J, (outs[0] if outs else kp).data_ptr(),
                     (outs[1] if outs else probs).data_ptr(), B, J, V ** 3, ws.data_ptr(), st), "lt_softargmax3d_fwd"),
                 "softargmax3d", nbytes=2 * B * J * V ** 3 * 4,
                 info={"logits": logits, "coords": coords, "mult": mult, "softmax": sm, "kp": kp, "probs": probs}, tail=True)
        plan = b.finish()
        plan.keep += [geo, geo_ring, coords, kp, probs, ws]
        if image_cell is not None and not dry_run:
            x_in.t.untyped_storage().resize_(0)
        return {"plan": plan, "x_in": x_in, "image_cell": image_cell, "feats": feats, "geo": geo, "geo_host": geo_host, "geo_ring": geo_ring,
                "geo_events": [None] * len(geo_ring), "geo_slot": 0, "coords": coords, "kp": kp,
                "probs": probs, "conf": conf, "logits": logits, "vol": vol, "hw": (h, w), "offs": (o_pos, o_cen, o_rot),
                "captured": False}

    def _host_cameras(self, batch, B, image_shape, P):
        h, w = P["hw"]
        K, R, t = multiview.stack_cameras(batch["cameras"])
        proj = multiview.resized_projections(K, R, t, image_shape, (h, w))
        axis = [0, 1, 0] if self.kind == "coco" else [0, 0, 1]
        rot = np.empty((B, 9))
        for i in range(B):
            theta = np.random.uniform(0.0, 2 * np.pi) if self.training else 0.0
            rot[i] = volumetric.get_rotation_matrix(axis, theta).reshape(-1)
        o_pos, o_cen, o_rot = P["offs"]
        slot = P["geo_slot"] = (P["geo_slot"] + 1) % len(P["geo_ring"])
        ev = P["geo_events"][slot]
        if ev is not None:
            ev.synchronize()
        gh = P["geo_host"] = P["geo_ring"][slot]
        gh[:o_pos] = torch.from_numpy(proj.astype(np.float32).reshape(-1))
        gh[o_rot:] = torch.from_numpy(rot.astype(np.float32).reshape(-1))
        return gh

    def _host_geometry(self, batch, B, image_shape, P):
        kp3d = batch["keypoints_3d"] if self.use_gt_pelvis else batch["pred_keypoints_3d"]
        base = np.empty((B, 3), dtype=np.float64)
        for i in range(B):
            k3 = np.asarray(kp3d[i])
            base[i] = (k3[11, :3] + k3[12, :3]) / 2 if self.kind == "coco" else k3[6, :3]
        sides = np.array([self.cuboid_side] * 3)
        position = base - sides / 2
        gh = self._host_cameras(batch, B, image_shape, P)
        o_pos, o_cen, o_rot = P["offs"]
        gh[o_pos:o_cen] = torch.from_numpy(position.astype(np.float32).reshape(-1))
        gh[o_cen:o_rot] = torch.from_numpy(base.astype(np.float32).reshape(-1))
        return position, base, sides

    def max_samples_per_launch(self, NV, Hh, W):
# ... 415 lines not shown
```

Before: 1425.

## Fuse process_features 1x1 conv into last transposed-deconv halo kernel epilogue

Adds a fused path in the 2D halo transposed-conv kernel where the 256-channel ReLU output tile is fed directly into a 256->32 pointwise MFMA. Partial sums across the eight waves are reduced in LDS with serialized barriers, then bias and scale are applied and only the 32-channel result is written. This removes one kernel launch and the write and re-read of the full 256-channel feature map. In exchange it adds many barriers, extra LDS use and occupancy 1. The halo path is also relaxed to accept heights divisible by 4 via a TH=4 variant.

```diff
diff --git a/include/lt_hip.h b/include/lt_hip.h
--- a/include/lt_hip.h
+++ b/include/lt_hip.h
@@ -80,6 +80,15 @@
 } lt_conv_skip;
 int lt_conv_skip_fwd(const lt_conv_desc* desc, const void* x, const float* bias, const float* scale, const float* shift,
                      const lt_conv_skip* skip, void* y, void* stream);
+typedef struct lt_conv_pw {
+    const void* weight;
+    const float* bias;
+    const float* scale;
+    const float* shift;
+    int32_t cin, cout, cout_pad, k_pad, ldc, flags;
+} lt_conv_pw;
+int lt_conv_pw_fwd(const lt_conv_desc* desc, const void* x, const float* bias, const float* scale, const float* shift,
+                   const lt_conv_pw* pw, void* y, void* stream);
 typedef struct lt_conv_cat2 {
     const void* x;
     int32_t cin, H, W, stride;
@@ -94,6 +103,7 @@
     int64_t s[5];
 } lt_wshape;
 int lt_sel_conv_skip(int32_t dtype, const int32_t x[5], const lt_wshape* w, const int32_t skip_x[5], const lt_wshape* skip_w);
+int lt_sel_conv_pw(const lt_conv_desc* d, const lt_wshape* w, const lt_wshape* pw_w);
 int lt_sel_conv_cat2(int32_t dtype, const int32_t t2[5], const lt_wshape* w_expand, const int32_t x[5], const lt_wshape* w_down, int32_t stride_down);
 int lt_sel_splitk_slices(const lt_conv_desc* d, const lt_wshape* w, int32_t transposed);
 int lt_sel_bottleneck(int32_t dtype, const int32_t x[5], const lt_wshape w[3], const int32_t strides[3]);
@@ -329,6 +339,7 @@
     int32_t graph_captured;
     const float* logits;
     int32_t logits_planar;
+    int32_t n_conv_pw;
 } lt_plan_info_t;
 int lt_plan_create_vol(const lt_vol_plan_config* cfg, const lt_named_tensor* weights, int32_t nweights, lt_plan** plan_out);
 int lt_plan_forward_vol(lt_plan* plan, const float* images, const double* K_host, const double* R_host, const double* t_host, const double* base_points_host,
diff --git a/learnable-triangulation-pytorch_amd/csrc/conv2d_halo.hip b/learnable-triangulation-pytorch_amd/csrc/conv2d_halo.hip
--- a/learnable-triangulation-pytorch_amd/csrc/conv2d_halo.hip
+++ b/learnable-triangulation-pytorch_amd/csrc/conv2d_halo.hip
@@ -1,4 +1,5 @@
 #include <stdlib.h>
+#include <string.h>
 
 #include <type_traits>
 
@@ -49,10 +50,15 @@
     int N, H, W, OH, OW, osh, osw, ldc, flags, tiles_h, tiles_w, pad_h, pad_w;
     int tile0;
     Halo2dPhase ph[4];
+    const bf16_t* pw_w;
+    const float* pw_bias;
+    const float* pw_scale;
+    const float* pw_shift;
+    int pw_cout, pw_cout_pad, pw_kpad, pw_ldc, pw_flags;
 };
 
-template <int TH, int NT, int NPH>
-__global__ __launch_bounds__(512, (TH == 8 ? 1 : 2)) void conv2d_halo_kernel(const Halo2dArgs a) {
+template <int TH, int NT, int NPH, bool FPW>
+__device__ __forceinline__ void halo2d_body(const Halo2dArgs& a) {
     typedef bf16_t T;
     constexpr int CIN = 256, CP = 256, TW = 24, G = CIN / 16, NB = CP / 32, PW = TW + 2, HH = TH + 2, PXB = CIN * 2;
     constexpr int RG = TH / 4, CG = TW / 8, FR = RG * CG;
@@ -116,6 +122,21 @@
     };
     if constexpr (NPH > 1) load_consts();
     const EpiFloors fl = epi_floors(a.flags);
+    [[maybe_unused]] V16 w1[2];
+    [[maybe_unused]] float* const red = (float*)(smem + HV * PXB);
+    [[maybe_unused]] float* const pwc = red + FR * 1024;
+    if constexpr (FPW) {
+#pragma unroll
+        for (int kb = 0; kb < 2; ++kb) {
+            w1[kb].u = make_uint4(0, 0, 0, 0);
+            if (vl < a.pw_cout_pad) w1[kb].u = *(const uint4*)(a.pw_w + (size_t)vl * a.pw_kpad + 32 * cb + 16 * kb + 8 * hk);
+        }
+        if (t < 32) {
+            const bool in = t < a.pw_cout;
+            const float bi = in && a.pw_bias ? a.pw_bias[t] : 0.f, sc = in && a.pw_scale ? a.pw_scale[t] : 1.f, sf = in && a.pw_shift ? a.pw_shift[t] : 0.f;
+            pwc[t] = sc; pwc[32 + t] = bi * sc + sf;
+        }
+    }
     int tapo[NPH][NT];
     {
         int4 tv[NPH][NT];
@@ -135,7 +156,8 @@
         if (bad) __builtin_trap();
     }
 
-    asm volatile("s_waitcnt vmcnt(0)\n\ts_barrier" ::: "memory");
+    if constexpr (FPW) asm volatile("s_waitcnt vmcnt(0) lgkmcnt(0)\n\ts_barrier" ::: "memory");
+    else asm volatile("s_waitcnt vmcnt(0)\n\ts_barrier" ::: "memory");
 
     static_for_p<0, NPH>([&](auto pc) {
         constexpr int p = decltype(pc)::value;
@@ -180,22 +202,87 @@
         });
 
         if constexpr (NPH == 1) load_consts();
-#pragma unroll
-        for (int f = 0; f < FR; ++f) {
-            const int th = 4 * (f / CG) + (vl >> 3), tw = 8 * (f % CG) + (vl & 7);
-            bf16_t* yo = a.y + (((size_t)n * a.OH + (h0 + th) * a.osh + a.ph[p].ooh) * a.OW + (w0 + tw) * a.osw + a.ph[p].oow) * a.ldc + 32 * cb + 8 * hk;
-#pragma unroll
-            for (int q = 0; q < 2; ++q) {
-                unsigned o[4];
-#pragma unroll
-                for (int d = 0; d < 4; ++d) {
-                    const int e = 8 * q + 2 * d;
-                    o[d] = pack_bf16x2(epi_apply(fmaf(acc[f][e], esc[e], esf[e]), fl, 0.f), epi_apply(fmaf(acc[f][e + 1], esc[e + 1], esf[e + 1]), fl, 0.f));
+        if constexpr (FPW) {
+#pragma unroll
+            for (int f = 0; f < FR; ++f) {
+                V16 b[2];
+#pragma unroll
+                for (int q = 0; q < 2; ++q) {
+                    unsigned o[4];
+#pragma unroll
+                    for (int d = 0; d < 4; ++d) {
+                        const int e = 8 * q + 2 * d;
+                        o[d] = pack_bf16x2(epi_apply(fmaf(acc[f][e], esc[e], esf[e]), fl, 0.f), epi_apply(fmaf(acc[f][e + 1], esc[e + 1], esf[e + 1]), fl, 0.f));
+                    }
+                    b[q].u = make_uint4(o[0], o[1], o[2], o[3]);
                 }
-                *(uint4*)(yo + 16 * q) = make_uint4(o[0], o[1], o[2], o[3]);
+#pragma unroll
+                for (int e = 0; e < 16; ++e) acc[f][e] = 0.f;
+                acc[f] = __builtin_amdgcn_mfma_f32_32x32x16_bf16(w1[0].h, b[0].h, acc[f], 0, 0, 0);
+                acc[f] = __builtin_amdgcn_mfma_f32_32x32x16_bf16(w1[1].h, b[1].h, acc[f], 0, 0, 0);
+            }
+            __syncthreads();
+            for (int i = 0; i < wave; ++i) __syncthreads();
+#pragma unroll
+            for (int f = 0; f < FR; ++f) {
+                float* r = red + f * 1024 + 128 * hk + vl;
+#pragma unroll
+                for (int e = 0; e < 16; ++e) {
+                    const int co = (e & 3) + 8 * (e >> 2);
+                    float v = acc[f][e];
+                    if (wave > 0) v = r[co * 32] + v;
+                    r[co * 32] = v;
+                }
+                __syncthreads();
+            }
+            for (int i = wave; i < 7; ++i) __syncthreads();
+            const EpiFloors fl2 = epi_floors(a.pw_flags);
+            const bool vec = (a.pw_ldc & 7) == 0 && (a.pw_cout & 7) == 0;
+            for (int it = t; it < FR * 128; it += 512) {
+                const int f = it >> 7, v = (it >> 2) & 31, c8 = it & 3;
+                const int th = 4 * (f / CG) + (v >> 3), tw = 8 * (f % CG) + (v & 7);
+                const float* r = red + f * 1024 + c8 * 256 + v;
+                float val[8];
+#pragma unroll
+                for (int j = 0; j < 8; ++j) val[j] = epi_apply(fmaf(r[j * 32], pwc[8 * c8 + j], pwc[32 + 8 * c8 + j]), fl2, 0.f);
+                bf16_t* yo = a.y + (((size_t)n * a.OH + (h0 + th) * a.osh + a.ph[p].ooh) * a.OW + (w0 + tw) * a.osw + a.ph[p].oow) * a.pw_ldc + 8 * c8;
+                if (vec) {
+                    if (8 * c8 < a.pw_cout)
+                        *(uint4*)yo = make_uint4(pack_bf16x2(val[0], val[1]), pack_bf16x2(val[2], val[3]), pack_bf16x2(val[4], val[5]), pack_bf16x2(val[6], val[7]));
+                } else {
+#pragma unroll
+                    for (int j = 0; j < 8; ++j)
+                        if (8 * c8 + j < a.pw_cout) yo[j] = (bf16_t)(pack_bf16x2(val[j], 0.f) & 0xffffu);
+                }
+            }
+        } else {
+#pragma unroll
+            for (int f = 0; f < FR; ++f) {
+                const int th = 4 * (f / CG) + (vl >> 3), tw = 8 * (f % CG) + (vl & 7);
+                bf16_t* yo = a.y + (((size_t)n * a.OH + (h0 + th) * a.osh + a.ph[p].ooh) * a.OW + (w0 + tw) * a.osw + a.ph[p].oow) * a.ldc + 32 * cb + 8 * hk;
+#pragma unroll
+                for (int q = 0; q < 2; ++q) {
+                    unsigned o[4];
+#pragma unroll
+                    for (int d = 0; d < 4; ++d) {
+                        const int e = 8 * q + 2 * d;
+                        o[d] = pack_bf16x2(epi_apply(fmaf(acc[f][e], esc[e], esf[e]), fl, 0.f), epi_apply(fmaf(acc[f][e + 1], esc[e + 1], esf[e + 1]), fl, 0.f));
+                    }
+                    *(uint4*)(yo + 16 * q) = make_uint4(o[0], o[1], o[2], o[3]);
+                }
             }
         }
     });
+}
+
+template <int TH, int NT, int NPH>
+__global__ __launch_bounds__(512, (TH == 8 ? 1 : 2)) void conv2d_halo_kernel(const Halo2dArgs a) {
+    halo2d_body<TH, NT, NPH, false>(a);
+}
+
+template <int TH>
+__global__ __launch_bounds__(512, 1) void conv2d_halo_pw_kernel(const Halo2dArgs a) {
+    halo2d_body<TH, 4, 4, true>(a);
 }
 
 template <int TH, int NT, int NPH>
@@ -216,28 +303,51 @@
     return LT_OK;
 }
 
+template <int TH>
+int launch_halo2d_pw(const Halo2dArgs& a0, hipStream_t s) {
+    Halo2dArgs a = a0;
+    a.tiles_h = a.H / TH;
+    a.tiles_w = a.W / 24;
+    const long long total = (long long)a.N * a.tiles_h * a.tiles_w;
+    if (total <= 0) return LT_OK;
+    a.tile0 = 0;
+    constexpr int lds = (TH + 2) * 26 * 512 + (TH / 4) * 3 * 4096 + 256;
+    static_assert(lds <= 160 * 1024, "halo + reduction buffer fit LDS");
+    auto kern = conv2d_halo_pw_kernel<TH>;
+    LT_OPT_IN_LDS(kern, 160 * 1024);
+    hipLaunchKernelGGL(kern, dim3((unsigned)total), dim3(512), lds, s, a);
+    LT_CHECK_LAUNCH("lt_conv_pw_fwd(2D halo)");
+    return LT_OK;
+}
+
+void halo2d_args(const ConvArgs& c, int nphase, Halo2dArgs& a) {
+    memset(&a, 0, sizeof(a));
+    for (int p = 0; p < nphase; ++p) {
+        const PhaseArg& ph = c.phase[p];
+        a.ph[p].wfrag = (const bf16_t*)ph.wfrag_t; a.ph[p].taps = ph.taps; a.ph[p].ooh = ph.ooh; a.ph[p].oow = ph.oow;
+    }
+    a.x = (const bf16_t*)c.x; a.y = (bf16_t*)c.y;
+    a.bias = c.bias; a.scale = c.scale; a.shift = c.shift;
+    a.N = c.N; a.H = c.H; a.W = c.W; a.OH = c.OH; a.OW = c.OW; a.osh = c.osh; a.osw = c.osw; a.ldc = c.ldc; a.flags = c.flags;
+    a.pad_h = c.ph; a.pad_w = c.pw;
+}
+
 }
 
 namespace lt {
 
 int conv2d_halo_try(int dtype, const ConvArgs& c, int cout_pad, int nphase, hipStream_t s) {
     if (dtype != LT_BF16 || c.res || c.skip_x || c.x2 || !halo2d_fits(c, cout_pad, nphase)) return 0;
+    for (int p = 0; p < nphase; ++p)
+        if (!c.phase[p].wfrag_t) return 0;
     Halo2dArgs a;
-    for (int p = 0; p < nphase; ++p) {
-        const PhaseArg& ph = c.phase[p];
-        if (!ph.wfrag_t) return 0;
-        a.ph[p].wfrag = (const bf16_t*)ph.wfrag_t; a.ph[p].taps = ph.taps; a.ph[p].ooh = ph.ooh; a.ph[p].oow = ph.oow;
-    }
-    a.x = (const bf16_t*)c.x; a.y = (bf16_t*)c.y;
-    a.bias = c.bias; a.scale = c.scale; a.shift = c.shift;
-    a.N = c.N; a.H = c.H; a.W = c.W; a.OH = c.OH; a.OW = c.OW; a.osh = c.osh; a.osw = c.osw; a.ldc = c.ldc; a.flags = c.flags; a.tiles_h = a.tiles_w = 0;
-    a.pad_h = c.ph; a.pad_w = c.pw; a.tile0 = 0;
+    halo2d_args(c, nphase, a);
     const char* th = getenv("LT_H2D_TH");
     const long long tiles8 = (long long)c.N * (c.H / 8) * (c.W / 24);
     const int n_cu = lt::device_cu_count8();
     const bool th4 = th ? th[0] == '4' : tiles8 <= n_cu / 2;
     int rc;
-    if (nphase != 1) rc = launch_halo2d<8, 4, 4>(a, s);
+    if (nphase != 1) rc = c.H % 8 ? launch_halo2d<4, 4, 4>(a, s) : launch_halo2d<8, 4, 4>(a, s);
     else if (th4) rc = launch_halo2d<4, 9, 1>(a, s);
     else {
         const long long rem = tiles8 % n_cu;
@@ -250,4 +360,20 @@
     return rc == LT_OK ? 1 : rc;
 }
 
-}
+int conv2d_halo_pw_try(const ConvArgs& c, int cout_pad, int nphase, const lt_conv_pw& pw, void* y, hipStream_t s) {
+    if (c.res || c.skip_x || c.x2 || nphase != 4 || !halo2d_fits(c, cout_pad, nphase)) return 0;
+    for (int p = 0; p < nphase; ++p)
+        if (!c.phase[p].wfrag_t) return 0;
+    if (!pw.weight || pw.cin != 256 || pw.cout < 1 || pw.cout > 32 || pw.cout_pad < pw.cout || pw.cout_pad > 32 || pw.k_pad < 256 || pw.k_pad % 8 ||
+        pw.ldc < pw.cout || (pw.flags & ~LT_EPI_RELU_POST))
+        return 0;
+    Halo2dArgs a;
+    halo2d_args(c, nphase, a);
+    a.y = (bf16_t*)y;
+    a.pw_w = (const bf16_t*)pw.weight; a.pw_bias = pw.bias; a.pw_scale = pw.scale; a.pw_shift = pw.shift;
+    a.pw_cout = pw.cout; a.pw_cout_pad = pw.cout_pad; a.pw_kpad = pw.k_pad; a.pw_ldc = pw.ldc; a.pw_flags = pw.flags;
+    const int rc = c.H % 8 ? launch_halo2d_pw<4>(a, s) : launch_halo2d_pw<8>(a, s);
+    return rc == LT_OK ? 1 : rc;
+}
+
+}
diff --git a/learnable-triangulation-pytorch_amd/csrc/conv_common.h b/learnable-triangulation-pytorch_amd/csrc/conv_common.h
--- a/learnable-triangulation-pytorch_amd/csrc/conv_common.h
+++ b/learnable-triangulation-pytorch_amd/csrc/conv_common.h
@@ -68,7 +68,7 @@
 
 inline bool halo2d_fits(const ConvArgs& c, int cout_pad, int nphase) {
     if ((nphase != 1 && nphase != 4) || c.D != 1 || c.Do != 1 || c.OD != 1) return false;
-    if (c.sh != 1 || c.sw != 1 || c.H != c.Ho || c.W != c.Wo || c.W % 24 || c.H % 8) return false;
+    if (c.sh != 1 || c.sw != 1 || c.H != c.Ho || c.W != c.Wo || c.W % 24 || c.H % (nphase == 4 ? 4 : 8)) return false;
     if (c.Cin != 256 || cout_pad != 256 || c.Cout != 256 || c.ldc % 8 || (c.flags & (LT_EPI_STORE_F32 | LT_EPI_SIGMOID)) || c.pd != 0) return false;
     if (nphase == 1 && (c.osh != 1 || c.osw != 1 || c.OH != c.Ho || c.OW != c.Wo || c.ph != 1 || c.pw != 1)) return false;
     if (nphase == 4 && (c.osh != 2 || c.osw != 2 || c.OH != 2 * c.Ho || c.OW != 2 * c.Wo || c.ph != 0 || c.pw != 0)) return false;
@@ -154,6 +154,7 @@
 int conv7_try(const ConvArgs& a, int cout_pad, int max_taps, bool pw, hipStream_t s);
 int conv_pw_try(int dtype, const ConvArgs& a, int cout_pad, int nphase, hipStream_t s);
 int conv2d_halo_try(int dtype, const ConvArgs& a, int cout_pad, int nphase, hipStream_t s);
+int conv2d_halo_pw_try(const ConvArgs& a, int cout_pad, int nphase, const lt_conv_pw& pw, void* y, hipStream_t s);
 int conv3d_halo_try(int dtype, const ConvArgs& a, int cout_pad, int nphase, bool forced, hipStream_t s);
 
 }
diff --git a/learnable-triangulation-pytorch_amd/csrc/conv_igemm.hip b/learnable-triangulation-pytorch_amd/csrc/conv_igemm.hip
--- a/learnable-triangulation-pytorch_amd/csrc/conv_igemm.hip
+++ b/learnable-triangulation-pytorch_amd/csrc/conv_igemm.hip
@@ -427,6 +427,24 @@
     return conv_fwd_impl(d, x, bias, scale, shift, nullptr, skip, nullptr, y, stream);
 }
 
+extern "C" int lt_conv_pw_fwd(const lt_conv_desc* d, const void* x, const float* bias, const float* scale, const float* shift,
+                              const lt_conv_pw* pw, void* y, void* stream) {
+    LT_REQUIRE(d && x && y && pw, LT_ERR_INVALID, "lt_conv_pw_fwd: null argument");
+    LT_REQUIRE(d->dtype == LT_BF16 && d->nphase == 4 && d->Cin == 256 && d->Cout == 256 && d->cout_pad == 256 && d->k_pad > 0, LT_ERR_UNSUPPORTED,
+               "lt_conv_pw_fwd: bf16 four-phase transposed convolution 256 -> 256 only (dtype %d, nphase %d, Cin %d, Cout %d)", d->dtype, d->nphase, d->Cin, d->Cout);
+    LT_REQUIRE((long long)d->N * d->H * d->W * 256 < (1ll << 31) && (long long)d->N * d->OH * d->OW * 256 < (1ll << 31) && d->N >= 1, LT_ERR_UNSUPPORTED,
+               "lt_conv_pw_fwd: batch of %d samples too large for one launch", d->N);
+    for (int p = 0; p < d->nphase; ++p)
+        LT_REQUIRE(d->phase[p].taps && d->phase[p].weight_frag && d->phase[p].weight_frag_layout == 2 && d->phase[p].ntaps == 4, LT_ERR_INVALID,
+                   "lt_conv_pw_fwd: phase %d needs four taps and weights in fragment layout 2", p);
+    ConvArgs a = conv_args_of(*d);
+    a.x = x; a.y = nullptr; a.bias = bias; a.scale = scale; a.shift = shift; a.log2Cin = 8; a.M = d->N * d->Do * d->Ho * d->Wo;
+    const int rc = conv2d_halo_pw_try(a, d->cout_pad, d->nphase, *pw, y, (hipStream_t)stream);
+    LT_REQUIRE(rc == 1, rc < 0 ? rc : LT_ERR_UNSUPPORTED, "lt_conv_pw_fwd: not covered by conv2d_halo_kernel (N %d, %d x %d; 1x1 %d -> %d, k_pad %d, ldc %d, flags 0x%x)",
+               d->N, d->H, d->W, pw->cin, pw->cout, pw->k_pad, pw->ldc, pw->flags);
+    return LT_OK;
+}
+
 extern "C" int lt_conv_cout_pad(int32_t cout) {
     if (cout <= 16) return 16;
     if (cout <= 32) return 32;
diff --git a/learnable-triangulation-pytorch_amd/csrc/plan.hip b/learnable-triangulation-pytorch_amd/csrc/plan.hip
--- a/learnable-triangulation-pytorch_amd/csrc/plan.hip
+++ b/learnable-triangulation-pytorch_amd/csrc/plan.hip
@@ -212,6 +212,7 @@
     int npre = 0, ntail = 0;
     std::deque<lt_conv_desc> conv_descs;
     std::deque<lt_conv_skip> skip_descs;
+    std::deque<lt_conv_pw> pw_conv_descs;
     std::deque<lt_conv_cat2> cat2_descs;
     std::deque<lt_pwchain_desc> pw_descs;
     std::deque<lt_stem_desc> stem_descs;
@@ -233,7 +234,7 @@
     int hm_h = 0, hm_w = 0;
     lt_plan* sub_alg = nullptr; lt_plan* sub_vol = nullptr; int kind = 0;
     float* cproj_dev = nullptr; float* cproj_host[GEO_RING] = {nullptr, nullptr, nullptr, nullptr}; float* ckp_alg = nullptr;
-    int n_xr = 0, n_bneck = 0, n_bneck_ds = 0, n_cat2 = 0, n_halo2d = 0, n_pwchain = 0, n_stem = 0, n_splitk = 0, n_conv_skip = 0;
+    int n_xr = 0, n_bneck = 0, n_bneck_ds = 0, n_cat2 = 0, n_halo2d = 0, n_pwchain = 0, n_stem = 0, n_splitk = 0, n_conv_skip = 0, n_conv_pw = 0;
 
     ~lt_plan() {
         if (graph) (void)hipGraphExecDestroy(graph);
@@ -304,6 +305,7 @@
         int stride = 1, pad = 0; bool transposed = false, relu = false, relu_pre = false, out_f32 = false, sigmoid = false;
         const Act* residual = nullptr;
         const Act* skip_x = nullptr; const WT* skip_w = nullptr; const float* skip_bias = nullptr; const BN* skip_bn = nullptr;
+        const WT* pw_w = nullptr; const float* pw_bias = nullptr;
     };
 
     void fill_desc(lt_conv_desc& d, const ConvSpec& sp) {
@@ -360,7 +362,22 @@
         fill_desc(d0, sp);
         const int S = lt_sel_splitk_slices(&d0, &ws, o.transposed);
         if (S > 1) return conv_splitk(x, w, sp, S, o.residual, y);
-        PL_TRY(alloc(sp.N, sp.OD, sp.OH, sp.OW, sp.Cout, o.out_f32 ? 4 : es, y));
+        lt_conv_pw* pw = nullptr;
+        ConvSpec ps;
+        if (o.pw_w) {
+            const lt_wshape pws = wshape(*o.pw_w);
+            LT_REQUIRE(!o.residual && !sk && !o.out_f32 && lt_sel_conv_pw(&d0, &ws, &pws), LT_ERR_INVALID, "plan: conv_pw on an unsupported shape");
+            const int pin[5] = {sp.N, sp.OD, sp.OH, sp.OW, sp.Cout};
+            PL_TRY(make_conv_spec(*o.pw_w, o.pw_bias, nullptr, pin, 1, 0, es, false, 0, 0, ps));
+            pw_conv_descs.emplace_back();
+            pw = &pw_conv_descs.back();
+            memset(pw, 0, sizeof(*pw));
+            PL_TRY(upload_w(ps.ph[0].w, &pw->weight));
+            PL_TRY(upload_f32(ps.bias, &pw->bias)); PL_TRY(upload_f32(ps.scale, &pw->scale)); PL_TRY(upload_f32(ps.shift, &pw->shift));
+            pw->cin = sp.Cout; pw->cout = ps.Cout; pw->cout_pad = ps.cout_pad; pw->k_pad = ps.k_pad; pw->ldc = ps.Cout; pw->flags = 0;
+            ++n_conv_pw;
+        }
+        PL_TRY(alloc(sp.N, sp.OD, sp.OH, sp.OW, pw ? ps.Cout : sp.Cout, o.out_f32 ? 4 : es, y));
         if (o.residual) LT_REQUIRE(o.residual->n == y.n && o.residual->d == y.d && o.residual->h == y.h && o.residual->w == y.w && o.residual->c == y.c && o.residual->es == es,
                                    LT_ERR_INVALID, "plan: residual shape");
         conv_descs.push_back(d0);
@@ -387,8 +404,22 @@
         if (sk) {
             flops += 2.0 * sp.N * sp.Do * sp.Ho * sp.Wo * sp.Cout * 16;
             ops.push_back([=](hipStream_t s) { return lt_conv_skip_fwd(dp, xp, bi, sc, sh, sk, yp, s); });
+        } else if (pw) {
+            flops += 2.0 * sp.N * sp.OD * sp.OH * sp.OW * ps.Cout * sp.Cout;
+            ops.push_back([=](hipStream_t s) { return lt_conv_pw_fwd(dp, xp, bi, sc, sh, pw, yp, s); });
         } else
             ops.push_back([=](hipStream_t s) { return lt_conv_fwd(dp, xp, bi, sc, sh, rp, yp, s); });
+        return LT_OK;
+    }
+
+    int can_conv_pw(const Act& x, const WT& w, const ConvOpt& o, const WT& pw_w, bool& yes) {
+        const int in[5] = {x.n, x.d, x.h, x.w, x.c};
+        ConvSpec sp;
+        PL_TRY(make_conv_spec(w, o.bias, o.bn, in, o.stride, o.pad, es, o.transposed, o.relu ? LT_EPI_RELU_POST : 0, 0, sp));
+        lt_conv_desc d;
+        fill_desc(d, sp);
+        const lt_wshape ws = wshape(w), pws = wshape(pw_w);
+        yes = o.transposed && !o.residual && lt_sel_conv_pw(&d, &ws, &pws) != 0;
         return LT_OK;
     }
 
@@ -705,7 +736,8 @@
         return LT_OK;
     }
 
-    int record_backbone(int N, int Hh, int W, int num_layers, bool caffe, const char* conf_head, bool want_heatmaps, Act& feats256, Act& conf, Act& heatmaps) {
+    int record_backbone(int N, int Hh, int W, int num_layers, bool caffe, const char* conf_head, bool want_heatmaps, Act& feats256, Act& conf, Act& heatmaps,
+                        const WT* tail_pw_w = nullptr, const float* tail_pw_b = nullptr) {
         int nb[4]; bool bott;
         switch (num_layers) {
             case 18: bott = false; nb[0] = 2; nb[1] = 2; nb[2] = 2; nb[3] = 2; break;
@@ -768,6 +800,10 @@
             if (has("backbone.deconv_layers." + std::to_string(3 * i) + ".bias")) PL_TRY(get_vec("backbone.deconv_layers." + std::to_string(3 * i) + ".bias", (int)dw.s[1], &db));
             LT_REQUIRE(dw.s[2] == 4 && dw.s[3] == 4, LT_ERR_UNSUPPORTED, "%s: only the 4x4 stride-2 deconvolution of the reference configs", who);
             ConvOpt o; o.bias = db; o.bn = &dbn; o.stride = 2; o.pad = 1; o.transposed = true; o.relu = true;
+            if (i == 2 && tail_pw_w && !want_heatmaps) {
+                bool fuse; PL_TRY(can_conv_pw(y, dw, o, *tail_pw_w, fuse));
+                if (fuse) { o.pw_w = tail_pw_w; o.pw_bias = tail_pw_b; }
+            }
             Act z; PL_TRY(conv(y, dw, o, z)); release(y);
             y = z;
         }
@@ -862,12 +898,16 @@
         const int B = cfg.B, NV = cfg.NV, V = cfg.volume_size, J = cfg.num_joints;
         Act f256, no_hm;
         const bool conf_head = cfg.aggregation == LT_AGG_CONF || cfg.aggregation == LT_AGG_CONF_NORM;
-        PL_TRY(record_backbone(B * NV, cfg.H, cfg.W, cfg.num_layers, cfg.style_caffe != 0, conf_head ? "backbone.vol_confidences" : nullptr, false, f256, volc, no_hm));
         WT pw; const float* pb;
         PL_TRY(get("process_features.0.weight", pw, 4)); PL_TRY(get_vec("process_features.0.bias", (int)pw.s[0], &pb));
         LT_REQUIRE(pw.s[0] == 32, LT_ERR_UNSUPPORTED, "lt_plan_create_vol: process_features has %d output channels (32)", (int)pw.s[0]);
-        ConvOpt o; o.bias = pb;
-        PL_TRY(conv(f256, pw, o, feats)); release(f256);
+        const int n_pw0 = n_conv_pw;
+        PL_TRY(record_backbone(B * NV, cfg.H, cfg.W, cfg.num_layers, cfg.style_caffe != 0, conf_head ? "backbone.vol_confidences" : nullptr, false, f256, volc, no_hm, &pw, pb));
+        if (n_conv_pw > n_pw0) feats = f256;
+        else {
+            ConvOpt o; o.bias = pb;
+            PL_TRY(conv(f256, pw, o, feats)); release(f256);
+        }
         feats.pooled = false;
         hm_h = feats.h; hm_w = feats.w;
         n_geo = (size_t)B * NV * 12 + (size_t)B * 15; o_pos = (size_t)B * NV * 12; o_cen = o_pos + 3 * B; o_rot = o_pos + 6 * B;
@@ -1242,7 +1282,7 @@
         info->flops += a.flops; info->bytes_allocated += a.bytes_allocated + (int64_t)p->bytes_alloc;
         info->n_expand_reduce += a.n_expand_reduce; info->n_bottleneck += a.n_bottleneck; info->n_bottleneck_ds += a.n_bottleneck_ds; info->n_conv_cat2 += a.n_conv_cat2;
         info->n_conv2d_halo += a.n_conv2d_halo; info->n_pwchain += a.n_pwchain; info->n_stem_pool += a.n_stem_pool; info->n_splitk += a.n_splitk;
-        info->n_conv_skip += a.n_conv_skip;
+        info->n_conv_skip += a.n_conv_skip; info->n_conv_pw += a.n_conv_pw;
         info->graph_captured = (!p->sub_alg->cfg.use_graph || a.graph_captured) && (!p->sub_vol->cfg.use_graph || info->graph_captured) &&
                                (p->sub_alg->cfg.use_graph || p->sub_vol->cfg.use_graph) ? 1 : 0;
         return LT_OK;
@@ -1251,7 +1291,7 @@
     info->heatmap_h = p->hm_h; info->heatmap_w = p->hm_w;
     info->flops = p->flops; info->bytes_allocated = (int64_t)p->bytes_alloc;
     info->n_expand_reduce = p->n_xr; info->n_bottleneck = p->n_bneck; info->n_bottleneck_ds = p->n_bneck_ds; info->n_conv_cat2 = p->n_cat2;
-    info->n_conv2d_halo = p->n_halo2d; info->n_pwchain = p->n_pwchain; info->n_stem_pool = p->n_stem; info->n_splitk = p->n_splitk; info->n_conv_skip = p->n_conv_skip;
+    info->n_conv2d_halo = p->n_halo2d; info->n_pwchain = p->n_pwchain; info->n_stem_pool = p->n_stem; info->n_splitk = p->n_splitk; info->n_conv_skip = p->n_conv_skip; info->n_conv_pw = p->n_conv_pw;
     info->graph_captured = p->captured ? 1 : 0;
     info->logits = (const float*)p->logits.p; info->logits_planar = p->logits.planar ? 1 : 0;
     return LT_OK;
diff --git a/learnable-triangulation-pytorch_amd/csrc/select.hip b/learnable-triangulation-pytorch_amd/csrc/select.hip
--- a/learnable-triangulation-pytorch_amd/csrc/select.hip
+++ b/learnable-triangulation-pytorch_amd/csrc/select.hip
@@ -28,6 +28,13 @@
     const int nc = lt_conv_chunk_samples(N, (long long)D * H * W * 32);
     if (nc < 1) return 0;
     return halo_col_fits(nc, D, H, W) && halo_col_fits(N - (N - 1) / nc * nc, D, H, W);
+}
+
+extern "C" int lt_sel_conv_pw(const lt_conv_desc* d, const lt_wshape* w, const lt_wshape* pw_w) {
+    if (d->dtype != LT_BF16 || env_on("LT_NO_CONV_PW")) return 0;
+    if (pw_w->nd != 4 || !pointwise(pw_w) || pw_w->s[1] != 256 || pw_w->s[0] < 1 || pw_w->s[0] > 32) return 0;
+    if (d->nphase != 4 || lt_sel_frag_layout(d, w, 1, 0) != 2) return 0;
+    return (long long)d->N * d->H * d->W * 256 < (1ll << 31) && (long long)d->N * d->OH * d->OW * 256 < (1ll << 31);
 }
 
 extern "C" int lt_sel_conv_cat2(int32_t dtype, const int32_t t2[5], const lt_wshape* we, const int32_t x[5], const lt_wshape* wd, int32_t s) {
diff --git a/learnable-triangulation-pytorch_amd/lt_engine.py b/learnable-triangulation-pytorch_amd/lt_engine.py
--- a/learnable-triangulation-pytorch_amd/lt_engine.py
+++ b/learnable-triangulation-pytorch_amd/lt_engine.py
@@ -204,7 +204,7 @@
     def _declines(self, *a, **k):
         return False
 
-    can_conv_skip = can_conv_cat2 = can_chain_pointwise = can_bottleneck = can_bottleneck_ds = can_expand_reduce = can_stem_pool = _declines
+    can_conv_skip = can_conv_pw = can_conv_cat2 = can_chain_pointwise = can_bottleneck = can_bottleneck_ds = can_expand_reduce = can_stem_pool = _declines
 
 
 class PlanBuilder(Recorder):
@@ -269,6 +269,12 @@
             return False
         return bool(H.lib().lt_sel_conv_skip(self.code, H.dims(x_shape), H.wshape(weight), H.dims(skip_shape), H.wshape(skip_weight)))
 
+    def can_conv_pw(self, x_shape, weight, bias, bn, pw_weight):
+        if not self._fusable():
+            return False
+        spec = make_conv_spec(weight, bias, bn, x_shape, 2, 1, self.dtype, True, H.EPI_RELU_POST)
+        return bool(H.lib().lt_sel_conv_pw(self._desc(spec), H.wshape(weight), H.wshape(pw_weight)))
+
     def _desc(self, spec):
         d = H.ConvDesc()
         d.dtype = self.code
@@ -316,7 +322,7 @@
         return spec, wfr.data_ptr(), sc.data_ptr(), sh.data_ptr()
 
     def conv(self, x, weight, bias=None, bn=None, stride=1, pad=0, transposed=False, relu=False, relu_pre=False,
-             residual=None, out_f32=False, out=None, sigmoid=False, output_padding=0, residual_f32=False, skip=None):
+             residual=None, out_f32=False, out=None, sigmoid=False, output_padding=0, residual_f32=False, skip=None, pw=None):
         flags = ((H.EPI_RELU_POST if relu else 0) | (H.EPI_RELU_PRE if relu_pre else 0) | (H.EPI_STORE_F32 if out_f32 else 0)
                  | (H.EPI_SIGMOID if sigmoid else 0) | (H.EPI_RES_F32 if residual_f32 else 0))
         assert not residual_f32 or (out_f32 and residual is not None and self.dtype in (torch.bfloat16, torch.float8_e4m3fn))
@@ -337,7 +343,19 @@
         S = self.splitk_slices(spec, weight, transposed, out_f32, sigmoid, out)
         if S > 1:
             return self._conv_splitk(x, weight, spec, S, residual)
-        y = out or self.alloc((spec.N, spec.OD, spec.OH, spec.OW, spec.Cout), torch.float32 if out_f32 else self.out_dtype)
+        pw_info = None
+        if pw is not None:
+            assert (transposed and residual is None and skip is None and not out_f32 and out is None and not relu_pre and not sigmoid and relu
+                    and stride == 2 and pad == 1 and self.can_conv_pw(x.shape, weight, bias, bn, pw[0]))
+            ps = make_conv_spec(pw[0], pw[1], None, (spec.N, spec.OD, spec.OH, spec.OW, spec.Cout), 1, 0, self.dtype, False, 0)
+            pwd = H.ConvPw()
+            pwt = [self.const(ps.phases[0].weight, self.dtype), self.const(ps.bias), self.const(ps.scale), self.const(ps.shift)]
+            pwd.weight, pwd.bias, pwd.scale, pwd.shift = (t.data_ptr() for t in pwt)
+            pwd.cin, pwd.cout, pwd.cout_pad, pwd.k_pad, pwd.ldc, pwd.flags = spec.Cout, ps.Cout, ps.cout_pad, ps.k_pad, ps.Cout, 0
+            self.keep.append(pwd)
+            pw_info = {"spec": ps, "desc": pwd}
+        y = out or self.alloc((spec.N, spec.OD, spec.OH, spec.OW, pw_info["spec"].Cout if pw_info else spec.Cout),
+                              torch.float32 if out_f32 else self.out_dtype)
         self.keep.append(x.t)
         if residual is not None:
             self.keep.append(residual.t)
@@ -375,6 +393,17 @@
             self._add(lambda s, d=d, xp=x.t.data_ptr(), bip=bi.data_ptr(), scp=sc.data_ptr(), shp=sh.data_ptr(), sk=skip_info["desc"], yp=y.t.data_ptr():
                       H.check(self.lib.lt_conv_skip_fwd(C.byref(d), xp, bip, scp, shp, C.byref(sk), yp, s), "lt_conv_skip_fwd"),
                       "conv", label + " + skip conv1x1x1 16->32", 2 * macs, nbytes, info)
+            return y
+        if pw_info is not None:
+            ps = pw_info["spec"]
+            pmacs = spec.N * spec.OD * spec.OH * spec.OW * ps.Cout * spec.Cout
+            macs += pmacs
+            self.flops += 2 * pmacs
+            nbytes += ps.phases[0].weight.numel() * esz
+            info["pw"] = pw_info
+            self._add(lambda s, d=d, xp=x.t.data_ptr(), bip=bi.data_ptr(), scp=sc.data_ptr(), shp=sh.data_ptr(), pwd=pw_info["desc"], yp=y.t.data_ptr():
+                      H.check(self.lib.lt_conv_pw_fwd(C.byref(d), xp, bip, scp, shp, C.byref(pwd), yp, s), "lt_conv_pw_fwd"),
+                      "conv", label + " + conv1x1 %d->%d" % (spec.Cout, ps.Cout), 2 * macs, nbytes, info)
             return y
         self._add(lambda s, d=d, xp=x.t.data_ptr(), bip=bi.data_ptr(), scp=sc.data_ptr(), shp=sh.data_ptr(),
                   rp=H.ptr(residual.t) if residual is not None else None, yp=y.t.data_ptr():
diff --git a/learnable-triangulation-pytorch_amd/lt_hip.py b/learnable-triangulation-pytorch_amd/lt_hip.py
--- a/learnable-triangulation-pytorch_amd/lt_hip.py
+++ b/learnable-triangulation-pytorch_amd/lt_hip.py
@@ -42,6 +42,10 @@
     _fields_ = [("x", vp), ("cin", i32), ("weight_frag", vp)]
 
 
+class ConvPw(C.Structure):
+    _fields_ = [("weight", vp), ("bias", vp), ("scale", vp), ("shift", vp), ("cin", i32), ("cout", i32), ("cout_pad", i32), ("k_pad", i32), ("ldc", i32), ("flags", i32)]
+
+
 class ConvCat2(C.Structure):
     _fields_ = [("x", vp), ("cin", i32), ("H", i32), ("W", i32), ("stride", i32)]
 
@@ -110,7 +114,7 @@
 class PlanInfo(C.Structure):
     _fields_ = [("launches", i32), ("heatmap_h", i32), ("heatmap_w", i32), ("flops", C.c_double), ("bytes_allocated", C.c_int64),
                 ("n_expand_reduce", i32), ("n_bottleneck", i32), ("n_bottleneck_ds", i32), ("n_conv_cat2", i32), ("n_conv2d_halo", i32), ("n_pwchain", i32),
-                ("n_stem_pool", i32), ("n_splitk", i32), ("n_conv_skip", i32), ("graph_captured", i32), ("logits", vp), ("logits_planar", i32)]
+                ("n_stem_pool", i32), ("n_splitk", i32), ("n_conv_skip", i32), ("graph_captured", i32), ("logits", vp), ("logits_planar", i32), ("n_conv_pw", i32)]
 
 
 SIGNATURES = {
@@ -127,10 +131,12 @@
     "lt_device_info": (C.c_int, [C.POINTER(C.c_int), C.POINTER(C.c_int), C.c_char_p, C.c_int]),
     "lt_conv_fwd": (C.c_int, [C.POINTER(ConvDesc), vp, vp, vp, vp, vp, vp, vp]),
     "lt_conv_skip_fwd": (C.c_int, [C.POINTER(ConvDesc), vp, vp, vp, vp, C.POINTER(ConvSkip), vp, vp]),
+    "lt_conv_pw_fwd": (C.c_int, [C.POINTER(ConvDesc), vp, vp, vp, vp, C.POINTER(ConvPw), vp, vp]),
     "lt_conv_cat2_fwd": (C.c_int, [C.POINTER(ConvDesc), vp, C.POINTER(ConvCat2), vp, vp, vp, vp, vp, vp]),
     "lt_conv_cout_pad": (C.c_int, [i32]),
     "lt_conv_chunk_samples": (i32, [i32, i64]),
     "lt_sel_conv_skip": (C.c_int, [i32, i32 * 5, C.POINTER(WShape), i32 * 5, C.POINTER(WShape)]),
+    "lt_sel_conv_pw": (C.c_int, [C.POINTER(ConvDesc), C.POINTER(WShape), C.POINTER(WShape)]),
     "lt_sel_conv_cat2": (C.c_int, [i32, i32 * 5, C.POINTER(WShape), i32 * 5, C.POINTER(WShape), i32]),
     "lt_sel_splitk_slices": (C.c_int, [C.POINTER(ConvDesc), C.POINTER(WShape), i32]),
     "lt_sel_bottleneck": (C.c_int, [i32, i32 * 5, WShape * 3, i32 * 3]),
diff --git a/learnable-triangulation-pytorch_amd/mvn/models/pose_resnet.py b/learnable-triangulation-pytorch_amd/mvn/models/pose_resnet.py
--- a/learnable-triangulation-pytorch_amd/mvn/models/pose_resnet.py
+++ b/learnable-triangulation-pytorch_amd/mvn/models/pose_resnet.py
@@ -152,7 +152,7 @@
         self.compute_dtype = torch.float32
         self._init_plan_cache()
 
-    def record(self, b, x, want_heatmaps=True, image_cell=None):
+    def record(self, b, x, want_heatmaps=True, image_cell=None, tail_pw=None):
         if b.can_stem_pool(x, self.conv1.weight, 2, 3, (3, 2, 1)):
             y = b.stem_pool(x, self.conv1.weight, bn_tuple(self.bn1), image_cell=image_cell)
         else:
@@ -179,7 +179,11 @@
         vol = self.vol_confidences.record(b, y) if hasattr(self, "vol_confidences") else None
         for i in range(0, len(self.deconv_layers), 3):
             dc, bn = self.deconv_layers[i], self.deconv_layers[i + 1]
-            z = b.conv(y, dc.weight, dc.bias, bn_tuple(bn), stride=2, pad=1, transposed=True, relu=True)
+            pw = None
+            if (tail_pw is not None and not want_heatmaps and i + 3 >= len(self.deconv_layers)
+                    and b.can_conv_pw(y.shape, dc.weight, dc.bias, bn_tuple(bn), tail_pw[0])):
+                pw = tail_pw
+            z = b.conv(y, dc.weight, dc.bias, bn_tuple(bn), stride=2, pad=1, transposed=True, relu=True, **({"pw": pw} if pw is not None else {}))
             b.release(y)
             y = z
         feats = y
diff --git a/learnable-triangulation-pytorch_amd/mvn/models/triangulation.py b/learnable-triangulation-pytorch_amd/mvn/models/triangulation.py
--- a/learnable-triangulation-pytorch_amd/mvn/models/triangulation.py
+++ b/learnable-triangulation-pytorch_amd/mvn/models/triangulation.py
@@ -344,12 +344,15 @@
         b, x_in = self._open_plan(B * NV, Hh, W, device, dry_run)
         lib = b.lib
         image_cell = {"ptr": None, "ref": None}
-        _, feats256, _, volc = self.backbone.record(b, x_in, want_heatmaps=False, image_cell=image_cell)
+        pf = self.process_features[0]
+        _, feats256, _, volc = self.backbone.record(b, x_in, want_heatmaps=False, image_cell=image_cell, tail_pw=(pf.weight, pf.bias))
         if not b.npre:
             image_cell = None
-        pf = self.process_features[0]
-        feats = b.conv(feats256, pf.weight, pf.bias, None)
-        b.release(feats256)
+        if feats256.shape[-1] != pf.weight.shape[1]:
+            feats = feats256
+        else:
+            feats = b.conv(feats256, pf.weight, pf.bias, None)
+            b.release(feats256)
         feats.pooled = False
         h, w = feats.shape[2], feats.shape[3]
         n_geo = B * NV * 12 + B * 15
```

Result: no change. 1424 (-0.1%).
